# jyf588/SimGAN

Measured on AMD Instinct MI355X. Metric: env-steps/sec of GAIL-dyn PPO update, higher is better.
Workload: dtype f32; 1 GPU; northstar: GAIL-dyn update, T=128 N=512/GPU obs=47 act=12 D-in=86 policy=mlp h64 D h100 ppo_epoch=10 num_mini_batch=1...; optimizer_steps_per_update=2720, parallelism=single GPU

## Files before the change

simgan_amd/_lib.py:

```python
import ctypes as C
import os

import numpy as np

_HERE = os.path.dirname(os.path.abspath(__file__))
LIB_PATH = os.path.join(_HERE, "libsimgan_hip.so")

c_float_p = C.POINTER(C.c_float)
c_i64_p = C.POINTER(C.c_int64)
c_double_p = C.POINTER(C.c_double)
c_u8_p = C.POINTER(C.c_uint8)
c_int_p = C.POINTER(C.c_int)
H = C.c_void_p

F_OBS, F_OBS_FEAT, F_ACTIONS, F_REWARDS, F_VALUE_PREDS, F_RETURNS, F_LOGP, F_MASKS, F_BAD_MASKS, \
    F_ADVANTAGES = range(10)
POLICY_MLP, POLICY_SPLIT, POLICY_GRU = 0, 1, 2
PROF_DISC_CHAIN, PROF_DISC_WGRAD, PROF_PPO_FWD, PROF_PPO_BWD, PROF_PPO_REDUCE, PROF_RELABEL, PROF_PPO_ADAM = range(7)


class PPOConfig(C.Structure):
    _fields_ = [("clip_param", C.c_float), ("ppo_epoch", C.c_int), ("num_mini_batch", C.c_int),
                ("value_loss_coef", C.c_float), ("entropy_coef", C.c_float), ("lr", C.c_float),
                ("eps", C.c_float), ("max_grad_norm", C.c_float),
# ... 40 lines not shown
                                         c_float_p, c_float_p]),
    "sg_policy_act_ensemble": (C.c_int, [C.POINTER(H), C.c_int, C.POINTER(C.c_int32), c_float_p, C.c_int, c_float_p, C.c_uint64,
                                         C.c_int, c_float_p, c_float_p, c_float_p]),
    "sg_rollout_create": (C.c_int, [H, C.c_int, C.c_int, C.c_int, C.c_int, C.c_int, C.POINTER(H)]),
    "sg_rollout_destroy": (C.c_int, [H]),
    "sg_rollout_upload": (C.c_int, [H, C.c_int, c_float_p, C.c_int64]),
    "sg_rollout_download": (C.c_int, [H, C.c_int, c_float_p, C.c_int64]),
    "sg_rollout_upload_step": (C.c_int, [H, C.c_int, C.c_int, c_float_p, C.c_int64]),
    "sg_rollout_download_step": (C.c_int, [H, C.c_int, C.c_int, c_float_p, C.c_int64]),
    "sg_rollout_after_update": (C.c_int, [H]),
    "sg_rollout_compute_returns": (C.c_int, [H, c_float_p, C.c_int, C.c_float, C.c_float, C.c_int]),
    "sg_rollout_compute_returns_policy": (C.c_int, [H, H, C.c_int, C.c_float, C.c_float, C.c_int]),
    "sg_rollout_fill_synthetic": (C.c_int, [H, H, C.c_uint64, C.c_float]),
    "sg_rollout_count_dones": (C.c_int, [H, c_double_p]),
    "sg_ppo_create": (C.c_int, [H, H, C.POINTER(PPOConfig), C.POINTER(H)]),
    "sg_ppo_destroy": (C.c_int, [H]),
    "sg_ppo_set_lr": (C.c_int, [H, C.c_float]),
    "sg_ppo_update": (C.c_int, [H, H, c_i64_p, C.c_int64, C.c_uint64, c_float_p]),
    "sg_ppo_last_perms": (C.c_int, [H, c_i64_p, C.c_int64]),
    "sg_ppo_set_hidden_states": (C.c_int, [H, c_float_p, C.c_int64]),
    "sg_ppo_get_adam": (C.c_int, [H, c_float_p, c_float_p, C.c_int64, c_i64_p]),
    "sg_ppo_set_adam": (C.c_int, [H, c_float_p, c_float_p, C.c_int64, C.c_int64]),
    "sg_ppo_set_symmetry": (C.c_int, [H, C.c_float, c_float_p, c_float_p]),
    "sg_ppo_set_mirrored_obs": (C.c_int, [H, c_float_p, C.c_int64]),
    "sg_ppo_last_symmetry_loss": (C.c_int, [H, c_float_p]),
    "sg_a2c_create": (C.c_int, [H, H, C.POINTER(A2CConfig), C.POINTER(H)]),
    "sg_a2c_get_rmsprop": (C.c_int, [H, c_float_p, C.c_int64, c_i64_p]),
    "sg_a2c_set_rmsprop": (C.c_int, [H, c_float_p, C.c_int64, C.c_int64]),
    "sg_acktr_create": (C.c_int, [H, H, C.POINTER(ACKTRConfig), C.POINTER(H)]),
    "sg_acktr_set_value_noise": (C.c_int, [H, c_float_p, C.c_int64]),
    "sg_acktr_get_state": (C.c_int, [H, c_float_p, C.c_int64, c_float_p, C.c_int64, c_float_p, C.c_int64, c_i64_p]),
    "sg_disc_create": (C.c_int, [H, C.c_int, C.c_int, C.POINTER(H)]),
    "sg_disc_destroy": (C.c_int, [H]),
    "sg_disc_num_params": (C.c_int, [H, c_i64_p]),
    "sg_disc_set_params": (C.c_int, [H, c_float_p, C.c_int64]),
    "sg_disc_get_params": (C.c_int, [H, c_float_p, C.c_int64]),
    "sg_disc_get_adam": (C.c_int, [H, c_float_p, c_float_p, C.c_int64, c_i64_p]),
    "sg_disc_set_adam": (C.c_int, [H, c_float_p, c_float_p, C.c_int64, C.c_int64]),
    "sg_disc_set_expert": (C.c_int, [H, c_float_p, C.c_int64]),
    "sg_disc_update_gail_dyn": (C.c_int, [H, H, C.c_int, c_i64_p, C.c_int64, c_i64_p, C.c_int64, c_float_p, C.c_int64, C.c_uint64,
                                          c_float_p, c_int_p]),
    "sg_disc_update_rows": (C.c_int, [H, c_float_p, C.c_int64, C.c_int, C.c_int, c_i64_p, C.c_int64, c_i64_p, C.c_int64, c_float_p,
                                      C.c_int64, C.c_uint64, c_float_p, c_int_p]),
    "sg_disc_predict_reward": (C.c_int, [H, c_float_p, C.c_int, C.c_float, c_float_p, C.c_float, c_float_p, c_float_p]),
    "sg_disc_predict_prob": (C.c_int, [H, c_float_p, C.c_int, c_float_p]),
    "sg_disc_predict_reward_steps": (C.c_int, [H, H, C.c_float, C.c_float, c_float_p, c_float_p]),
    "sg_disc_grad_pen": (C.c_int, [H, c_float_p, c_float_p, c_float_p, C.c_int, C.c_uint64, c_float_p]),
    "sg_disc_last_draws": (C.c_int, [H, c_i64_p, c_i64_p, c_float_p, c_i64_p]),
    "sg_disc_reset_returns": (C.c_int, [H]),
    "sg_disc_get_returns": (C.c_int, [H, c_float_p, C.c_int, c_int_p]),
    "sg_disc_set_returns": (C.c_int, [H, c_float_p, C.c_int]),
    "sg_disc_relabel_rewards": (C.c_int, [H, H, C.c_float, C.c_float, c_double_p]),
    "sg_disc_relabel_rewards_auto": (C.c_int, [H, H, C.c_float, C.c_double, C.c_int]),
    "sg_disc_set_rms": (C.c_int, [H, c_double_p]),
    "sg_disc_get_scalars": (C.c_int, [H, c_double_p]),
    "sg_results_publish": (C.c_int, [H, H, H, C.c_int]),
    "sg_results_fetch": (C.c_int, [H, C.c_int, c_double_p]),
    "sg_ctx_profile": (C.c_int, [H, C.c_int]),
    "sg_ctx_profile_read": (C.c_int, [H, C.c_int, c_double_p, c_i64_p]),
    "sg_ctx_profile_reset": (C.c_int, [H]),
    "sg_host_alloc": (C.c_int, [C.c_int64, C.POINTER(C.c_void_p)]),
    "sg_host_free": (C.c_int, [C.c_void_p]),
    "sg_ctx_mark": (C.c_int, [H, c_int_p]),
    "sg_ctx_mark_elapsed": (C.c_int, [H, C.c_int, C.c_int, c_double_p]),
}

TEST_LIB_PATH = os.path.join(_HERE, "libsimgan_hip_test.so")
c_ll_p = C.POINTER(C.c_longlong)
TEST_PROTOTYPES = {
    "sg_test_last_error": (C.c_char_p, []),
    "sg_test_gemm": (C.c_int, [H, C.c_int, C.c_int, C.c_int, C.c_int, c_float_p, c_float_p, c_float_p]),
    "sg_test_gemm_bench": (C.c_int, [H, C.c_int, C.c_int, C.c_int, C.c_int, C.c_int, C.c_int, C.c_int, c_ll_p]),
    "sg_test_mfma_probe": (C.c_int, [H, C.c_int, c_float_p, c_float_p, c_float_p]),
    "sg_test_flag_probe": (C.c_int, [H, C.c_int, C.c_int, C.c_int, C.c_int, c_ll_p, c_float_p]),
    "sg_test_fetch_probe": (C.c_int, [H, C.c_int, C.c_int, C.c_int, c_ll_p]),
    "sg_test_pmc_calibrate": (C.c_int, [H, C.c_int64]),
    "sg_test_pstep_probe": (C.c_int, [H, C.c_int, C.c_int, C.c_int, C.c_int, C.c_int, c_ll_p, c_int_p]),
    "sg_test_graph_state": (C.c_int, [H, H, c_int_p]),
    "sg_test_disc_phase_times": (C.c_int, [H, C.c_int, c_ll_p, C.c_int]),
    "sg_test_disc_step4_times": (C.c_int, [H, C.c_int, c_ll_p, C.c_int]),
    "sg_test_disc_gathers": (C.c_int, [H, c_ll_p]),
    "sg_test_ppo_phase_times": (C.c_int, [H, C.c_int, c_ll_p, C.c_int]),
    "sg_test_rng": (C.c_int, [H, C.c_int, C.c_int64, C.c_uint64, C.c_void_p]),
    "sg_test_kfac_eig": (C.c_int, [H, C.c_int, c_float_p, c_float_p, c_float_p, C.POINTER(C.c_int)]),
    "sg_test_acktr_noise": (C.c_int, [H, C.c_int64, C.c_uint64, C.c_int64, c_float_p]),
    "sg_test_raise_kfac_error": (C.c_int, [H]),
    "sg_test_tear_probe": (C.c_int, [H, C.c_int, C.c_int, C.c_int, c_ll_p]),
    "sg_test_raise_handoff_error": (C.c_int, [H, H]),
}
_TEST_LIB = None

_LIB = None


class SimganHipError(RuntimeError):
    pass


def load():
    global _LIB
    if _LIB is not None:
        return _LIB
    if not os.path.exists(LIB_PATH):
        raise SimganHipError(
            f"{LIB_PATH} not found: the HIP extension is not built. There is no CPU fallback; "
            "run `make -C simgan_amd/csrc` (hipcc, gfx950).")
    lib = C.CDLL(LIB_PATH)
    for name, (res, args) in PROTOTYPES.items():
        fn = getattr(lib, name)
        fn.restype = res
        fn.argtypes = args
    _LIB = lib
    return lib


def check(rc):
    if rc != 0:
        raise SimganHipError(load().sg_last_error().decode(errors="replace"))


def load_test():
    global _TEST_LIB
    if _TEST_LIB is not None:
        return _TEST_LIB
    load()
    if not os.path.exists(TEST_LIB_PATH):
        raise SimganHipError(f"{TEST_LIB_PATH} not found: run `make -C simgan_amd/csrc`")
    lib = C.CDLL(TEST_LIB_PATH)
    for name, (res, args) in TEST_PROTOTYPES.items():
        fn = getattr(lib, name)
        fn.restype = res
        fn.argtypes = args
    _TEST_LIB = lib
    return lib


def check_test(rc):
    if rc != 0:
        raise SimganHipError(load_test().sg_test_last_error().decode(errors="replace"))


def fptr(a):
    assert isinstance(a, np.ndarray) and a.dtype == np.float32 and a.flags["C_CONTIGUOUS"], (type(a), getattr(a, "dtype", None))
    return a.ctypes.data_as(c_float_p)


def i64ptr(a):
    assert isinstance(a, np.ndarray) and a.dtype == np.int64 and a.flags["C_CONTIGUOUS"]
    return a.ctypes.data_as(c_i64_p)


def as_f32(x):
    if hasattr(x, "detach"):
        x = x.detach().cpu().numpy()
    return np.ascontiguousarray(x, dtype=np.float32)


def as_i64(x):
    if hasattr(x, "detach"):
        x = x.detach().cpu().numpy()
    return np.ascontiguousarray(x, dtype=np.int64)


class _PinnedBlock(object):

    def __init__(self, nbytes):
# ... 143 lines not shown
```

simgan_amd/csrc/sg_common.h:

```cpp
#pragma once
#include <hip/hip_runtime.h>
#include <stdint.h>

#include <string>
#include <atomic>
#include <vector>
#include <mutex>
inline std::recursive_mutex& sg_capture_mutex() { static std::recursive_mutex m; return m; }
struct SgDeviceWideGuard {
    std::lock_guard<std::recursive_mutex> l{sg_capture_mutex()};
    ~SgDeviceWideGuard() { (void)hipGetLastError(); }
};
#define SG_DEVICE_WIDE() SgDeviceWideGuard _sg_device_wide_guard
static inline hipError_t sg_dev_malloc(void** p, size_t n) { std::lock_guard<std::recursive_mutex> l(sg_capture_mutex()); return hipMalloc(p, n); }
static inline hipError_t sg_dev_free(void* p) { std::lock_guard<std::recursive_mutex> l(sg_capture_mutex()); return hipFree(p); }
static inline hipError_t sg_host_malloc(void** p, size_t n) { std::lock_guard<std::recursive_mutex> l(sg_capture_mutex()); return hipHostMalloc(p, n, hipHostMallocDefault); }
static inline hipError_t sg_host_release(void* p) { std::lock_guard<std::recursive_mutex> l(sg_capture_mutex()); return hipHostFree(p); }

#include "../../include/simgan_hip.h"
#include "sg_gemm.hpp"

void sg_set_error(const char* fmt, ...);

#define SG_CHECK(expr)                                                                      \
// ... 79 lines not shown
    hipStream_t stream = nullptr;
    int num_cu = 0;
    int lds_bytes = 0;
    bool profile = false;
    SgProfSlot prof[SG_PROF_COUNT];
    std::vector<hipEvent_t> event_pool;
    std::vector<hipEvent_t> marks;
    SgComm* comm = nullptr;
    int rank = 0, world = 1;
    bool disc_sharded = false;
    bool use_comm = false;
    std::atomic<int> n_learners{0};
    float* d_scratch = nullptr;
    size_t scratch_bytes = 0;
    void* h_pinned = nullptr;
    size_t pinned_bytes = 0;
    double* mailbox = nullptr;
    double* results = nullptr;
    hipEvent_t res_ev[8] = {nullptr};
    struct sg_disc* res_d[8] = {nullptr};
    struct sg_ppo* res_a[8] = {nullptr};
};
#define SG_RESULT_SLOTS 8

bool sg_ctx_exclusive(const sg_ctx* ctx);
void sg_ctx_learner_born(sg_ctx* ctx);
void sg_ctx_learner_gone(sg_ctx* ctx);
int sg_ctx_scratch(sg_ctx* ctx, size_t bytes, float** out);
int sg_ctx_pinned(sg_ctx* ctx, size_t bytes, void** out);
int sg_ctx_fetch_f64(sg_ctx* ctx, const double* dev, double* host, int n);
int sg_ctx_put_f64(sg_ctx* ctx, double* dev, const double* host, int n);
struct SgEv { hipEvent_t a = nullptr, b = nullptr; };
SgEv sg_prof_events(sg_ctx* ctx, int which);
#ifdef __HIPCC__
#include <hip/hip_ext.h>
#define SG_LAUNCH(ctx, which, kernel, grid, block, lds, ...)                                                  \
    do {                                                                                                      \
        if ((ctx)->profile) {                                                                                 \
            SgEv _ev = sg_prof_events(ctx, which);                                                            \
            hipExtLaunchKernelGGL(kernel, grid, block, lds, (ctx)->stream, _ev.a, _ev.b, 0, __VA_ARGS__);     \
        } else {                                                                                              \
            hipLaunchKernelGGL(kernel, grid, block, lds, (ctx)->stream, __VA_ARGS__);                         \
        }                                                                                                     \
    } while (0)
#endif

struct SgGruDesc {
    int O, H, Op, ldO, Hp, ldH;
    int off;
    int wih, whh, bih, bhh;
    int total;
};
SgGruDesc sg_make_gru_desc(int O, int H, int off);
int64_t sg_gru_flat_count(const SgGruDesc& g);
void sg_gru_pad(const SgGruDesc& g, const float* flat, float* padded);
void sg_gru_unpad(const SgGruDesc& g, const float* padded, float* flat);

struct sg_policy {
    sg_ctx* ctx;
    SgPolicyDesc desc;
    bool recurrent = false;
    SgGruDesc gru;
    float* d_params = nullptr;
    float* d_io = nullptr;
    size_t io_bytes = 0;
};

size_t sg_policy_padded_count(const sg_policy* p);
bool sg_gru_fits(const sg_ctx* ctx, const SgGruDesc& g);

#define SG_STEP4_FLAG_WORD0 64
#define SG_STEP4_MAX_FLAGS 1024
#ifndef SG_STEP4_FLAG_STRIDE
#define SG_STEP4_FLAG_STRIDE 32
#endif
#define SG_STEP4_ERR_WORD (SG_STEP4_FLAG_WORD0 + SG_STEP4_MAX_FLAGS * SG_STEP4_FLAG_STRIDE)
#define SG_STEP4_STATE_BYTES (4 * (SG_STEP4_ERR_WORD + 16))
#define SG_PAIR_ERR_WORD 0
unsigned* sg_comm_peer_err_word(struct sg_ctx* ctx);
bool sg_comm_peer_on(const struct sg_ctx* ctx);
uint32_t sg_comm_peer_generation(const struct sg_ctx* ctx);
unsigned* sg_disc_err_word(struct sg_disc* d);
uint64_t sg_next_feat_version();
struct sg_rollout {
    sg_ctx* ctx;
    int T, N, O, A, F;
    float* d_field[SG_F_COUNT] = {nullptr};
    int64_t field_count[SG_F_COUNT] = {0};
    int field_slots[SG_F_COUNT] = {0};
    int field_width[SG_F_COUNT] = {0};
    int64_t* d_perm = nullptr;
    uint64_t feat_version = sg_next_feat_version();
};

#define SG_H0_SLOTS 8
struct sg_ppo {
    int64_t opt_t = 0;
    uint64_t scratch_key = 0;
    hipGraphExec_t steps_graph = nullptr;
    bool graph_refused = false;
    uint64_t steps_graph_key[18] = {0};
    sg_ctx* ctx;
    sg_policy* policy;
    sg_ppo_config cfg;
    float *d_m = nullptr, *d_v = nullptr, *d_grad = nullptr;
    float* d_slabs = nullptr;
    size_t slabs_cap = 0;
    float* d_stacks = nullptr;
    size_t stacks_cap = 0;
    float* d_state = nullptr;
    int64_t* d_perms = nullptr;
    int64_t perms_cap = 0;
    int64_t last_perm_count = 0;
    double* d_loss_acc = nullptr;
    float* d_part = nullptr;
    long long* d_dbg = nullptr;
    unsigned* d_pair = nullptr;
    bool self_wait_failed = false;
    bool pair_primed = false;
    float sym_coef = 0.f;
    float* d_mobs_mat = nullptr;
    float* d_mact = nullptr;
    float* d_mrows = nullptr;
    int64_t mrows_cap = 0;
    int64_t mrows_host = 0;
    float* d_h0 = nullptr;
    int64_t h0_cap = 0, h0_count = 0;
    float* h_h0 = nullptr;
    hipEvent_t h0_ev[8] = {nullptr};
    uint64_t h0_calls = 0;
    float* d_gru = nullptr;
    size_t gru_cap = 0;
    int64_t gru_layout[8] = {0};
    bool a2c = false;
    float alpha = 0.f;
    struct SgKfac* kfac = nullptr;
};

struct sg_disc {
    sg_ctx* ctx;
    SgDiscDesc desc;
    bool self_wait_failed = false;
    float *d_params = nullptr, *d_m = nullptr, *d_v = nullptr;
    float* d_slabs = nullptr;
    int n_slabs = 0;
    float* d_state = nullptr;
    float* d_expert = nullptr;
    int64_t n_expert = 0;
    int64_t *d_eperm = nullptr, *d_pperm = nullptr;
    int64_t eperm_cap = 0, pperm_cap = 0;
    float* d_alpha = nullptr;
    int64_t alpha_cap = 0;
    int64_t last_draws[3] = {0, 0, 0};
    float* d_feat_all = nullptr;
    int64_t feat_all_cap = 0;
    const float* gather_src = nullptr;
    int64_t gather_rows = 0;
    uint64_t gather_version = 0;
    int64_t n_gathers = 0;
    int64_t opt_t = 0;
    hipGraphExec_t epoch_graph = nullptr;
    bool graph_refused = false;
    uint64_t epoch_graph_key[12] = {0};
    float* d_wT = nullptr;
    float *d_erows = nullptr, *d_prows = nullptr;
    int64_t erows_cap = 0, prows_cap = 0;
    float* d_rows = nullptr;
    int64_t rows_cap = 0;
    double* d_loss_acc = nullptr;
    double* d_scal = nullptr;
    int last_n_d = 0;
    float* d_returns = nullptr;
    int returns_n = 0;
    bool returns_none = true;
    uint64_t rng_calls = 0;
    long long* d_dbg_step4 = nullptr;
    long long* d_dbg = nullptr;
};

struct SgOptState {
    float lr;
    float reserved[3];
    float step_size2[2];
    float bc2_sqrt2[2];
    int t0;
    int pad[3];
};

#ifdef __HIPCC__
__attribute__((unused)) static __global__ void k_zero_f64(double* p, int n) {
    if ((int)threadIdx.x < n) p[threadIdx.x] = 0.0;
}
__attribute__((unused)) static __global__ void k_opt_commit(SgOptState* st, int n_steps) { st->t0 += n_steps; }
__device__ __forceinline__ void sg_opt_prepare(SgOptState* st, int t) {
    const double bc1 = 1.0 - pow(0.9, (double)t), bc2 = 1.0 - pow(0.999, (double)t);
    st->step_size2[t & 1] = (float)((double)st->lr / bc1);
    st->bc2_sqrt2[t & 1] = (float)sqrt(bc2);
}
#endif

#include <stdio.h>

template <typename F>
static inline int sg_try_capture(sg_ctx* ctx, hipGraphExec_t* exec, F&& enqueue) {
    std::lock_guard<std::recursive_mutex> lock(sg_capture_mutex());
    hipGraph_t graph = nullptr;
    auto refuse = [&](const char* what, hipError_t e, int rc) {
        static bool told = false;
        if (!told) {
            fprintf(stderr, "[simgan_hip] graph capture not used (%s: %s%s); falling back to direct launches\n", what,
                    e != hipSuccess ? hipGetErrorString(e) : "no HIP error", rc != 0 ? ", enqueue reported an error" : "");
            told = true;
        }
        (void)hipGetLastError();
        return 1;
    };
    hipError_t e = hipStreamBeginCapture(ctx->stream, hipStreamCaptureModeRelaxed);
    if (e != hipSuccess) return refuse("hipStreamBeginCapture", e, 0);
    const int rc = enqueue();
    e = hipStreamEndCapture(ctx->stream, &graph);
    if (rc != 0 || e != hipSuccess || !graph) {
        if (graph) (void)hipGraphDestroy(graph);
        return refuse("hipStreamEndCapture", e, rc);
    }
    e = hipGraphInstantiate(exec, graph, nullptr, nullptr, 0);
    (void)hipGraphDestroy(graph);
    if (e != hipSuccess) { *exec = nullptr; return refuse("hipGraphInstantiate", e, 0); }
    return 0;
}

int sg_comm_graph_ok(const sg_ctx* ctx);
void sg_comm_destroy(sg_ctx* ctx);
int sg_rollout_count_dones_dev(sg_rollout* r, double* d_out);
int sg_comm_allreduce_f32(sg_ctx* ctx, float* dev, int64_t n);
int sg_comm_allreduce_f64(sg_ctx* ctx, double* dev, int64_t n);
int sg_comm_allgather_f32(sg_ctx* ctx, const float* dev_in, float* dev_out, int64_t n_per_rank);
```

simgan_amd/csrc/sg_disc.hip:

```cpp
#include <math.h>
#include <stdio.h>
#include <stdlib.h>
#include <string.h>

#include <chrono>
#include <vector>

#include "sg_common.h"
#include "sg_rng.hpp"

int sg_fill_perm(sg_ctx* ctx, int64_t* d_perm, int64_t n, uint64_t seed, uint64_t stream_id);

#include "sg_disc_kernels.hpp"
#include "sg_disc_step4.hpp"

static bool disc_needs_gw(const sg_ctx* ctx, const SgDiscDesc& dd) {
    const char* e = getenv("SG_DISC_GW");
    if (e && e[0] == '1') return true;
    return disc_chain_lds_bytes(dd) > (size_t)ctx->lds_bytes;
}
static void launch_disc_chain(sg_ctx* ctx, const SgDiscDesc& dd, dim3 grid, size_t lds, const DiscArgs& a, bool gw) {
    const int kf = dd.Fp / 16, kh = dd.Hp / 16;
    const dim3 block(SG_DISC_THREADS);
    if (gw) { SG_LAUNCH(ctx, SG_PROF_DISC_CHAIN, (k_disc_chain<0, 0, true>), grid, block, lds, a); return; }
    if (kf == 6 && kh == 7) SG_LAUNCH(ctx, SG_PROF_DISC_CHAIN, (k_disc_chain<6, 7>), grid, block, lds, a);
    else if (kf == 2 && kh == 7) SG_LAUNCH(ctx, SG_PROF_DISC_CHAIN, (k_disc_chain<2, 7>), grid, block, lds, a);
    else if (kf == 1 && kh == 1) SG_LAUNCH(ctx, SG_PROF_DISC_CHAIN, (k_disc_chain<1, 1>), grid, block, lds, a);
    else SG_LAUNCH(ctx, SG_PROF_DISC_CHAIN, (k_disc_chain<0, 0>), grid, block, lds, a);
}

static bool disc_chain_thin(const sg_ctx* ctx, const SgDiscDesc& dd) {
    const char* e = getenv("SG_DISC_CHAIN");
    if (e && !strcmp(e, "wide")) return false;
    if (disc_needs_gw(ctx, dd)) return false;
    const int kf = dd.Fp / 16, kh = dd.Hp / 16;
    return (kf == 6 && kh == 7) || (kf == 2 && kh == 7) || (kf == 1 && kh == 1);
}
static void launch_disc_chain4(sg_ctx* ctx, const SgDiscDesc& dd, dim3 grid, const DiscArgs& a, const PregatherArgs& next) {
    const int kf = dd.Fp / 16, kh = dd.Hp / 16;
    const dim3 block(64 * (kf > kh ? kf : kh));
#define SG_CHAIN4(KF_, KH_)                                                                                         \
    SG_LAUNCH(ctx, SG_PROF_DISC_CHAIN, (k_disc_chain4<KF_, KH_>), grid, block, 0, a.params, a.wT, a.ops, a.part, a.dbg, \
              a.B, a.G, a.inv_B, a.lambda_, next)
    if (kf == 6 && kh == 7) SG_CHAIN4(6, 7);
    else if (kf == 2 && kh == 7) SG_CHAIN4(2, 7);
    else SG_CHAIN4(1, 1);
#undef SG_CHAIN4
}
static void launch_disc_step4(sg_ctx* ctx, const SgDiscDesc& dd, sg_disc* d, float* ops, int B, int G, int k1, const Step4Args& sa) {
    const int kf = dd.Fp / 16, kh = dd.Hp / 16;
    const dim3 grid(((12 * G + 7) & ~7) + 8 * (kh + kf) + 2 * G), block(512);
    SgOptState* st = reinterpret_cast<SgOptState*>(d->d_state);
#define SG_STEP4(KF_, KH_)                                                                                                   \
    SG_LAUNCH(ctx, SG_PROF_DISC_STEP, (k_disc_step4<KF_, KH_>), grid, block, 0, d->d_params, d->d_m, d->d_v, d->d_wT, ops, st, \
              sg_wgrad_pack(G, 0, k1), B, sa)
    if (kf == 6 && kh == 7) SG_STEP4(6, 7);
    else if (kf == 2 && kh == 7) SG_STEP4(2, 7);
    else SG_STEP4(1, 1);
#undef SG_STEP4
}
unsigned* sg_disc_err_word(sg_disc* d) { return reinterpret_cast<unsigned*>(d->d_state) + SG_STEP4_ERR_WORD; }
static void disc_refresh_images(sg_disc* d) {
    hipLaunchKernelGGL(k_disc_images, dim3(32), dim3(256), 0, d->ctx->stream, d->desc, d->d_params, d->d_wT);
}

__global__ void k_fill_alpha(float* alpha, int64_t n, uint64_t seed, uint64_t stream) {
    const int64_t i = (int64_t)blockIdx.x * blockDim.x + threadIdx.x;
    if (i < n) alpha[i] = sg_uniform(seed, stream, (uint64_t)i);
}

__global__ void __launch_bounds__(128) k_disc_grad_pen(SgDiscDesc d, const float* __restrict__ W, const float* __restrict__ e,
                                                       const float* __restrict__ p, const float* __restrict__ alpha, int n,
                                                       float* __restrict__ pen) {
    extern __shared__ float sm[];
    float* xm = sm;
    float* h1 = xm + d.Fp;
    float* h2 = h1 + d.Hp;
    float* d2 = h2 + d.Hp;
    float* d1 = d2 + d.Hp;
    float* red = d1 + d.Hp;
    const int r = blockIdx.x, t = threadIdx.x, F = d.F, Hd = d.Hd;
    if (r >= n) return;
    const float al = alpha[r];
    for (int j = t; j < F; j += blockDim.x) xm[j] = al * e[(size_t)r * F + j] + (1.0f - al) * p[(size_t)r * F + j];
    __syncthreads();
    for (int i = t; i < Hd; i += blockDim.x) {
        float a = W[d.b1 + i];
        const float* w = W + d.w1 + (size_t)i * d.ldF;
        for (int j = 0; j < F; ++j) a += w[j] * xm[j];
        h1[i] = sg_tanh(a);
    }
    __syncthreads();
    for (int i = t; i < Hd; i += blockDim.x) {
        float a = W[d.b2 + i];
        const float* w = W + d.w2 + (size_t)i * d.ldH;
        for (int k = 0; k < Hd; ++k) a += w[k] * h1[k];
        const float h = sg_tanh(a);
        h2[i] = h;
        d2[i] = W[d.w3 + i] * (1.0f - h * h);
    }
    __syncthreads();
    for (int k = t; k < Hd; k += blockDim.x) {
        float a = 0.f;
        for (int i = 0; i < Hd; ++i) a += W[d.w2 + (size_t)i * d.ldH + k] * d2[i];
        d1[k] = a * (1.0f - h1[k] * h1[k]);
    }
    __syncthreads();
    float part = 0.f;
    for (int j = t; j < F; j += blockDim.x) {
        float a = 0.f;
        for (int i = 0; i < Hd; ++i) a += W[d.w1 + (size_t)i * d.ldF + j] * d1[i];
        part += a * a;
    }
    for (int o = 32; o > 0; o >>= 1) part += __shfl_down(part, o, 64);
    if ((t & 63) == 0) red[t >> 6] = part;
    __syncthreads();
    if (t == 0) {
        const float nn = sqrtf(red[0] + red[1]);
        pen[r] = (nn - 1.0f) * (nn - 1.0f);
    }
}


struct DiscFwdArgs {
    SgDiscDesc d;
    const float* params;
    const float* x;
    int n;
    float offset;
    const double* neg_offset_dev;
    float* reward;
    int prob;
};

static size_t disc_fwd_lds_bytes(const SgDiscDesc& d, bool gw = false) {
    return sizeof(float) * ((gw ? 0 : (size_t)d.total) + 32 * d.ldF + 2 * 32 * d.ldH);
}

template <bool GW>
__global__ __launch_bounds__(256) void k_disc_forward(DiscFwdArgs a) {
    extern __shared__ __attribute__((aligned(16))) float smem[];
    constexpr int R = 32;
    const SgDiscDesc& d = a.d;
    const int tid = threadIdx.x, ldF = d.ldF, ldH = d.ldH, Fp = d.Fp, Hp = d.Hp;
    const float* W = GW ? a.params : smem;
    float* X = smem + (GW ? 0 : d.total);
    float* H1 = X + R * ldF;
    float* H2 = H1 + R * ldH;
    const float* b1 = W + d.b1;
    const float* b2 = W + d.b2;
    const float* w3 = W + d.w3;
    if (!GW) sg_stage(smem, a.params, d.total / 4);
    const float offset = a.neg_offset_dev ? -(float)(*a.neg_offset_dev) : a.offset;
    for (int base = blockIdx.x * R; base < a.n; base += gridDim.x * R) {
        __syncthreads();
        {
            const __amdgpu_buffer_rsrc_t rx = __builtin_amdgcn_make_buffer_rsrc(
                const_cast<float*>(a.x) + (size_t)base * d.F, 0, (a.n - base < R ? a.n - base : R) * d.F * 4, 0x00020000);
            for (int i0 = tid; i0 < R * Fp; i0 += 12 * blockDim.x) {
                float v[12];
#pragma unroll
                for (int u = 0; u < 12; ++u) {
                    const int i = i0 + u * blockDim.x, r = i / Fp, c = i - r * Fp;
                    const int off = (i < R * Fp && c < d.F) ? (r * d.F + c) * 4 : 0x7ffffff0;
                    v[u] = __uint_as_float(__builtin_amdgcn_raw_buffer_load_b32(rx, off, 0, 0));
                }
#pragma unroll
                for (int u = 0; u < 12; ++u) {
                    const int i = i0 + u * blockDim.x, r = i / Fp, c = i - r * Fp;
                    if (i < R * Fp) X[r * ldF + c] = v[u];
                }
            }
        }
        __syncthreads();
        sg_layer_nt<2, GW>(X, ldF, W + d.w1, ldF, Fp, Hp, [&](int r, int c, float v) { H1[r * ldH + c] = sg_tanh(v + b1[c]); });
        __syncthreads();
        sg_layer_nt<2, GW>(H1, ldH, W + d.w2, ldH, Hp, Hp, [&](int r, int c, float v) { H2[r * ldH + c] = sg_tanh(v + b2[c]); });
        __syncthreads();
        const int r = tid >> 3, sub = tid & 7;
        float s = 0.f;
        for (int c = sub; c < Hp; c += 8) s += H2[r * ldH + c] * w3[c];
        s += __shfl_xor(s, 1); s += __shfl_xor(s, 2); s += __shfl_xor(s, 4);
        if (sub == 0 && base + r < a.n) {
            const float sg = sg_sigmoid(s + W[d.b3]);
            a.reward[base + r] = a.prob ? sg : logf(sg + 1e-7f) - logf(1.f - sg + 1e-7f) + offset;
        }
    }
}

__global__ void k_returns_step(float* returns, const float* reward, const float* masks, float gamma, int first, int n) {
    const int i = blockIdx.x * blockDim.x + threadIdx.x;
    if (i < n) returns[i] = first ? reward[i] : returns[i] * gamma * masks[i] + reward[i];
}

__global__ void k_returns_scan(float* d_returns, const float* raw , const float* masks ,
                               float gamma, int first, int T, int N, float* rets ) {
    constexpr int C = 8;
    const int n = blockIdx.x * blockDim.x + threadIdx.x;
    if (n >= N) return;
    float ret = first ? 0.f : d_returns[n];
    for (int t0 = 0; t0 < T; t0 += C) {
        float rw[C], mk[C];
#pragma unroll
        for (int u = 0; u < C; ++u) {
            const int t = t0 + u < T ? t0 + u : T - 1;
            rw[u] = raw[(size_t)t * N + n];
            mk[u] = masks[(size_t)t * N + n];
        }
#pragma unroll
        for (int u = 0; u < C; ++u) {
            const int t = t0 + u;
            if (t >= T) break;
            ret = (first && t == 0) ? rw[u] : ret * gamma * mk[u] + rw[u];
            rets[(size_t)t * N + n] = ret;
        }
    }
    d_returns[n] = ret;
}

__global__ __launch_bounds__(256) void k_batch_stats(const float* rets, int N, double n_global, double* stats , int pass) {
    __shared__ double ws[4];
    const int t = blockIdx.x;
    const float* x = rets + (size_t)t * N;
    double s = 0.0;
    if (pass == 0) {
        for (int i = threadIdx.x; i < N; i += blockDim.x) s += (double)x[i];
    } else {
        const float mean = (float)(stats[t] / n_global);
        for (int i = threadIdx.x; i < N; i += blockDim.x) { const float dd = x[i] - mean; s += (double)(dd * dd); }
    }
    s = sg_wave_sum(s);
    if ((threadIdx.x & 63) == 0) ws[threadIdx.x >> 6] = s;
    __syncthreads();
    if (threadIdx.x == 0) stats[(size_t)pass * gridDim.x + t] = ws[0] + ws[1] + ws[2] + ws[3];
}

constexpr size_t SG_RMS_SCAN_LDS_BYTES = 64 * 1024;
__global__ __launch_bounds__(256) void k_rms_scan(const double* stats, int T, double n_global, double* rms ,
                                                  float* scale , int staged) {
    extern __shared__ __attribute__((aligned(16))) double sst[];
    if (staged) {
        for (int i = threadIdx.x; i < 2 * T; i += blockDim.x) sst[i] = stats[i];
        __syncthreads();
    }
    if (threadIdx.x == 0) {
        const double* st = staged ? sst : stats;
        double mean = rms[0], var = rms[1], count = rms[2];
        for (int t = 0; t < T; ++t) {
            const double bmean = (double)(float)(st[t] / n_global);
            const double bvar = (double)(float)(st[T + t] / n_global);
            const double delta = bmean - mean, tot = count + n_global;
            const double new_mean = mean + delta * n_global / tot;
            const double M2 = var * count + bvar * n_global + delta * delta * count * n_global / tot;
            mean = new_mean; var = M2 / tot; count = tot;
            if (staged) sst[2 * T + t] = sqrt(var + 1e-7);
            else scale[t] = (float)sqrt(var + 1e-7);
        }
        rms[0] = mean; rms[1] = var; rms[2] = count;
    }
    if (!staged) return;
    __syncthreads();
    for (int t = threadIdx.x; t < T; t += blockDim.x) scale[t] = (float)sst[2 * T + t];
}

__global__ void k_normalize_rewards(float* rewards, const float* scale, int T, int N) {
    const int64_t i = (int64_t)blockIdx.x * blockDim.x + threadIdx.x;
    if (i >= (int64_t)T * N) return;
    const float v = rewards[i] / scale[i / N];
    rewards[i] = fminf(fmaxf(v, -10.f), 10.f);
}


extern "C" int sg_disc_create(sg_ctx* ctx, int input_dim, int hidden_dim, sg_disc** out) {
    SG_DEVICE_WIDE();
    SG_REQUIRE(ctx && out, "sg_disc_create: NULL argument");
    SG_REQUIRE(input_dim > 0 && hidden_dim > 0, "sg_disc_create: bad dims");
    SG_CHECK(hipSetDevice(ctx->device));
    sg_disc* d = new sg_disc();
    d->ctx = ctx;
    d->desc = sg_make_disc_desc(input_dim, hidden_dim);
    SG_REQUIRE(disc_chain_lds_bytes(d->desc, true) <= (size_t)ctx->lds_bytes,
               "sg_disc_create: the activation tiles of a (%d x %d) discriminator need %zu bytes of LDS, the CU has %d", input_dim,
               hidden_dim, disc_chain_lds_bytes(d->desc, true), ctx->lds_bytes);
    const size_t tot = d->desc.total;
    SG_CHECK(sg_dev_malloc((void**)&d->d_params, sizeof(float) * tot));
    SG_CHECK(sg_dev_malloc((void**)&d->d_m, sizeof(float) * tot));
    SG_CHECK(sg_dev_malloc((void**)&d->d_v, sizeof(float) * tot));
    static_assert(sizeof(SgOptState) <= 4 * SG_STEP4_FLAG_WORD0, "the hand-off flags of k_disc_step4 sit behind the optimizer state");
    SG_CHECK(sg_dev_malloc((void**)&d->d_state, SG_STEP4_STATE_BYTES));
    SG_CHECK(hipMemsetAsync(d->d_state, 0, SG_STEP4_STATE_BYTES, ctx->stream));
    SG_CHECK(sg_dev_malloc((void**)&d->d_loss_acc, sizeof(double) * 8));
    SG_CHECK(sg_dev_malloc((void**)&d->d_scal, sizeof(double) * 8));
    {
        const double scal0[8] = {0.0, 1.0, 1e-4, 0.0, 0.0, 0.0, 0.0, 0.0};
        SG_CHECK(hipMemcpyAsync(d->d_scal, scal0, sizeof scal0, hipMemcpyHostToDevice, ctx->stream));
        SG_CHECK(hipStreamSynchronize(ctx->stream));
    }
    const size_t wT_f = (size_t)2 * d->desc.Hp * (d->desc.Fp + d->desc.Hp);
    SG_CHECK(sg_dev_malloc((void**)&d->d_wT, sizeof(float) * wT_f));
    SG_CHECK(hipMemsetAsync(d->d_wT, 0, sizeof(float) * wT_f, ctx->stream));
    SG_CHECK(hipMemsetAsync(d->d_params, 0, sizeof(float) * tot, ctx->stream));
    SG_CHECK(hipMemsetAsync(d->d_m, 0, sizeof(float) * tot, ctx->stream));
    SG_CHECK(hipMemsetAsync(d->d_v, 0, sizeof(float) * tot, ctx->stream));
    SgOptState st;
    memset(&st, 0, sizeof st);
    st.lr = 1e-3f;
    SG_CHECK(hipMemcpyAsync(d->d_state, &st, sizeof st, hipMemcpyHostToDevice, ctx->stream));
    SG_CHECK(hipStreamSynchronize(ctx->stream));
    sg_ctx_learner_born(ctx);
#if SG_STEP4_VERIFY
    SG_CHECK(sg_dev_malloc((void**)&d->d_dbg_step4, sizeof(long long) * 8 * 512 + sizeof(float) * 128 * 8 * 32 * 64 + 4 * 96 * 8 * 8 * 64 + 8 * 4 * 512));
    SG_CHECK(hipMemset(d->d_dbg_step4, 0, sizeof(long long) * 8 * 512 + sizeof(float) * 128 * 8 * 32 * 64 + 4 * 96 * 8 * 8 * 64 + 8 * 4 * 512));
#endif
    *out = d;
    return 0;
}

// ... 145 lines not shown
    const bool replicated = ctx->use_comm && !ctx->disc_sharded;
    const bool sharded = ctx->use_comm && ctx->disc_sharded;
    const bool owned = sharded && world > 1 && policy_perm != nullptr;
    SG_REQUIRE(!owned || (expert_perm && alpha), "sg_disc_update_gail_dyn: sharded data-parallel mode takes injected draws all "
               "together (expert_perm, policy_perm and alpha), or none of them");
    SG_REQUIRE(!(sharded && world > 1 && !policy_perm && (expert_perm || alpha)), "sg_disc_update_gail_dyn: sharded data-parallel "
               "mode takes injected draws all together (expert_perm, policy_perm and alpha), or none of them");
    const int split = (sharded && !owned) ? world : 1;
    SG_REQUIRE(batch_size % split == 0, "sg_disc_update_gail_dyn: batch_size %d must divide by world size %d", batch_size, world);
    SG_REQUIRE(d->n_expert >= batch_size, "The size of tensor a (%lld) must match the size of tensor b (%d) at "
               "non-singleton dimension 0 (expert rows < gail batch size)", (long long)d->n_expert, batch_size);
    SG_CHECK(hipSetDevice(ctx->device));
    const int64_t TN_glob = TN_loc * (ctx->use_comm ? world : 1);
    const int64_t TN = (replicated || owned) ? TN_glob : TN_loc;
    const int64_t n_e = d->n_expert / batch_size;
    const int64_t n_p = (sharded && !owned) ? TN_loc / (batch_size / split) : TN / batch_size;
    const int n_d = (int)(n_e < n_p ? n_e : n_p);
    SG_REQUIRE(n_d > 0, "sg_disc_update_gail_dyn: rollout (%lld rows) smaller than one batch (%d)", (long long)TN, batch_size / split);
    if (n_steps) *n_steps = n_d;
    if (expert_perm) SG_TRY(check_index_array(who, "expert_perm", expert_perm, n_expert_perm, d->n_expert, d->n_expert));
    if (policy_perm) SG_TRY(check_index_array(who, "policy_perm", policy_perm, n_policy_perm, TN, TN));
    if (alpha) SG_REQUIRE(n_alpha >= (int64_t)n_d * batch_size, "sg_disc_update_gail_dyn: alpha holds %lld draws, the epoch consumes %lld",
                          (long long)n_alpha, (long long)n_d * batch_size);
    const float* next_feat = rows_local;
    if (replicated) {
        const char* cenv = getenv("SG_DISC_GATHER_CACHE");
        const bool reuse = src_version && d->gather_version == src_version && d->gather_src == rows_local && d->gather_rows == TN_loc &&
                           d->feat_all_cap >= TN * rowF && !(cenv && !strcmp(cenv, "0"));
        if (!reuse) {
            d->gather_rows = 0;
            SG_TRY(ensure_cap(&d->d_feat_all, &d->feat_all_cap, TN * rowF, ctx->stream));
            SG_TRY(sg_comm_allgather_f32(ctx, next_feat, d->d_feat_all, TN_loc * rowF));
            d->gather_src = rows_local; d->gather_rows = TN_loc; d->gather_version = src_version;
        }
        d->n_gathers += reuse ? 0 : 1;
        next_feat = d->d_feat_all;
    }

    std::vector<int> step_cnt(n_d), step_off(n_d + 1);
    std::vector<int64_t> ep_own, pp_own;
    std::vector<float> al_own;
    int B_loc = batch_size / split;
    if (owned) {
        const int64_t Ng = n_cols ? (int64_t)n_cols * world : 0;
        B_loc = 1;
        for (int k = 0; k < n_d; ++k) {
            step_off[k] = (int)pp_own.size();
            for (int i = 0; i < batch_size; ++i) {
                const int64_t g = policy_perm[(size_t)k * batch_size + i];
                int64_t owner, local;
                if (Ng) { const int64_t t = g / Ng, c = g - t * Ng; owner = c / n_cols; local = t * n_cols + (c - owner * n_cols); }
                else { owner = g / TN_loc; local = g - owner * TN_loc; }
                if (owner != ctx->rank) continue;
                pp_own.push_back(local);
                ep_own.push_back(expert_perm[(size_t)k * batch_size + i]);
                al_own.push_back(alpha[(size_t)k * batch_size + i]);
            }
            step_cnt[k] = (int)pp_own.size() - step_off[k];
            if (step_cnt[k] > B_loc) B_loc = step_cnt[k];
        }
        step_off[n_d] = (int)pp_own.size();
    } else {
        for (int k = 0; k <= n_d; ++k) { step_off[k] = k * B_loc; if (k < n_d) step_cnt[k] = B_loc; }
    }
    const int64_t rows_total = step_off[n_d];

    SG_TRY(ensure_cap(&d->d_eperm, &d->eperm_cap, d->n_expert, ctx->stream));
    SG_TRY(ensure_cap(&d->d_pperm, &d->pperm_cap, TN, ctx->stream));
    SG_TRY(ensure_cap(&d->d_alpha, &d->alpha_cap, (int64_t)n_d * batch_size, ctx->stream));
    SG_TRY(ensure_cap(&d->d_erows, &d->erows_cap, (rows_total + B_loc) * rowF, ctx->stream));
    SG_TRY(ensure_cap(&d->d_prows, &d->prows_cap, (rows_total + B_loc) * rowF, ctx->stream));
    d->rng_calls += 1;
    d->last_draws[0] = d->n_expert; d->last_draws[1] = TN; d->last_draws[2] = (int64_t)n_d * batch_size;
    if (owned) {
        d->last_draws[0] = d->last_draws[1] = d->last_draws[2] = 0;
        if (rows_total) {
            SG_CHECK(hipMemcpyAsync(d->d_eperm, ep_own.data(), sizeof(int64_t) * rows_total, hipMemcpyHostToDevice, ctx->stream));
            SG_CHECK(hipMemcpyAsync(d->d_pperm, pp_own.data(), sizeof(int64_t) * rows_total, hipMemcpyHostToDevice, ctx->stream));
            SG_CHECK(hipMemcpyAsync(d->d_alpha, al_own.data(), sizeof(float) * rows_total, hipMemcpyHostToDevice, ctx->stream));
            SG_CHECK(hipStreamSynchronize(ctx->stream));
        }
    } else {
        if (expert_perm) SG_CHECK(hipMemcpyAsync(d->d_eperm, expert_perm, sizeof(int64_t) * d->n_expert, hipMemcpyHostToDevice, ctx->stream));
        else SG_TRY(sg_fill_perm(ctx, d->d_eperm, d->n_expert, seed, 0xE0000000ull + d->rng_calls));
        if (policy_perm) SG_CHECK(hipMemcpyAsync(d->d_pperm, policy_perm, sizeof(int64_t) * TN, hipMemcpyHostToDevice, ctx->stream));
        else SG_TRY(sg_fill_perm(ctx, d->d_pperm, TN, seed, 0xF0000000ull + d->rng_calls * 1024 + (uint64_t)(sharded ? ctx->rank : 0)));
        if (alpha) SG_CHECK(hipMemcpyAsync(d->d_alpha, alpha, sizeof(float) * (size_t)n_d * batch_size, hipMemcpyHostToDevice, ctx->stream));
        else {
            const int64_t na = (int64_t)n_d * batch_size;
            hipLaunchKernelGGL(k_fill_alpha, dim3((unsigned)((na + 255) / 256)), dim3(256), 0, ctx->stream, d->d_alpha, na,
                               seed, 0xA1000000ull + d->rng_calls);
        }
        if (!out3 && (expert_perm || policy_perm || alpha)) SG_CHECK(hipStreamSynchronize(ctx->stream));
    }

    const int G = (B_loc + 15) / 16;
    SG_REQUIRE(G < 1024 && n_d < (1 << SG_WGRAD_PACK_K1_BITS) && dd.Hp < 65536 && dd.Fp < 32768,
               "sg_disc_update_gail_dyn: %d steps per epoch / batch %d exceed the weight-gradient kernel's packed arguments "
               "(< %d steps, batch < 16384 per rank)", n_d, B_loc, 1 << SG_WGRAD_PACK_K1_BITS);
    const bool thin = disc_chain_thin(ctx, dd);
    const bool gw = disc_needs_gw(ctx, dd);
    const int n_chain_wg = thin ? 12 * G : 2 * G;
    const size_t ops_f = disc_ops_floats(dd, G), part_f = (size_t)12 * G * 4 * dd.Hp, grad_f = (size_t)dd.total + 8;
    if (d->n_slabs < G) {
        SG_CHECK(hipStreamSynchronize(ctx->stream));
        if (d->d_slabs) SG_CHECK(sg_dev_free(d->d_slabs));
        SG_CHECK(sg_dev_malloc((void**)&d->d_slabs, sizeof(float) * (2 * ops_f + part_f + grad_f)));
        d->n_slabs = G;
        SG_CHECK(hipMemsetAsync(d->d_slabs, 0, sizeof(float) * (2 * ops_f + part_f + grad_f), ctx->stream));
    }

    DiscArgs a;
    a.d = dd; a.params = d->d_params; a.expert = d->d_expert;
    a.next_feat = next_feat;
    a.B = B_loc; a.G = G; a.inv_B = 1.0f / (float)batch_size; a.lambda_ = 10.0f;
    float* stacks[2] = {d->d_slabs, d->d_slabs + ops_f};
    a.part = d->d_slabs + 2 * ops_f; a.st = reinterpret_cast<SgOptState*>(d->d_state);
    a.dbg = d->d_dbg;
    a.wT = d->d_wT;
    float* grad = d->d_slabs + 2 * ops_f + part_f;
    WgradArgs wa;
    wa.d = dd; wa.part = a.part; wa.G = G; wa.params = d->d_params; wa.m = d->d_m; wa.v = d->d_v;
    wa.grad_out = sharded ? grad : nullptr; wa.st = a.st; wa.eps = 1e-8f; wa.inv_B = a.inv_B; wa.lambda_ = a.lambda_;
    wa.loss_acc = d->d_loss_acc;
    wa.nparts = n_chain_wg; wa.wT = d->d_wT; wa.dbg = d->d_dbg;
    const size_t lds = disc_chain_lds_bytes(dd, gw);
    const int n_tiles = (dd.Hp / 16) * (dd.Hp / 16) + (dd.Hp / 16) * (dd.Fp / 16);
    const int nblk = (dd.total + 255) / 256;
    const int n_vec = (3 * dd.Hp + 4 + 63) / 64;
    const int th_ = dd.Hp / 16, tf_ = dd.Fp / 16;
    const char* xenv = getenv("SG_WGRAD_XCD");
    wa.xcd_map = (th_ <= 7 && n_vec <= (8 - th_) * (th_ + tf_) && !(xenv && !strcmp(xenv, "0"))) ? 1 : 0;
    const int n_gather_wgrad = !thin ? 2 * G : (wa.xcd_map && (8 - th_) * (th_ + tf_) > n_vec) ? 0 : 1;
    const int n_wgrad_blocks = (wa.xcd_map ? 8 * (th_ + tf_) : n_tiles + n_vec) + n_gather_wgrad;
    const char* fenv = getenv("SG_DISC_FUSED");
    const bool fused = thin && !sharded && !owned && !d->d_dbg && wa.xcd_map && 12 * G <= SG_STEP4_MAX_FLAGS && !d->self_wait_failed &&
                       (fenv ? strcmp(fenv, "0") != 0 : sg_ctx_exclusive(ctx));
    const bool dbg_timing = getenv("SG_DEBUG_TIMING") != nullptr;
    const auto t_enq0 = std::chrono::steady_clock::now();
    auto enqueue_epoch = [&]() -> int {
        hipLaunchKernelGGL(k_zero_f64, dim3(1), dim3(64), 0, ctx->stream, d->d_loss_acc, 3);
        {
            EpochRowsArgs er;
            er.expert = d->d_expert; er.feat = a.next_feat; er.eperm = d->d_eperm; er.pperm = d->d_pperm;
            er.erows = d->d_erows; er.prows = d->d_prows; er.F = dd.F;
            if (owned) {
                er.n_d = 1; er.B_loc = (int)rows_total; er.batch_size = (int)rows_total; er.roff = 0;
            } else {
                er.n_d = n_d; er.B_loc = B_loc; er.batch_size = batch_size; er.roff = sharded ? ctx->rank * B_loc : 0;
            }
            er.remap_N = (replicated && world > 1) ? n_cols : 0; er.remap_W = world; er.TN_loc = TN_loc;
            if (rows_total) hipLaunchKernelGGL(k_disc_epoch_rows, dim3(2048), dim3(256), 0, ctx->stream, er);
        }
        for (int k = 0; k < n_d; ++k) {
            const size_t al_off = owned ? (size_t)step_off[k] : (size_t)k * batch_size + (sharded ? (size_t)ctx->rank * B_loc : 0);
            const size_t al_next = owned ? (size_t)step_off[k + 1] : al_off + batch_size;
            a.eperm = d->d_eperm + al_off;
            a.alpha = d->d_alpha + al_off;
            a.pperm = d->d_pperm + (size_t)step_off[k];
            a.B = step_cnt[k];
            a.ops = stacks[k & 1];
            wa.ops = a.ops;
            PregatherArgs pg;
            pg.B = step_cnt[k]; pg.G = G; pg.F = dd.F; pg.Fp = dd.Fp; pg.ldF = dd.ldF; pg.Hp = dd.Hp; pg.st = a.st;
            wa.k1 = k + 1;
            if (k == 0) {
                pg.erows = d->d_erows; pg.prows = d->d_prows; pg.alpha = a.alpha; pg.ops = a.ops;
                hipLaunchKernelGGL(k_disc_pregather, dim3(2 * G), dim3(512), 0, ctx->stream, pg);
            }
            pg.B = k + 1 < n_d ? step_cnt[k + 1] : 0;
            pg.erows = d->d_erows + (size_t)step_off[k + 1] * dd.F; pg.prows = d->d_prows + (size_t)step_off[k + 1] * dd.F;
            pg.alpha = d->d_alpha + al_next;
            pg.ops = (k + 1 < n_d) ? stacks[(k + 1) & 1] : nullptr;
            wa.next = pg;
            if (fused) {
                Step4Args sa;
                sa.next = pg; sa.loss_acc = d->d_loss_acc;
                sa.dbg = (SG_STEP4_VERIFY || k == n_d - 2 || n_d < 2) ? d->d_dbg_step4 : nullptr;
                launch_disc_step4(ctx, dd, d, a.ops, a.B, G, wa.k1, sa);
                continue;
            }
            if (thin) launch_disc_chain4(ctx, dd, dim3(n_chain_wg + 2 * G), a, pg);
            else launch_disc_chain(ctx, dd, dim3(n_chain_wg), lds, a, gw);
            SG_LAUNCH(ctx, SG_PROF_DISC_WGRAD, k_disc_wgrad, dim3(n_wgrad_blocks), dim3(SG_WGRAD_THREADS), 0, wa.ops, wa.params, wa.m,
                      wa.v, wa.st, wa.wT, dd.Hp | (dd.Fp << 16),
                      sg_wgrad_pack(wa.G, (wa.xcd_map ? 1 : 0) | (wa.grad_out ? 2 : 0) | (wa.dbg ? 4 : 0) | (thin ? 8 : 0), wa.k1), wa);
            if (sharded) {
                SG_TRY(sg_comm_allreduce_f32(ctx, grad, (int64_t)grad_f));
                hipLaunchKernelGGL(k_disc_adam_flat, dim3(nblk), dim3(256), 0, ctx->stream, d->d_params, d->d_m, d->d_v, grad,
                                   dd.total, a.st, 1e-8f, a.inv_B, a.lambda_, d->d_loss_acc, dd, d->d_wT, wa.k1);
            }
        }
        hipLaunchKernelGGL(k_opt_commit, dim3(1), dim3(1), 0, ctx->stream, a.st, n_d);
        return 0;
    };
    const char* genv = getenv("SG_DISC_GRAPH");
    const char* gcenv = getenv("SG_DISC_GRAPH_COMM");
    const bool comm_ok = !d->graph_refused && (!sharded || (sg_comm_graph_ok(ctx) && !(gcenv && !strcmp(gcenv, "0"))));
    bool use_graph = comm_ok && !owned && !ctx->profile && !d->d_dbg && !(genv && !strcmp(genv, "0"));
    if (use_graph) {
        const uint64_t key[12] = {(uint64_t)(uintptr_t)d->d_slabs, (uint64_t)(uintptr_t)d->d_eperm, (uint64_t)(uintptr_t)d->d_pperm,
                                  (uint64_t)(uintptr_t)d->d_alpha, (uint64_t)(uintptr_t)next_feat, (uint64_t)(uintptr_t)d->d_expert,
                                  (uint64_t)n_d, (uint64_t)B_loc, (uint64_t)batch_size,
                                  (uint64_t)thin | (sharded ? 2u : 0u) | (gw ? 4u : 0u) | (fused ? 8u : 0u) | (sg_comm_peer_on(ctx) ? 16u : 0u) | ((uint64_t)((replicated && world > 1) ? n_cols : 0) << 8), (uint64_t)ops_f | ((uint64_t)sg_comm_peer_generation(ctx) << 40),
                                  (uint64_t)(uintptr_t)d->d_erows ^ ((uint64_t)(uintptr_t)d->d_prows << 1)};
        if (!d->epoch_graph || memcmp(key, d->epoch_graph_key, sizeof key) != 0) {
            if (d->epoch_graph) { SG_CHECK(hipGraphExecDestroy(d->epoch_graph)); d->epoch_graph = nullptr; }
            if (sg_try_capture(ctx, &d->epoch_graph, enqueue_epoch) != 0) {
                d->graph_refused = true;
                use_graph = false;
            } else {
                memcpy(d->epoch_graph_key, key, sizeof key);
            }
        }
        if (use_graph) SG_CHECK(hipGraphLaunch(d->epoch_graph, ctx->stream));
    }
    if (!use_graph) SG_TRY(enqueue_epoch());
    SG_CHECK(hipGetLastError());
    const auto t_enq1 = std::chrono::steady_clock::now();
    d->opt_t += n_d;
    d->last_n_d = n_d;
    if (!out3) return 0;
    double acc[3];
    SG_TRY(sg_ctx_fetch_f64(ctx, d->d_loss_acc, acc, 3));
    if (dbg_timing) {
        const auto t_done = std::chrono::steady_clock::now();
        fprintf(stderr, "[sg] disc epoch: %d steps, enqueue %.3f ms, enqueue->done %.3f ms\n", n_d,
                std::chrono::duration<double, std::milli>(t_enq1 - t_enq0).count(),
                std::chrono::duration<double, std::milli>(t_done - t_enq1).count());
    }
    if (fused && acc[0] != acc[0]) {
        unsigned err = 0;
        SG_COPY_SYNC(ctx, &err, reinterpret_cast<unsigned*>(d->d_state) + SG_STEP4_ERR_WORD, sizeof err, hipMemcpyDeviceToHost);
        if (err) {
            SG_CHECK(hipMemsetAsync(reinterpret_cast<unsigned*>(d->d_state) + SG_STEP4_ERR_WORD, 0, sizeof err, ctx->stream));
            d->self_wait_failed = true;
            SG_REQUIRE(false, "sg_disc_update_gail_dyn: the weight-gradient workgroups of k_disc_step4 waited %d s for the chain "
                       "workgroups of their own launch and gave up (the discriminator's state is undefined; SG_DISC_FUSED=0 runs "
                       "the step as two launches)", (int)(SG_STEP4_TIMEOUT_TICKS / 100000000ll));
        }
    }
    for (int i = 0; i < 3; ++i) out3[i] = (float)(acc[i] / n_d);
    return 0;
}

extern "C" int sg_disc_update_gail_dyn(sg_disc* d, sg_rollout* r, int batch_size, const int64_t* expert_perm, int64_t n_expert_perm,
                                       const int64_t* policy_perm, int64_t n_policy_perm, const float* alpha, int64_t n_alpha,
                                       uint64_t seed, float out3[3], int* n_steps) {
    SG_REQUIRE(d && r, "sg_disc_update_gail_dyn: NULL argument");
    SG_REQUIRE(r->F == d->desc.F, "sg_disc_update_gail_dyn: rollout feat_len %d != discriminator input_dim %d", r->F, d->desc.F);
    return disc_update_core(d, r->d_field[SG_F_OBS_FEAT] + (size_t)r->N * r->F, (int64_t)r->T * r->N, r->N, batch_size,
                            expert_perm, n_expert_perm, policy_perm, n_policy_perm, alpha, n_alpha, seed, out3, n_steps, r->feat_version);
}

extern "C" int sg_disc_update_rows(sg_disc* d, const float* policy_rows, int64_t n_rows, int n_cols, int batch_size,
                                   const int64_t* expert_perm, int64_t n_expert_perm, const int64_t* policy_perm, int64_t n_policy_perm,
                                   const float* alpha, int64_t n_alpha, uint64_t seed, float out3[3], int* n_steps) {
    SG_REQUIRE(d && policy_rows && n_rows > 0, "sg_disc_update_rows: bad argument");
    sg_ctx* ctx = d->ctx;
    SG_CHECK(hipSetDevice(ctx->device));
    SG_TRY(ensure_cap(&d->d_rows, &d->rows_cap, n_rows * d->desc.F, ctx->stream));
    SG_CHECK(hipMemcpyAsync(d->d_rows, policy_rows, sizeof(float) * (size_t)n_rows * d->desc.F, hipMemcpyHostToDevice, ctx->stream));
    return disc_update_core(d, d->d_rows, n_rows, n_cols, batch_size, expert_perm, n_expert_perm, policy_perm, n_policy_perm, alpha,
                            n_alpha, seed, out3, n_steps);
}

static int disc_forward_dev(sg_disc* d, const float* d_x, int n, float offset, float* d_reward, int prob = 0,
                            const double* neg_offset_dev = nullptr) {
    sg_ctx* ctx = d->ctx;
    DiscFwdArgs f;
    f.d = d->desc; f.params = d->d_params; f.x = d_x; f.n = n; f.offset = offset; f.reward = d_reward; f.prob = prob;
    f.neg_offset_dev = neg_offset_dev;
    int grid = (n + 31) / 32;
    if (grid > 2 * ctx->num_cu) grid = 2 * ctx->num_cu;
    const bool gw = disc_needs_gw(ctx, d->desc) || disc_fwd_lds_bytes(d->desc) > (size_t)ctx->lds_bytes;
    if (gw) SG_LAUNCH(ctx, SG_PROF_RELABEL, k_disc_forward<true>, dim3(grid), dim3(256), disc_fwd_lds_bytes(d->desc, true), f);
    else SG_LAUNCH(ctx, SG_PROF_RELABEL, k_disc_forward<false>, dim3(grid), dim3(256), disc_fwd_lds_bytes(d->desc), f);
    SG_CHECK(hipGetLastError());
    return 0;
}

static int ensure_returns(sg_disc* d, int n) {
    if (d->d_returns && d->returns_n == n) return 0;
    SG_REQUIRE(d->returns_none || d->returns_n == n,
               "Discriminator.returns holds %d rows but %d were passed (the reference would broadcast-fail)", d->returns_n, n);
    SG_CHECK(hipStreamSynchronize(d->ctx->stream));
    if (d->d_returns) SG_CHECK(sg_dev_free(d->d_returns));
// ... 69 lines not shown
        hipLaunchKernelGGL(k_fill_alpha, dim3((unsigned)((n + 255) / 256)), dim3(256), 0, ctx->stream, d_al, (int64_t)n, seed, 0xA2000000ull);
    }
    const size_t lds = sizeof(float) * (size_t)(dd.Fp + 4 * dd.Hp + 2);
    hipLaunchKernelGGL(k_disc_grad_pen, dim3((unsigned)n), dim3(128), lds, ctx->stream, dd, d->d_params, d_e, d_p, d_al, n, d_pen);
    SG_CHECK(hipGetLastError());
    SG_CHECK(hipMemcpyAsync(pen, d_pen, sizeof(float) * n, hipMemcpyDeviceToHost, ctx->stream));
    SG_CHECK(hipStreamSynchronize(ctx->stream));
    return 0;
}

extern "C" int sg_disc_predict_prob(sg_disc* d, const float* x, int n, float* prob) {
    SG_REQUIRE(d && x && prob && n > 0, "sg_disc_predict_prob: bad argument");
    sg_ctx* ctx = d->ctx;
    SG_CHECK(hipSetDevice(ctx->device));
    float* scratch = nullptr;
    const size_t fx = (size_t)n * d->desc.F;
    SG_TRY(sg_ctx_scratch(ctx, sizeof(float) * (fx + (size_t)n), &scratch));
    SG_CHECK(hipMemcpyAsync(scratch, x, sizeof(float) * fx, hipMemcpyHostToDevice, ctx->stream));
    SG_TRY(disc_forward_dev(d, scratch, n, 0.f, scratch + fx, 1));
    SG_CHECK(hipMemcpyAsync(prob, scratch + fx, sizeof(float) * n, hipMemcpyDeviceToHost, ctx->stream));
    SG_CHECK(hipStreamSynchronize(ctx->stream));
    return 0;
}

extern "C" int sg_disc_last_draws(sg_disc* d, int64_t* expert_perm, int64_t* policy_perm, float* alpha, int64_t counts3[3]) {
    SG_REQUIRE(d, "sg_disc_last_draws: NULL argument");
    SG_REQUIRE(d->last_draws[0] > 0, "sg_disc_last_draws: no update epoch has run on this discriminator");
    if (counts3) for (int i = 0; i < 3; ++i) counts3[i] = d->last_draws[i];
    SG_CHECK(hipSetDevice(d->ctx->device));
    SG_CHECK(hipStreamSynchronize(d->ctx->stream));
    if (expert_perm) SG_COPY_SYNC(d->ctx, expert_perm, d->d_eperm, sizeof(int64_t) * d->last_draws[0], hipMemcpyDeviceToHost);
    if (policy_perm) SG_COPY_SYNC(d->ctx, policy_perm, d->d_pperm, sizeof(int64_t) * d->last_draws[1], hipMemcpyDeviceToHost);
    if (alpha) SG_COPY_SYNC(d->ctx, alpha, d->d_alpha, sizeof(float) * d->last_draws[2], hipMemcpyDeviceToHost);
    return 0;
}

extern "C" int sg_disc_reset_returns(sg_disc* d) {
    SG_REQUIRE(d, "sg_disc_reset_returns: NULL argument");
    d->returns_none = true;
    return 0;
}

extern "C" int sg_disc_get_returns(sg_disc* d, float* returns, int n, int* is_none) {
    SG_REQUIRE(d && is_none, "sg_disc_get_returns: NULL argument");
    *is_none = d->returns_none ? 1 : 0;
    if (d->returns_none || !returns) return 0;
    SG_REQUIRE(n == d->returns_n, "sg_disc_get_returns: holds %d rows, asked for %d", d->returns_n, n);
    SG_CHECK(hipMemcpyAsync(returns, d->d_returns, sizeof(float) * n, hipMemcpyDeviceToHost, d->ctx->stream));
    SG_CHECK(hipStreamSynchronize(d->ctx->stream));
    return 0;
}

extern "C" int sg_disc_set_returns(sg_disc* d, const float* returns, int n) {
    SG_REQUIRE(d && returns && n > 0, "sg_disc_set_returns: bad argument");
    d->returns_none = true;
    SG_TRY(ensure_returns(d, n));
    SG_CHECK(hipMemcpyAsync(d->d_returns, returns, sizeof(float) * n, hipMemcpyHostToDevice, d->ctx->stream));
    SG_CHECK(hipStreamSynchronize(d->ctx->stream));
    d->returns_none = false;
    return 0;
}

static int relabel_core(sg_disc* d, sg_rollout* r, float gamma, float offset, const double* neg_offset_dev, double* rms_host) {
    sg_ctx* ctx = d->ctx;
    SG_REQUIRE(r->F == d->desc.F, "sg_disc_relabel_rewards: rollout feat_len %d != discriminator input_dim %d", r->F, d->desc.F);
    SG_CHECK(hipSetDevice(ctx->device));
    const int T = r->T, N = r->N;
    const int64_t TN = (int64_t)T * N;
    SG_TRY(ensure_returns(d, N));
    float* scratch = nullptr;
    const size_t bytes = sizeof(float) * (size_t)TN + sizeof(double) * (2 * (size_t)T + 4) + sizeof(float) * T + 64;
    SG_TRY(sg_ctx_scratch(ctx, bytes, &scratch));
    float* rets = scratch;
    double* stats = reinterpret_cast<double*>(scratch + ((TN + 3) & ~(int64_t)3));
    double* rms = rms_host ? stats + 2 * (size_t)T : d->d_scal;
    float* scale = reinterpret_cast<float*>(stats + 2 * (size_t)T + 4);
    if (rms_host) SG_TRY(sg_ctx_put_f64(ctx, rms, rms_host, 3));
    float* rewards = r->d_field[SG_F_REWARDS];
    SG_TRY(disc_forward_dev(d, r->d_field[SG_F_OBS_FEAT] + (size_t)N * r->F, (int)TN, offset, rewards, 0, neg_offset_dev));
    hipLaunchKernelGGL(k_returns_scan, dim3((N + 63) / 64), dim3(64), 0, ctx->stream, d->d_returns, rewards,
                       r->d_field[SG_F_MASKS], gamma, d->returns_none ? 1 : 0, T, N, rets);
    d->returns_none = false;
    const double n_global = (double)N * ctx->world;
    hipLaunchKernelGGL(k_batch_stats, dim3(T), dim3(256), 0, ctx->stream, rets, N, n_global, stats, 0);
    if (ctx->use_comm) SG_TRY(sg_comm_allreduce_f64(ctx, stats, T));
    hipLaunchKernelGGL(k_batch_stats, dim3(T), dim3(256), 0, ctx->stream, rets, N, n_global, stats, 1);
    if (ctx->use_comm) SG_TRY(sg_comm_allreduce_f64(ctx, stats + T, T));
    const size_t rms_lds = sizeof(double) * 3 * (size_t)T;
    const int rms_staged = rms_lds <= SG_RMS_SCAN_LDS_BYTES ? 1 : 0;
    hipLaunchKernelGGL(k_rms_scan, dim3(1), dim3(256), rms_staged ? rms_lds : 0, ctx->stream, stats, T, n_global, rms, scale, rms_staged);
    hipLaunchKernelGGL(k_normalize_rewards, dim3((unsigned)((TN + 255) / 256)), dim3(256), 0, ctx->stream, rewards, scale, T, N);
    SG_CHECK(hipGetLastError());
    if (rms_host) SG_TRY(sg_ctx_fetch_f64(ctx, rms, rms_host, 3));
    return 0;
}

extern "C" int sg_disc_relabel_rewards(sg_disc* d, sg_rollout* r, float gamma, float offset, double rms_state[3]) {
    SG_REQUIRE(d && r && rms_state, "sg_disc_relabel_rewards: NULL argument");
    return relabel_core(d, r, gamma, offset, nullptr, rms_state);
}

__global__ void k_alive_bonus(double* scal, double n_glob, double t_steps, double tar_length, int no_alive_bonus) {
    const double dones = scal[3] + n_glob / 2.0;
    const double expert_dones = (t_steps * n_glob) / tar_length;
    const double d_sa = 1.0 - dones / (dones + expert_dones);
    scal[4] = no_alive_bonus ? 0.0 : log(d_sa) - log(1.0 - d_sa);
}

extern "C" int sg_disc_relabel_rewards_auto(sg_disc* d, sg_rollout* r, float gamma, double gail_tar_length, int no_alive_bonus) {
    SG_REQUIRE(d && r && gail_tar_length > 0, "sg_disc_relabel_rewards_auto: bad argument");
    sg_ctx* ctx = d->ctx;
    SG_CHECK(hipSetDevice(ctx->device));
    SG_TRY(sg_rollout_count_dones_dev(r, d->d_scal + 3));
    hipLaunchKernelGGL(k_alive_bonus, dim3(1), dim3(1), 0, ctx->stream, d->d_scal, (double)r->N * ctx->world, (double)r->T,
                       gail_tar_length, no_alive_bonus);
    return relabel_core(d, r, gamma, 0.f, d->d_scal + 4, nullptr);
}

extern "C" int sg_disc_set_rms(sg_disc* d, const double rms_state[3]) {
    SG_REQUIRE(d && rms_state, "sg_disc_set_rms: NULL argument");
    SG_COPY_SYNC(d->ctx, d->d_scal, rms_state, sizeof(double) * 3, hipMemcpyHostToDevice);
    return 0;
}

extern "C" int sg_disc_get_scalars(sg_disc* d, double out5[5]) {
    SG_REQUIRE(d && out5, "sg_disc_get_scalars: NULL argument");
    SG_COPY_SYNC(d->ctx, out5, d->d_scal, sizeof(double) * 5, hipMemcpyDeviceToHost);
    return 0;
}
```

simgan_amd/csrc/sg_disc_kernels.hpp:

```cpp
#pragma once
#include "sg_common.h"
#include "sg_thin.hpp"

struct DiscArgs {
    SgDiscDesc d;
    const float* params;
    const float* expert;
    const float* next_feat;
    const int64_t* eperm;
    const int64_t* pperm;
    const float* alpha;
    int B;
    int G;
    float inv_B;
    float lambda_;
    float* ops;
    float* part;
    SgOptState* st;
    long long* dbg;
    const float* wT;
};

#define SG_PHASE_SYNC(n)                                                         \
    do {                                                                         \
        __syncthreads();                                                         \
        if (a.dbg && threadIdx.x == 0) a.dbg[blockIdx.x * 32 + (n)] = clock64(); \
    } while (0)

__device__ __forceinline__ float sg_log_sigmoid(float x) { return fminf(x, 0.f) - log1pf(expf(-fabsf(x))); }
__device__ __forceinline__ float sg_sigmoid(float x) { return 1.f / (1.f + expf(-x)); }

__device__ __forceinline__ float sg_rowlane_sum(float s, int L) {
    for (int o = 1; o < L; o <<= 1) s += __shfl_xor(s, o);
    return s;
}

#define SG_DISC_THREADS 512

#define SG_STK(Kt, row, c) ((((size_t)((c) >> 4)) * (size_t)(Kt) + (size_t)(row)) * 16 + ((c) & 15))
struct SgStacks { float *L2, *R2, *L1, *R1, *R1t; };
__host__ __device__ __forceinline__ SgStacks sg_disc_stacks(float* ops, int Kt, int Hp, int Fp, int ldF) {
    SgStacks k;
    k.L2 = ops; k.R2 = k.L2 + (size_t)Kt * Hp; k.L1 = k.R2 + (size_t)Kt * Hp; k.R1 = k.L1 + (size_t)Kt * Hp;
    k.R1t = k.R1 + (size_t)Kt * ldF;
    return k;
}

static size_t disc_chain_lds_bytes(const SgDiscDesc& d, bool gw = false) {
    const size_t bce = (size_t)32 * d.ldF + 2 * 32 * d.ldH + 64;
    const size_t mix = (size_t)2 * 16 * d.ldF + 7 * 16 * d.ldH + 64;
    return sizeof(float) * ((gw ? 0 : (size_t)d.total) + (bce > mix ? bce : mix));
}
static size_t disc_ops_floats(const SgDiscDesc& d, int G) {
    const size_t Kt = (size_t)64 * G;
    return Kt * (3 * (size_t)d.Hp + d.ldF + d.Fp);
}

struct PregatherArgs {
    const float* erows;
    const float* prows;
    const float* alpha;
    float* ops;
    int B, G, F, Fp, ldF, Hp;
    SgOptState* st;
};

struct EpochRowsArgs {
    const float *expert, *feat;
    const int64_t *eperm, *pperm;
    float *erows, *prows;
    int n_d, B_loc, batch_size, roff, F;
    int remap_N, remap_W;
    int64_t TN_loc;
};
__global__ __launch_bounds__(256) void k_disc_epoch_rows(EpochRowsArgs a) {
    const int64_t total = (int64_t)a.n_d * a.B_loc * a.F;
    for (int64_t i = (int64_t)blockIdx.x * blockDim.x + threadIdx.x; i < total; i += (int64_t)gridDim.x * blockDim.x) {
        const int64_t row = i / a.F;
        const int c = (int)(i - row * a.F);
        const int k = (int)(row / a.B_loc), b = (int)(row - (int64_t)k * a.B_loc);
        a.erows[i] = a.expert[(size_t)a.eperm[(size_t)k * a.batch_size + a.roff + b] * a.F + c];
        int64_t g = a.pperm[(size_t)k * a.B_loc + b];
        if (a.remap_N) {
            const int64_t Ng = (int64_t)a.remap_N * a.remap_W, t = g / Ng, cg = g - t * Ng, rk = cg / a.remap_N;
            g = rk * a.TN_loc + t * a.remap_N + (cg - rk * a.remap_N);
        }
        a.prows[i] = a.feat[(size_t)g * a.F + c];
    }
}

__device__ __forceinline__ void sg_disc_pregather(const PregatherArgs& p, int j) {
    const int nb = 16 * p.G, Kt = 4 * nb;
    const SgStacks stk = sg_disc_stacks(p.ops, Kt, p.Hp, p.Fp, p.ldF);
    float* R1s = stk.R1;
    float* R1t = stk.R1t;
    const int Fp = p.Fp, F = p.F;
    const bool bce = j < p.G;
    const int g = bce ? j : j - p.G;
    const int rows = bce ? 32 : 16;
    const int row0 = bce ? 32 * g : 3 * nb + 16 * g;
    for (int base = threadIdx.x; base < rows * Fp; base += 8 * blockDim.x) {
        float v[8];
#pragma unroll
        for (int u = 0; u < 8; ++u) {
            const int i = base + u * blockDim.x;
            const int r = i / Fp, c = i - r * Fp;
            const int b = g * 16 + (r & 15);
            v[u] = 0.f;
            if (i < rows * Fp && b < p.B && c < F) {
                if (bce) v[u] = (r < 16) ? p.erows[(size_t)b * F + c] : p.prows[(size_t)b * F + c];
                else {
                    const float al = p.alpha[b];
                    v[u] = al * p.erows[(size_t)b * F + c] + (1.f - al) * p.prows[(size_t)b * F + c];
                }
            }
        }
#pragma unroll
        for (int u = 0; u < 8; ++u) {
            const int i = base + u * blockDim.x;
            if (i < rows * Fp) {
                R1s[(size_t)(row0 + i / Fp) * p.ldF + (i % Fp)] = v[u];
                R1t[SG_STK(Kt, row0 + i / Fp, i % Fp)] = v[u];
            }
        }
    }
}

__global__ __launch_bounds__(512) void k_disc_pregather(PregatherArgs p) {
    if (blockIdx.x == 0 && threadIdx.x == 0) sg_opt_prepare(p.st, p.st->t0 + 1);
    sg_disc_pregather(p, blockIdx.x);
}

template <int KF, int KH, bool GW = false>
__global__ __launch_bounds__(SG_DISC_THREADS) void k_disc_chain(DiscArgs a) {
    extern __shared__ __attribute__((aligned(16))) float smem[];
    SgDiscDesc d = a.d;
    if (KF > 0 && KH > 0) {
        d.Fp = 16 * KF; d.ldF = d.Fp + 4; d.Hp = 16 * KH; d.ldH = d.Hp + 4;
        d.w1 = 0; d.b1 = d.Hp * d.ldF; d.w2 = d.b1 + d.Hp; d.b2 = d.w2 + d.Hp * d.ldH;
        d.w3 = d.b2 + d.Hp; d.b3 = d.w3 + d.Hp; d.total = d.b3 + 16;
    }
    const int tid = threadIdx.x;
    const int ldF = d.ldF, ldH = d.ldH, Fp = d.Fp, Hp = d.Hp;
    const float* W = GW ? a.params : smem;
    const float* W1 = W + d.w1;
    const float* b1 = W + d.b1;
    const float* W2 = W + d.w2;
    const float* b2 = W + d.b2;
    const float* w3 = W + d.w3;
    float* buf = smem + (GW ? 0 : d.total);
    const int nb = 16 * a.G, Kt = 4 * nb;
    const SgStacks stk = sg_disc_stacks(a.ops, Kt, Hp, Fp, ldF);
    float* L2s = stk.L2;
    float* R2s = stk.R2;
    float* L1s = stk.L1;
    float* R1s = stk.R1;
    float* R1t = stk.R1t;
    float* part = a.part + (size_t)blockIdx.x * (4 * Hp);
    if (a.dbg && tid == 0) a.dbg[blockIdx.x * 32] = clock64();

    const int li = tid & 15, lq = (tid & 63) >> 4;
    if ((int)blockIdx.x < a.G) {
        constexpr int R = 32;
        const int g = blockIdx.x;
        const int row0 = 32 * g;
        float* X = buf;
        float* H1 = X + R * ldF;
        float* H2 = H1 + R * ldH;
        float* DD = H2 + R * ldH;
        float* LOSS = DD + R;
        float4 wv[12];
        if (!GW) sg_stage_issue<12>(wv, a.params, d.total / 4);
        for (int i = tid; i < R * (Fp / 4); i += blockDim.x) {
            const int r = i / (Fp / 4), c = 4 * (i % (Fp / 4));
            *reinterpret_cast<float4*>(X + r * ldF + c) = *reinterpret_cast<const float4*>(R1s + (size_t)(row0 + r) * ldF + c);
        }
        if (!GW) sg_stage_commit<12>(smem, wv, a.params, d.total / 4);
        SG_PHASE_SYNC(1);
        sg_layer_nt<2, GW>(X, ldF, W1, ldF, Fp, Hp, [&](int r, int c, float v) {
            const float h = sg_tanh(v + b1[c]);
            H1[r * ldH + c] = h;
            R2s[SG_STK(Kt, row0 + r, c)] = h;
        });
        SG_PHASE_SYNC(2);
        sg_layer_nt<2, GW>(H1, ldH, W2, ldH, Hp, Hp, [&](int r, int c, float v) { H2[r * ldH + c] = sg_tanh(v + b2[c]); });
        SG_PHASE_SYNC(3);
        {
            const int L = blockDim.x / R, r = tid / L, sub = tid % L;
            float s = 0.f;
            for (int c = sub; c < Hp; c += L) s += H2[r * ldH + c] * w3[c];
            s = sg_rowlane_sum(s, L);
            if (sub == 0) {
                const float dd = s + W[d.b3];
                const bool valid = g * 16 + (r & 15) < a.B;
                float loss = 0.f, grad = 0.f;
                if (valid) {
                    if (r < 16) { loss = -sg_log_sigmoid(dd); grad = a.inv_B * (sg_sigmoid(dd) - 1.f); }
                    else { loss = dd - sg_log_sigmoid(dd); grad = a.inv_B * sg_sigmoid(dd); }
                }
                DD[r] = grad;
                LOSS[r] = loss;
            }
        }
        SG_PHASE_SYNC(4);
        for (int c = tid; c < Hp; c += blockDim.x) {
            const float w = w3[c];
            float gw = 0.f, gb = 0.f;
            for (int r = 0; r < R; ++r) {
                const float h = H2[r * ldH + c], dd = DD[r];
                gw += dd * h;
                const float dz = dd * w * (1.f - h * h);
                gb += dz;
// ... 671 lines not shown
```

simgan_amd/csrc/sg_ppo.hip:

```cpp
#include <math.h>
#include <stdlib.h>
#include <string.h>

#include <algorithm>
#include <vector>

#include "sg_common.h"
#include "sg_rng.hpp"
#include "sg_ppo_kernels.hpp"
#include "sg_kfac.hpp"
#include "sg_gru_kernels.hpp"

__global__ void k_fill_perm(int64_t* perm, int64_t n, int half_bits, uint64_t key) {
    const int64_t i = (int64_t)blockIdx.x * blockDim.x + threadIdx.x;
    if (i < n) perm[i] = sg_perm_at(i, n, half_bits, key);
}

int sg_fill_perm(sg_ctx* ctx, int64_t* d_perm, int64_t n, uint64_t seed, uint64_t stream_id) {
    const uint64_t key = sg_key(seed, 0x5045524Dull, stream_id);
    hipLaunchKernelGGL(k_fill_perm, dim3((unsigned)((n + 255) / 256)), dim3(256), 0, ctx->stream, d_perm, n,
                       sg_perm_half_bits((uint64_t)n), key);
    SG_CHECK(hipGetLastError());
    return 0;
}

static int max_trunk_floats(const SgPolicyDesc& d) {
    int m = 0;
    for (int t = 0; t < d.n_trunks; ++t) m = d.trunk[t].size > m ? d.trunk[t].size : m;
    return m;
}
static int max_bwd_floats(const SgPolicyDesc& d) {
    int m = 0;
    for (int t = 0; t < d.n_trunks; ++t) { const int s = d.trunk[t].size - d.trunk[t].w2; m = s > m ? s : m; }
    return m;
}
static int stack_ldP(const SgPolicyDesc& d) {
    int m = 0;
    for (int t = 0; t < d.n_trunks; ++t) m = d.trunk[t].ldP > m ? d.trunk[t].ldP : m;
    return m;
}
static size_t ppo_fwd_lds(const SgPolicyDesc& d, int MT, bool gw) {
    const int R = 16 * MT;
    return sizeof(float) * ((gw ? 0 : (size_t)max_trunk_floats(d)) + R * d.ldO + 2 * R * d.ldH);
}
static bool ppo_fused(const SgPolicyDesc& d, int MT) {
    const char* e = getenv("SG_PPO_FUSED");
    return d.kind == SG_POLICY_MLP && MT <= 2 && !(e && !strcmp(e, "0"));
}
static size_t ppo_bwd_lds(const SgPolicyDesc& d, int MT, bool gw) {
    const int R = 16 * MT;
    return sizeof(float) * ((gw ? 0 : (size_t)(ppo_fused(d, MT) ? max_trunk_floats(d) : max_bwd_floats(d))) + R * d.ldO + 2 * R * d.ldH + 2 * R * stack_ldP(d) +
                            ((R * d.A + 3) & ~3) + 7 * R);
}
static size_t ppo_bwd_sym_lds(const SgPolicyDesc& d, int MT, bool gw) {
    const int R = 16 * MT;
    return sizeof(float) * ((gw ? 0 : (size_t)max_bwd_floats(d)) + R * d.ldO + 2 * R * d.ldH + 3 * R * stack_ldP(d) +
                            ((R * d.A + 3) & ~3) + 7 * R + ((d.A * d.A + 3) & ~3));
}

static size_t a2c_bwd_lds(const SgPolicyDesc& d, int MT, bool gw) {
    const int R = 16 * MT;
    return sizeof(float) * ((gw ? 0 : (size_t)max_bwd_floats(d)) + R * d.ldO + 2 * R * d.ldH + 2 * R * stack_ldP(d) +
                            ((R * d.A + 3) & ~3) + 7 * R);
}
#define SG_A2C_CHUNK_ROWS 4096

#define SG_PPO_SHAPES(X) X(1, 3, 4) X(2, 3, 4)  X(2, 1, 7)  \
                         X(2, 4, 7)  X(2, 7, 4)

static int ppo_block_threads(int MT) {
    const char* we = getenv("SG_PPO_WAVES");
    return (MT >= 2 && !(we && atoi(we) == 4)) ? 512 : 256;
}

static void launch_ppo_fwd(sg_ctx* ctx, int MT, const SgPolicyDesc& d, dim3 grid, size_t lds, const PpoArgs& pa, bool gw) {
    const int ko = d.Op / 16, kh = d.Hc == d.H ? d.Hp / 16 : 0;
    const dim3 block(ppo_block_threads(MT));
    if (gw) {
        if (MT == 2) SG_LAUNCH(ctx, SG_PROF_PPO_FWD, (k_ppo_fwd<2, 0, 0, true>), grid, block, lds, pa);
        else SG_LAUNCH(ctx, SG_PROF_PPO_FWD, (k_ppo_fwd<1, 0, 0, true>), grid, block, lds, pa);
        return;
    }
#define SG_CASE(mt, o, h) \
    if (MT == mt && ko == o && kh == h) { SG_LAUNCH(ctx, SG_PROF_PPO_FWD, (k_ppo_fwd<mt, o, h>), grid, block, lds, pa); return; }
    SG_PPO_SHAPES(SG_CASE)
#undef SG_CASE
    if (MT == 4) SG_LAUNCH(ctx, SG_PROF_PPO_FWD, (k_ppo_fwd<4, 0, 0>), grid, block, lds, pa);
    else if (MT == 2) SG_LAUNCH(ctx, SG_PROF_PPO_FWD, (k_ppo_fwd<2, 0, 0>), grid, block, lds, pa);
    else SG_LAUNCH(ctx, SG_PROF_PPO_FWD, (k_ppo_fwd<1, 0, 0>), grid, block, lds, pa);
}
static void launch_ppo_fwd_critic(sg_ctx* ctx, int MT, const SgPolicyDesc& d, dim3 grid, size_t lds, const PpoArgs& pa) {
    const int ko = d.Op / 16, kh = d.Hc == d.H ? d.Hp / 16 : 0;
    const dim3 block(ppo_block_threads(MT));
    if (MT == 2 && ko == 4 && kh == 7) { SG_LAUNCH(ctx, SG_PROF_PPO_FWD, (k_ppo_fwd_critic<2, 4, 7>), grid, block, lds, pa); return; }
    if (MT == 2 && ko == 1 && kh == 7) { SG_LAUNCH(ctx, SG_PROF_PPO_FWD, (k_ppo_fwd_critic<2, 1, 7>), grid, block, lds, pa); return; }
    if (MT == 2) SG_LAUNCH(ctx, SG_PROF_PPO_FWD, (k_ppo_fwd_critic<2, 0, 0>), grid, block, lds, pa);
    else SG_LAUNCH(ctx, SG_PROF_PPO_FWD, (k_ppo_fwd_critic<1, 0, 0>), grid, block, lds, pa);
}
static void launch_ppo_pair(sg_ctx* ctx, int MT, const SgPolicyDesc& d, int G, size_t lds, const PpoArgs& pa) {
    const int ko = d.Op / 16, kh = d.Hc == d.H ? d.Hp / 16 : 0;
    const dim3 block(ppo_block_threads(MT)), grid(3 * G);
    if (MT == 2 && ko == 1 && kh == 7) { SG_LAUNCH(ctx, SG_PROF_PPO_BWD, (k_ppo_pair<2, 1, 7>), grid, block, lds, pa); return; }
    if (MT == 2 && ko == 4 && kh == 7) { SG_LAUNCH(ctx, SG_PROF_PPO_BWD, (k_ppo_pair<2, 4, 7>), grid, block, lds, pa); return; }
    if (MT == 2) SG_LAUNCH(ctx, SG_PROF_PPO_BWD, (k_ppo_pair<2, 0, 0>), grid, block, lds, pa);
// ... 124 lines not shown
    SG_CHECK(sg_dev_malloc((void**)&k->d_ks, sizeof(KfacDevState)));
    SG_CHECK(sg_dev_malloc((void**)&k->d_vec, sizeof(float) * (d.total + 8)));
    SG_CHECK(sg_dev_malloc((void**)&k->d_t0, sizeof(float) * to));
    SG_CHECK(sg_dev_malloc((void**)&k->d_t1, sizeof(float) * to));
    SG_CHECK(sg_dev_malloc((void**)&k->d_one, sizeof(float) * 4));
    SG_CHECK(sg_dev_malloc((void**)&k->d_vpart, sizeof(float) * SG_KFAC_MODULES * k->max_tiles));
    SG_CHECK(hipMemsetAsync(k->d_m, 0, sizeof(float) * fo, ctx->stream));
    SG_CHECK(hipMemsetAsync(k->d_Q, 0, sizeof(float) * fo, ctx->stream));
    SG_CHECK(hipMemsetAsync(k->d_d, 0, sizeof(float) * vo, ctx->stream));
    SG_CHECK(hipMemsetAsync(k->d_ks, 0, sizeof(KfacDevState), ctx->stream));
    SG_CHECK(hipMemsetAsync(k->d_vec, 0, sizeof(float) * (d.total + 8), ctx->stream));
    const float one[4] = {1.f, 1.f, 1.f, 1.f};
    SG_COPY_SYNC(ctx, k->d_one, one, sizeof one, hipMemcpyHostToDevice);
    std::vector<KfacJob> jobs(4 * SG_KFAC_MODULES);
    for (int m = 0; m < SG_KFAC_MODULES; ++m) {
        const KfacModule& md = k->mod[m];
        const float* Qa = md.a_f >= 0 ? k->d_Q + k->off[md.a_f] : k->d_one;
        const float* da = md.a_f >= 0 ? k->d_d + k->voff[md.a_f] : k->d_one;
        const float* Qg = k->d_Q + k->off[md.g_f];
        const float* dg = k->d_d + k->voff[md.g_f];
        float* t0 = k->d_t0 + md.toff;
        float* t1 = k->d_t1 + md.toff;
        const int M = md.out, N = md.in;
        KfacJob j;
        memset(&j, 0, sizeof j);
        j.M = M; j.N = N;
        KfacJob s1 = j, s2 = j, s3 = j, s4 = j;
        s1.K = M; s1.A = Qg; s1.lda = M; s1.ta = 1; s1.B = d_grad + md.goff; s1.ldb = md.gld; s1.C = t0; s1.ldc = N;
        s2.K = N; s2.A = t0; s2.lda = N; s2.B = Qa; s2.ldb = N; s2.C = t1; s2.ldc = N; s2.epi = 1; s2.dg = dg; s2.da = da;
        s3.K = M; s3.A = Qg; s3.lda = M; s3.B = t1; s3.ldb = N; s3.C = t0; s3.ldc = N;
        s4.K = N; s4.A = t0; s4.lda = N; s4.B = Qa; s4.ldb = N; s4.tb = 1; s4.C = k->d_vec + md.goff; s4.ldc = md.gld; s4.epi = 2;
        s4.G = d_grad + md.goff; s4.ldg = md.gld;
        jobs[0 * SG_KFAC_MODULES + m] = s1;
        jobs[1 * SG_KFAC_MODULES + m] = s2;
        jobs[2 * SG_KFAC_MODULES + m] = s3;
        jobs[3 * SG_KFAC_MODULES + m] = s4;
    }
    SG_CHECK(sg_dev_malloc((void**)&k->d_jobs, sizeof(KfacJob) * jobs.size()));
    SG_COPY_SYNC(ctx, k->d_jobs, jobs.data(), sizeof(KfacJob) * jobs.size(), hipMemcpyHostToDevice);
    std::vector<int4> tiles;
    for (int f = 0; f < SG_KFAC_NF; ++f) {
        const int T = (k->n[f] + 15) / 16;
        for (int ti = 0; ti < T; ++ti)
            for (int tj = ti; tj < T; ++tj) tiles.push_back(make_int4(f, ti, tj, 0));
    }
    k->n_tiles = (int)tiles.size();
    SG_CHECK(sg_dev_malloc((void**)&k->d_tiles, sizeof(int4) * tiles.size()));
    SG_COPY_SYNC(ctx, k->d_tiles, tiles.data(), sizeof(int4) * tiles.size(), hipMemcpyHostToDevice);
    return 0;
}

static KfacEigArgs kfac_eig_args(const SgKfac* k) {
    KfacEigArgs e;
    memset(&e, 0, sizeof e);
    e.m = k->d_m; e.Q = k->d_Q; e.dv = k->d_d; e.work = k->d_work;
    for (int f = 0; f < SG_KFAC_NF; ++f) { e.n[f] = k->n[f]; e.off[f] = k->off[f]; e.voff[f] = k->voff[f]; e.woff[f] = k->woff[f]; }
    e.lds_n = k->lds_n; e.tf = k->cfg.Tf; e.ks = k->d_ks;
    return e;
}

static size_t kfac_eig_lds(const SgKfac* k) {
    int nl = 0;
    for (int f = 0; f < SG_KFAC_NF; ++f) if (k->n[f] <= k->lds_n) nl = std::max(nl, k->n[f]);
    return sizeof(double) * 2 * (size_t)nl * nl;
}

extern "C" int sg_ppo_create(sg_ctx* ctx, sg_policy* p, const sg_ppo_config* cfg, sg_ppo** out) {
    SG_DEVICE_WIDE();
    SG_REQUIRE(ctx && p && cfg && out, "sg_ppo_create: NULL argument");
    SG_REQUIRE(!(p->recurrent && ctx->use_comm && ctx->world > 1), "sg_ppo_create: PPO with a recurrent policy runs on one rank: this "
               "context has a communicator of world %d (data-parallel PPO through time is not implemented)", ctx->world);
    SG_REQUIRE(cfg->ppo_epoch > 0 && cfg->num_mini_batch > 0, "sg_ppo_create: ppo_epoch and num_mini_batch must be positive");
    SG_REQUIRE(ppo_fwd_lds(p->desc, 1, true) <= (size_t)ctx->lds_bytes && ppo_bwd_lds(p->desc, 1, true) <= (size_t)ctx->lds_bytes,
               "sg_ppo_create: the 16-row activation tiles of this policy do not fit LDS (%zu / %zu > %d bytes)",
               ppo_fwd_lds(p->desc, 1, true), ppo_bwd_lds(p->desc, 1, true), ctx->lds_bytes);
    SG_CHECK(hipSetDevice(ctx->device));
    sg_ppo* a = new sg_ppo();
    a->ctx = ctx; a->policy = p; a->cfg = *cfg;
    const size_t tot = sg_policy_padded_count(p) + 8;
    SG_CHECK(sg_dev_malloc((void**)&a->d_m, sizeof(float) * tot));
    SG_CHECK(sg_dev_malloc((void**)&a->d_v, sizeof(float) * tot));
    SG_CHECK(sg_dev_malloc((void**)&a->d_grad, sizeof(float) * tot));
    SG_CHECK(sg_dev_malloc((void**)&a->d_state, sizeof(SgOptState)));
    SG_CHECK(sg_dev_malloc((void**)&a->d_loss_acc, sizeof(double) * 8));
    SG_CHECK(sg_dev_malloc((void**)&a->d_part, sizeof(float) * ((tot + 8 + SG_PPO_REDUCE_PARAMS - 1) / SG_PPO_REDUCE_PARAMS + 8 +
                                                                 (p->recurrent ? (p->gru.total + 255) / 256 : 0))));
    SG_CHECK(hipMemsetAsync(a->d_m, 0, sizeof(float) * tot, ctx->stream));
    SG_CHECK(hipMemsetAsync(a->d_v, 0, sizeof(float) * tot, ctx->stream));
    SG_CHECK(hipMemsetAsync(a->d_loss_acc, 0, sizeof(double) * 8, ctx->stream));
    SG_CHECK(sg_dev_malloc((void**)&a->d_pair, SG_PAIR_BYTES));
    SG_CHECK(hipMemsetAsync(a->d_pair, 0, SG_PAIR_BYTES, ctx->stream));
    SgOptState st;
    memset(&st, 0, sizeof st);
    st.lr = cfg->lr;
    SG_CHECK(hipMemcpyAsync(a->d_state, &st, sizeof st, hipMemcpyHostToDevice, ctx->stream));
    SG_CHECK(hipStreamSynchronize(ctx->stream));
    sg_ctx_learner_born(ctx);
    *out = a;
    return 0;
}

extern "C" int sg_a2c_create(sg_ctx* ctx, sg_policy* p, const sg_a2c_config* cfg, sg_ppo** out) {
    SG_REQUIRE(ctx && p && cfg && out, "sg_a2c_create: NULL argument");
    SG_REQUIRE(!p->recurrent, "sg_a2c_create: A2C is implemented for feed-forward policies only, not for a recurrent Policy");
    SG_REQUIRE(p->desc.kind == SG_POLICY_MLP, "sg_a2c_create: A2C is implemented for Policy (MLP) only, not for SplitPolicy");
    SG_REQUIRE(!(ctx->use_comm && ctx->world > 1), "sg_a2c_create: A2C runs on one rank: this context has a communicator of "
               "world %d (data-parallel A2C is not implemented)", ctx->world);
    SG_REQUIRE(cfg->alpha >= 0.f && cfg->alpha <= 1.f && cfg->eps >= 0.f && cfg->max_grad_norm > 0.f,
               "sg_a2c_create: alpha must lie in [0, 1], eps >= 0 and max_grad_norm > 0 (got %g, %g, %g)", (double)cfg->alpha,
               (double)cfg->eps, (double)cfg->max_grad_norm);
    sg_ppo_config pc;
    memset(&pc, 0, sizeof pc);
    pc.ppo_epoch = 1; pc.num_mini_batch = 1;
    pc.value_loss_coef = cfg->value_loss_coef; pc.entropy_coef = cfg->entropy_coef;
    pc.lr = cfg->lr; pc.eps = cfg->eps; pc.max_grad_norm = cfg->max_grad_norm;
    sg_ppo* a = nullptr;
    SG_TRY(sg_ppo_create(ctx, p, &pc, &a));
    a->a2c = true;
    a->alpha = cfg->alpha;
    *out = a;
    return 0;
}

extern "C" int sg_acktr_create(sg_ctx* ctx, sg_policy* p, const sg_acktr_config* cfg, sg_ppo** out) {
    SG_DEVICE_WIDE();
    SG_REQUIRE(ctx && p && cfg && out, "sg_acktr_create: NULL argument");
    SG_REQUIRE(!p->recurrent, "sg_acktr_create: ACKTR is not defined for a recurrent Policy (the reference refuses it too: "
               "a2c/arguments.py:253-255)");
    SG_REQUIRE(p->desc.kind == SG_POLICY_MLP, "sg_acktr_create: ACKTR is implemented for Policy (MLP) only, not for SplitPolicy");
    SG_REQUIRE(!(ctx->use_comm && ctx->world > 1), "sg_acktr_create: ACKTR runs on one rank: this context has a communicator of "
               "world %d (data-parallel ACKTR is not implemented)", ctx->world);
    SG_REQUIRE(cfg->lr > 0.f && cfg->momentum >= 0.f && cfg->momentum < 1.f && cfg->stat_decay > 0.f && cfg->stat_decay < 1.f &&
               cfg->kl_clip > 0.f && cfg->damping >= 0.f && cfg->Tf >= 1,
               "sg_acktr_create: need lr > 0, momentum in [0, 1), stat_decay in (0, 1), kl_clip > 0, damping >= 0 and Tf >= 1");
    sg_a2c_config ac;
    memset(&ac, 0, sizeof ac);
    ac.value_loss_coef = cfg->value_loss_coef; ac.entropy_coef = cfg->entropy_coef;
    ac.lr = cfg->lr; ac.eps = 1.f; ac.alpha = 0.f; ac.max_grad_norm = 1.f;
    sg_ppo* a = nullptr;
    SG_TRY(sg_a2c_create(ctx, p, &ac, &a));
    a->kfac = new SgKfac();
    a->kfac->cfg = *cfg;
    const int rc = kfac_setup(ctx, a->kfac, p->desc, a->d_grad);
    if (rc != 0) {
        const std::string err = sg_last_error();
        sg_ppo_destroy(a);
        sg_set_error("%s", err.c_str());
        return rc;
    }
    *out = a;
    return 0;
}

extern "C" int sg_acktr_set_value_noise(sg_ppo* a, const float* eps, int64_t n) {
    SG_REQUIRE(a, "sg_acktr_set_value_noise: NULL argument");
    SG_REQUIRE(a->kfac, "sg_acktr_set_value_noise: not an ACKTR handle");
    SgKfac* k = a->kfac;
    if (!eps) {
        k->eps_pending = false;
        k->eps_host.clear();
        return 0;
    }
    SG_REQUIRE(n > 0 && n < (1ll << 30), "sg_acktr_set_value_noise: %lld values", (long long)n);
    k->eps_host.assign(eps, eps + n);
    k->eps_pending = true;
    return 0;
}

extern "C" int sg_acktr_get_state(sg_ppo* a, float* m_aa, int64_t n_aa, float* m_gg, int64_t n_gg, float* momentum_buf,
                                  int64_t n, int64_t* steps) {
    SG_REQUIRE(a && m_aa && m_gg && momentum_buf && steps, "sg_acktr_get_state: NULL argument");
    SG_REQUIRE(a->kfac, "sg_acktr_get_state: not an ACKTR handle");
// ... 417 lines not shown
                memcpy(a->steps_graph_key, key, sizeof key);
            }
        }
        if (use_graph) SG_CHECK(hipGraphLaunch(a->steps_graph, ctx->stream));
    }
    if (!use_graph) SG_TRY(enqueue_step());
    SG_CHECK(hipGetLastError());
    a->opt_t += 1;
    if (!out3) return 0;
    double acc[4];
    SG_TRY(sg_ctx_fetch_f64(ctx, a->d_loss_acc, acc, kf ? 4 : 3));
    for (int i = 0; i < 3; ++i) out3[i] = (float)acc[i];
    SG_REQUIRE(!kf || acc[3] == 0.0, "sg_ppo_update: k_kfac_eig hit its sweep cap (%d): the K-FAC eigenbases are not valid",
               SG_KFAC_SWEEPS);
    return 0;
}

extern "C" int sg_ppo_set_hidden_states(sg_ppo* a, const float* hxs0, int64_t count) {
    SG_REQUIRE(a && hxs0, "sg_ppo_set_hidden_states: NULL argument");
    SG_REQUIRE(a->policy->recurrent, "sg_ppo_set_hidden_states: the policy is feed-forward: it has no hidden state");
    const int H = a->policy->gru.H;
    SG_REQUIRE(count > 0 && count % H == 0, "sg_ppo_set_hidden_states: %lld floats is not a whole number of %d-float states",
               (long long)count, H);
    sg_ctx* ctx = a->ctx;
    SG_CHECK(hipSetDevice(ctx->device));
    if (a->h0_cap < count) {
        SG_DEVICE_WIDE();
        SG_CHECK(hipStreamSynchronize(ctx->stream));
        if (a->d_h0) SG_CHECK(sg_dev_free(a->d_h0));
        if (a->h_h0) SG_CHECK(sg_host_release(a->h_h0));
        a->d_h0 = nullptr; a->h_h0 = nullptr; a->h0_cap = 0;
        SG_CHECK(sg_dev_malloc((void**)&a->d_h0, sizeof(float) * count));
        SG_CHECK(sg_host_malloc((void**)&a->h_h0, sizeof(float) * count * SG_H0_SLOTS));
        a->h0_cap = count;
    }
    const int slot = (int)(a->h0_calls++ % SG_H0_SLOTS);
    if (!a->h0_ev[slot]) SG_CHECK(hipEventCreateWithFlags(&a->h0_ev[slot], hipEventDisableTiming));
    else SG_CHECK(hipEventSynchronize(a->h0_ev[slot]));
    float* stage = a->h_h0 + (size_t)slot * a->h0_cap;
    memcpy(stage, hxs0, sizeof(float) * count);
    SG_CHECK(hipMemcpyAsync(a->d_h0, stage, sizeof(float) * count, hipMemcpyHostToDevice, ctx->stream));
    SG_CHECK(hipEventRecord(a->h0_ev[slot], ctx->stream));
    a->h0_count = count;
    return 0;
}

static int gru_ppo_update(sg_ppo* a, sg_rollout* r, const int64_t* perms, int64_t n_perms, uint64_t seed, float out3[3]) {
    sg_ctx* ctx = a->ctx;
    sg_policy* pol = a->policy;
    const SgPolicyDesc& d = pol->desc;
    const SgGruDesc& g = pol->gru;
    SG_REQUIRE(r->O == g.O && r->A == d.A, "sg_ppo_update: rollout dims (obs %d, act %d) do not match the policy (%d, %d)", r->O, r->A,
               g.O, d.A);
    SG_REQUIRE(!(ctx->use_comm && ctx->world > 1), "sg_ppo_update: PPO with a recurrent policy runs on one rank (world %d)", ctx->world);
    const int T = r->T, N = r->N, M = a->cfg.num_mini_batch, E = a->cfg.ppo_epoch;
    SG_REQUIRE(N >= M, "PPO requires the number of processes (%d) to be greater than or equal to the number of PPO mini batches (%d).", N, M);
    const int per = N / M;
    SG_REQUIRE(N % per == 0, "sg_ppo_update: %d processes do not split into minibatches of %d = %d // %d environments (the reference "
               "indexes past its permutation here)", N, per, N, M);
    const int S = N / per;
    SG_REQUIRE((int64_t)a->h0_count == (int64_t)N * g.H, "sg_ppo_update: a recurrent policy takes the hidden states of rollout slot 0 "
               "from the host: sg_ppo_set_hidden_states must hand over %lld floats before every update (pending: %lld)",
               (long long)N * g.H, (long long)a->h0_count);
    a->h0_count = 0;
    const int64_t TN = (int64_t)T * N;
    SG_REQUIRE(TN < (1ll << 30), "sg_ppo_update: rollout too large");
    if (perms) {
        SG_REQUIRE(n_perms == (int64_t)E * N, "sg_ppo_update: perms holds %lld indices, %d epochs x %d environments need %lld",
                   (long long)n_perms, E, N, (long long)E * N);
        std::vector<uint8_t> seen((size_t)N);
        for (int e = 0; e < E; ++e) {
            std::fill(seen.begin(), seen.end(), (uint8_t)0);
            for (int i = 0; i < N; ++i) {
                const int64_t v = perms[(size_t)e * N + i];
                SG_REQUIRE(v >= 0 && v < N && !seen[(size_t)v], "sg_ppo_update: perms of epoch %d are not a permutation of the %d environments", e, N);
                seen[(size_t)v] = 1;
            }
        }
    }
    SG_CHECK(hipSetDevice(ctx->device));

    float* adv = r->d_field[SG_F_ADVANTAGES];
    double* stats = a->d_loss_acc + 4;
    hipLaunchKernelGGL(k_adv_stats, dim3(1), dim3(1024), 0, ctx->stream, r->d_field[SG_F_RETURNS], r->d_field[SG_F_VALUE_PREDS], TN, adv, stats, 0);
    hipLaunchKernelGGL(k_adv_stats, dim3(1), dim3(1024), 0, ctx->stream, r->d_field[SG_F_RETURNS], r->d_field[SG_F_VALUE_PREDS], TN, adv, stats, 1);
    hipLaunchKernelGGL(k_adv_stats, dim3(64), dim3(1024), 0, ctx->stream, r->d_field[SG_F_RETURNS], r->d_field[SG_F_VALUE_PREDS], TN, adv, stats, 2);
    SG_CHECK(hipGetLastError());

    if (a->perms_cap < (int64_t)E * N) {
        SG_CHECK(hipStreamSynchronize(ctx->stream));
        if (a->d_perms) SG_CHECK(sg_dev_free(a->d_perms));
        a->d_perms = nullptr; a->perms_cap = 0;
        SG_CHECK(sg_dev_malloc((void**)&a->d_perms, sizeof(int64_t) * (size_t)E * N));
        a->perms_cap = (int64_t)E * N;
    }
    a->last_perm_count = (int64_t)E * N;
    if (perms) {
        SG_CHECK(hipMemcpyAsync(a->d_perms, perms, sizeof(int64_t) * (size_t)E * N, hipMemcpyHostToDevice, ctx->stream));
        if (!out3) SG_CHECK(hipStreamSynchronize(ctx->stream));
    } else {
        for (int e = 0; e < E; ++e) SG_TRY(sg_fill_perm(ctx, a->d_perms + (size_t)e * N, N, seed, (uint64_t)e * 2654435761ull));
    }

    const int mb = T * per;
    const bool gw = sg_policy_needs_gw(ctx, d) || ppo_fwd_lds(d, 1, false) > (size_t)ctx->lds_bytes;
    const int ldP = stack_ldP(d);
    auto bwd_lds = [&](int mt) {
        const int R = 16 * mt;
        return sizeof(float) * ((gw ? 0 : (size_t)max_trunk_floats(d)) + R * d.ldO + 2 * R * d.ldH + 2 * R * ldP + ((R * d.A + 3) & ~3) + 7 * R);
    };
    int MT = ((mb + 31) / 32) * d.n_trunks >= ctx->num_cu ? 2 : 1;
    if (MT == 2 && bwd_lds(2) > (size_t)ctx->lds_bytes) MT = 1;
    SG_REQUIRE(bwd_lds(MT) <= (size_t)ctx->lds_bytes, "sg_ppo_update: the heads' 16-row tiles do not fit LDS (%zu bytes)", bwd_lds(MT));
    const int R = 16 * MT, G = (mb + R - 1) / R, mbp = G * R;
    const int slab_stride = (d.total + 8 + 63) & ~63;
    const int TNp = (int)TN + 64;
    const int rows_p = (mb + 15) & ~15;
    const int Hp = g.Hp, G3 = 3 * Hp;
    const int chunks = rows_p / 16;
    const int KS = std::max(1, std::min(16, chunks / 8));
    const int gblocks = (g.total + 255) / 256;
    const int nblk_r = (d.total + 8 + SG_PPO_REDUCE_PARAMS - 1) / SG_PPO_REDUCE_PARAMS;
    const int tot_all = d.total + g.total;
    const int nblk = (tot_all + 8 + 255) / 256;

    const size_t slab_f = (size_t)G * slab_stride;
    const size_t hx_f = (size_t)(mbp + 64) * d.ldO;
    const size_t stack_f = hx_f + (size_t)TNp * d.A + 4 * (size_t)TNp;
    auto r4 = [](size_t x) { return (x + 3) & ~(size_t)3; };
    const size_t o_x = 0, o_mk = o_x + r4((size_t)TNp * g.ldO), o_h0 = o_mk + r4((size_t)TNp), o_gi = o_h0 + r4((size_t)N * g.H);
    const size_t o_sr = o_gi + (size_t)rows_p * G3, o_sz = o_sr + (size_t)rows_p * Hp, o_sn = o_sz + (size_t)rows_p * Hp;
    const size_t o_shn = o_sn + (size_t)rows_p * Hp, o_hm = o_shn + (size_t)rows_p * Hp, o_dgi = o_hm + (size_t)rows_p * g.ldH;
    const size_t o_dgh = o_dgi + (size_t)rows_p * G3, o_dxa = o_dgh + (size_t)rows_p * G3, o_dxc = o_dxa + (size_t)mbp * d.ldO;
    const size_t o_part = o_dxc + (size_t)mbp * d.ldO, gru_f = o_part + (size_t)KS * g.total;
    if (a->slabs_cap < slab_f || a->stacks_cap < stack_f || a->gru_cap < gru_f) {
        SG_CHECK(hipStreamSynchronize(ctx->stream));
        if (a->d_slabs) SG_CHECK(sg_dev_free(a->d_slabs));
        if (a->d_stacks) SG_CHECK(sg_dev_free(a->d_stacks));
        if (a->d_gru) SG_CHECK(sg_dev_free(a->d_gru));
        a->d_slabs = a->d_stacks = a->d_gru = nullptr;
        a->slabs_cap = a->stacks_cap = a->gru_cap = 0;
        SG_CHECK(sg_dev_malloc((void**)&a->d_slabs, sizeof(float) * slab_f));
        SG_CHECK(sg_dev_malloc((void**)&a->d_stacks, sizeof(float) * stack_f));
        SG_CHECK(sg_dev_malloc((void**)&a->d_gru, sizeof(float) * gru_f));
        a->slabs_cap = slab_f; a->stacks_cap = stack_f; a->gru_cap = gru_f;
        a->scratch_key = 0;
    }
    const int64_t layout[8] = {G, slab_stride, mbp, TNp, MT, KS, per, ((int64_t)g.total << 32) | (int64_t)rows_p};
    if (a->scratch_key != 0x475255ull || memcmp(layout, a->gru_layout, sizeof layout) != 0) {
        SG_CHECK(hipMemsetAsync(a->d_slabs, 0, sizeof(float) * slab_f, ctx->stream));
        SG_CHECK(hipMemsetAsync(a->d_stacks, 0, sizeof(float) * stack_f, ctx->stream));
        SG_CHECK(hipMemsetAsync(a->d_gru, 0, sizeof(float) * gru_f, ctx->stream));
        memcpy(a->gru_layout, layout, sizeof layout);
        a->scratch_key = 0x475255ull;
    }
    hipLaunchKernelGGL(k_zero_f64, dim3(1), dim3(64), 0, ctx->stream, a->d_loss_acc, 4);

    float* hX = a->d_stacks;
    float* epACT = hX + hx_f;
    float* epSC = epACT + (size_t)TNp * d.A;
    float* gb = a->d_gru;

    GruGatherArgs ga;
    ga.obs = r->d_field[SG_F_OBS]; ga.actions = r->d_field[SG_F_ACTIONS]; ga.old_logp = r->d_field[SG_F_LOGP]; ga.adv = adv;
    ga.vpred = r->d_field[SG_F_VALUE_PREDS]; ga.ret = r->d_field[SG_F_RETURNS]; ga.masks = r->d_field[SG_F_MASKS]; ga.h0 = a->d_h0;
    ga.T = T; ga.N = N; ga.per = per; ga.O = g.O; ga.ldO = g.ldO; ga.A = d.A; ga.H = g.H; ga.sc_stride = TNp;
    ga.X = gb + o_x; ga.ACT = epACT; ga.SC = epSC; ga.MK = gb + o_mk; ga.H0 = gb + o_h0;

    PpoArgs pa;
    pa.d = d; pa.params = pol->d_params;
    pa.sc_stride = TNp; pa.mb = mb; pa.mbp = mbp; pa.inv_B = 1.0f / (float)mb;
    pa.clip = a->cfg.clip_param; pa.vcoef = a->cfg.value_loss_coef; pa.ecoef = a->cfg.entropy_coef;
    pa.use_clipped = a->cfg.use_clipped_value_loss;
    pa.slabs = a->d_slabs; pa.slab_stride = slab_stride; pa.ldP = ldP; pa.dbg = nullptr;
    pa.st = reinterpret_cast<SgOptState*>(a->d_state); pa.G = G; pa.k1 = 0;
    pa.pair = a->d_pair; pa.Xm = nullptr; pa.MA = nullptr; pa.sym_c = 0.f;
    for (int t = 0; t < 3; ++t) { pa.H1[t] = hX; pa.H2[t] = hX; pa.OUT[t] = hX; }
    pa.X = hX;
    pa.DX[0] = gb + o_dxa; pa.DX[1] = gb + o_dxc;
    pa.wbuf_floats = gw ? 0 : max_trunk_floats(d);

    GruScanArgs tr;
    tr.sr = gb + o_sr; tr.sz = gb + o_sz; tr.sn = gb + o_sn; tr.shn = gb + o_shn; tr.hm = gb + o_hm;
    GruBwdArgs ba;
// ... 93 lines not shown
    }
    if (a->policy->recurrent) return gru_ppo_update(a, r, perms, n_perms, seed, out3);
    sg_ctx* ctx = a->ctx;
    const SgPolicyDesc& d = a->policy->desc;
    SG_REQUIRE(r->O == d.O && r->A == d.A, "sg_ppo_update: rollout dims (obs %d, act %d) do not match the policy (%d, %d)",
               r->O, r->A, d.O, d.A);
    const int64_t TN = (int64_t)r->T * r->N;
    const int M = a->cfg.num_mini_batch, E = a->cfg.ppo_epoch;
    SG_REQUIRE(TN >= M, "PPO requires the number of processes (%d) * number of steps (%d) = %lld to be greater than "
               "or equal to the number of PPO mini batches (%d).", r->N, r->T, (long long)TN, M);
    SG_CHECK(hipSetDevice(ctx->device));
    const int world = ctx->world;
    const bool owned = perms != nullptr && ctx->use_comm && world > 1;
    const int64_t TN_perm = owned ? TN * world : TN;
    if (perms) {
        SG_REQUIRE(n_perms == (int64_t)E * TN_perm, "sg_ppo_update: perms holds %lld indices, %d epochs x %lld rows need %lld",
                   (long long)n_perms, E, (long long)TN_perm, (long long)E * TN_perm);
        for (int64_t i = 0; i < n_perms; ++i)
            SG_REQUIRE(perms[i] >= 0 && perms[i] < TN_perm, "sg_ppo_update: perms[%lld] = %lld is outside [0, %lld)", (long long)i,
                       (long long)perms[i], (long long)TN_perm);
    }
    std::vector<int> step_cnt((size_t)E * M), step_off((size_t)E * M);
    std::vector<int64_t> own_perm;
    std::vector<int64_t> epoch_rows(E, TN);
    int mb = (int)(TN / M);
    int64_t mb_global = (int64_t)mb * (ctx->use_comm ? world : 1);
    if (owned) {
        const int64_t Ng = (int64_t)r->N * world;
        mb_global = TN_perm / M;
        own_perm.assign((size_t)E * TN, 0);
        mb = 1;
        std::vector<uint8_t> seen((size_t)TN_perm);
        for (int e = 0; e < E; ++e) {
            std::fill(seen.begin(), seen.end(), (uint8_t)0);
            for (int64_t i = 0; i < TN_perm; ++i) {
                const int64_t g = perms[(size_t)e * TN_perm + i];
                SG_REQUIRE(!seen[(size_t)g], "sg_ppo_update: perms of epoch %d repeat row id %lld: not a permutation", e, (long long)g);
                seen[(size_t)g] = 1;
            }
            int64_t n_own = 0;
            for (int k = 0; k < M; ++k) {
                step_off[(size_t)e * M + k] = (int)n_own;
                for (int64_t i = 0; i < mb_global; ++i) {
                    const int64_t g = perms[(size_t)e * TN_perm + (size_t)k * mb_global + i];
                    const int64_t t = g / Ng, c = g - t * Ng, owner = c / r->N;
                    if (owner == ctx->rank) {
                        SG_REQUIRE(n_own < TN, "sg_ppo_update: epoch %d hands this rank more than its %lld rows", e, (long long)TN);
                        own_perm[(size_t)e * TN + n_own++] = t * r->N + (c - owner * r->N);
                    }
                }
                const int cnt = (int)n_own - step_off[(size_t)e * M + k];
                step_cnt[(size_t)e * M + k] = cnt;
                if (cnt > mb) mb = cnt;
            }
            epoch_rows[e] = n_own;
        }
    } else {
        for (int e = 0; e < E; ++e)
            for (int k = 0; k < M; ++k) { step_cnt[(size_t)e * M + k] = mb; step_off[(size_t)e * M + k] = k * mb; }
    }

    const bool sym = a->sym_coef > 0.f;
    if (sym) {
        if (a->d_mobs_mat) {
            if (a->mrows_cap < TN * d.O) {
                SG_CHECK(hipStreamSynchronize(ctx->stream));
                if (a->d_mrows) SG_CHECK(sg_dev_free(a->d_mrows));
                SG_CHECK(sg_dev_malloc((void**)&a->d_mrows, sizeof(float) * TN * d.O));
                a->mrows_cap = TN * d.O;
            }
            hipLaunchKernelGGL(k_mirror_rows, dim3((unsigned)((TN * d.O + 255) / 256)), dim3(256), 0, ctx->stream,
                               r->d_field[SG_F_OBS], a->d_mobs_mat, a->d_mrows, TN, d.O);
            SG_CHECK(hipGetLastError());
        } else {
            SG_REQUIRE(a->mrows_host == TN * d.O, "sg_ppo_update: the symmetry loss takes its mirrored observations from the host: "
                       "sg_ppo_set_mirrored_obs must hand over %lld floats (T*N rows of %d) before every update (pending: %lld)",
                       (long long)(TN * d.O), d.O, (long long)a->mrows_host);
            a->mrows_host = 0;
        }
    }

    float* adv = r->d_field[SG_F_ADVANTAGES];
    double* stats = a->d_loss_acc + 4;
    hipLaunchKernelGGL(k_adv_stats, dim3(1), dim3(1024), 0, ctx->stream, r->d_field[SG_F_RETURNS],
                       r->d_field[SG_F_VALUE_PREDS], TN, adv, stats, 0);
    if (ctx->use_comm) SG_TRY(sg_comm_allreduce_f64(ctx, stats, 3));
    hipLaunchKernelGGL(k_adv_stats, dim3(1), dim3(1024), 0, ctx->stream, r->d_field[SG_F_RETURNS],
                       r->d_field[SG_F_VALUE_PREDS], TN, adv, stats, 1);
    if (ctx->use_comm) SG_TRY(sg_comm_allreduce_f64(ctx, stats + 1, 1));
    hipLaunchKernelGGL(k_adv_stats, dim3(64), dim3(1024), 0, ctx->stream, r->d_field[SG_F_RETURNS],
                       r->d_field[SG_F_VALUE_PREDS], TN, adv, stats, 2);
    SG_CHECK(hipGetLastError());

    if (a->perms_cap < (int64_t)E * TN) {
        SG_CHECK(hipStreamSynchronize(ctx->stream));
        if (a->d_perms) SG_CHECK(sg_dev_free(a->d_perms));
        SG_CHECK(sg_dev_malloc((void**)&a->d_perms, sizeof(int64_t) * (size_t)E * TN));
        a->perms_cap = (int64_t)E * TN;
    }
    a->last_perm_count = owned ? 0 : (int64_t)E * TN;
    if (owned) {
        SG_CHECK(hipMemcpyAsync(a->d_perms, own_perm.data(), sizeof(int64_t) * (size_t)E * TN, hipMemcpyHostToDevice, ctx->stream));
        SG_CHECK(hipStreamSynchronize(ctx->stream));
    } else if (perms) {
        SG_CHECK(hipMemcpyAsync(a->d_perms, perms, sizeof(int64_t) * (size_t)E * TN, hipMemcpyHostToDevice, ctx->stream));
        if (!out3) SG_CHECK(hipStreamSynchronize(ctx->stream));
    } else {
        for (int e = 0; e < E; ++e)
            SG_TRY(sg_fill_perm(ctx, a->d_perms + (size_t)e * TN, TN, seed, (uint64_t)e * 2654435761ull + (uint64_t)ctx->rank));
    }

    const int ncols = d.n_trunks + (sym ? 1 : 0);
    int MT = ((size_t)((mb + 15) / 16) * (size_t)(d.total + 8) * sizeof(float) > ((size_t)24 << 20) ||
              ((mb + 31) / 32) * ncols >= ctx->num_cu) ? 2 : 1;
    if (const char* e = getenv("SG_PPO_ROWS")) {
        const int v = atoi(e);
        if (v == 16 || v == 32 || v == 64) MT = v / 16;
    }
    const bool gw = sg_policy_needs_gw(ctx, d) || ppo_fwd_lds(d, 1, false) > (size_t)ctx->lds_bytes ||
                    ppo_bwd_lds(d, 1, false) > (size_t)ctx->lds_bytes || (sym && ppo_bwd_sym_lds(d, 1, false) > (size_t)ctx->lds_bytes);
    if ((gw || sym) && MT > 2) MT = 2;
    while (MT > 1 && (ppo_fwd_lds(d, MT, gw) > (size_t)ctx->lds_bytes || ppo_bwd_lds(d, MT, gw) > (size_t)ctx->lds_bytes ||
                      (sym && ppo_bwd_sym_lds(d, MT, gw) > (size_t)ctx->lds_bytes))) MT /= 2;
    const int R = 16 * MT;
    const int G = (mb + R - 1) / R;
    const int mbp = G * R;
    const int ldP = stack_ldP(d);
    const int slab_stride = (d.total + 8 + 63) & ~63;
    const int TNp = (int)TN + 64 + (owned ? mbp : 0);

    const size_t slab_f = (size_t)(sym ? 2 : 1) * G * slab_stride;
    const size_t xm_off = ((size_t)TNp * (d.ldO + d.A + 4) + 3) & ~(size_t)3;
    const size_t epoch_f = sym ? xm_off + (size_t)TNp * d.ldO : (size_t)TNp * (d.ldO + d.A + 4);
    const size_t stack_f = (size_t)ncols * mbp * (2 * (size_t)d.ldH + ldP);
    if (a->slabs_cap < slab_f || a->stacks_cap < epoch_f + stack_f) {
        SG_CHECK(hipStreamSynchronize(ctx->stream));
        if (a->d_slabs) SG_CHECK(sg_dev_free(a->d_slabs));
        if (a->d_stacks) SG_CHECK(sg_dev_free(a->d_stacks));
        SG_CHECK(sg_dev_malloc((void**)&a->d_slabs, sizeof(float) * slab_f));
        SG_CHECK(sg_dev_malloc((void**)&a->d_stacks, sizeof(float) * (epoch_f + stack_f)));
        a->slabs_cap = slab_f;
        a->stacks_cap = epoch_f + stack_f;
        a->scratch_key = 0;
    }
    const uint64_t key = ((uint64_t)G << 40) ^ ((uint64_t)slab_stride << 20) ^ ((uint64_t)mbp << 8) ^ (uint64_t)TNp ^ ((uint64_t)MT << 60) ^
                         ((uint64_t)sym << 63);
    if (a->scratch_key != key) {
        SG_CHECK(hipMemsetAsync(a->d_slabs, 0, sizeof(float) * slab_f, ctx->stream));
        SG_CHECK(hipMemsetAsync(a->d_stacks, 0, sizeof(float) * (epoch_f + stack_f), ctx->stream));
        a->scratch_key = key;
    }
    hipLaunchKernelGGL(k_zero_f64, dim3(1), dim3(64), 0, ctx->stream, a->d_loss_acc, 4);

    float* epX = a->d_stacks;
    float* epACT = epX + (size_t)TNp * d.ldO;
    float* epSC = epACT + (size_t)TNp * d.A;
    float* epXm = sym ? a->d_stacks + xm_off : nullptr;
    float* stk = a->d_stacks + epoch_f;

    EpochGatherArgs ga;
    ga.obs = r->d_field[SG_F_OBS]; ga.actions = r->d_field[SG_F_ACTIONS]; ga.old_logp = r->d_field[SG_F_LOGP];
    ga.adv = adv; ga.vpred = r->d_field[SG_F_VALUE_PREDS]; ga.ret = r->d_field[SG_F_RETURNS];
    ga.TN = TN; ga.O = d.O; ga.Op = d.Op; ga.ldO = d.ldO; ga.A = d.A; ga.sc_stride = TNp;
    ga.X = epX; ga.ACT = epACT; ga.SC = epSC;
    ga.mobs = sym ? a->d_mrows : nullptr; ga.Xm = epXm;

    PpoArgs pa;
    pa.d = d; pa.params = a->policy->d_params;
    pa.sc_stride = TNp; pa.mb = mb; pa.mbp = mbp; pa.inv_B = 1.0f / (float)mb_global;
    pa.clip = a->cfg.clip_param; pa.vcoef = a->cfg.value_loss_coef; pa.ecoef = a->cfg.entropy_coef;
    pa.use_clipped = a->cfg.use_clipped_value_loss;
    pa.slabs = a->d_slabs; pa.slab_stride = slab_stride; pa.ldP = ldP; pa.dbg = a->d_dbg;
    pa.st = reinterpret_cast<SgOptState*>(a->d_state); pa.G = G; pa.k1 = 0;
    pa.pair = a->d_pair;
    pa.Xm = nullptr; pa.MA = a->d_mact;
    pa.sym_c = sym ? (float)(2.0 * a->sym_coef / ((double)mb_global * d.A)) : 0.f;
    for (int t = 0; t < 3; ++t) {
        const bool on = t < ncols;
        pa.H1[t] = on ? stk : nullptr; if (on) stk += (size_t)mbp * d.ldH;
        pa.H2[t] = on ? stk : nullptr; if (on) stk += (size_t)mbp * d.ldH;
        pa.OUT[t] = on ? stk : nullptr; if (on) stk += (size_t)mbp * ldP;
    }
    const int wb_f = gw ? 0 : max_trunk_floats(d), wb_b = gw ? 0 : max_bwd_floats(d);
    const bool fused = !sym && ppo_fused(d, MT);
    const size_t lds_fc = sizeof(float) * ((size_t)wb_f + R * d.ldO + 2 * R * d.ldH + 2 * R * ldP + ((R * d.A + 3) & ~3) + 7 * R);
    const char* cfenv = getenv("SG_PPO_CRITIC_FIRST");
    const bool crit_first = !gw && !fused && d.kind == SG_POLICY_SPLIT && MT <= 2 && lds_fc <= (size_t)ctx->lds_bytes &&
                            (cfenv ? cfenv[0] == '1' : G * d.n_trunks > ctx->num_cu);
    const char* penv = getenv("SG_PPO_PAIR");
    const bool pair = !gw && !fused && !crit_first && d.kind == SG_POLICY_SPLIT && d.n_trunks == 3 && MT <= 2 &&
                      lds_fc <= (size_t)ctx->lds_bytes && 3 * G <= ctx->num_cu && 2 * ldP + 2 <= std::min(d.trunk[0].ldH, d.trunk[1].ldH) && !a->d_dbg &&
                      !a->self_wait_failed && (penv ? strcmp(penv, "0") != 0 : sg_ctx_exclusive(ctx));
    if (pair && !a->pair_primed) SG_CHECK(hipMemsetAsync(a->d_stacks, 0, sizeof(float) * (epoch_f + stack_f), ctx->stream));
    a->pair_primed = pair;
    const size_t lds_f = ppo_fwd_lds(d, MT, gw), lds_b = sym ? ppo_bwd_sym_lds(d, MT, gw) : ppo_bwd_lds(d, MT, gw);
    const int nblk = (d.total + 8 + 255) / 256;
    const int nblk_r = (d.total + 8 + SG_PPO_REDUCE_PARAMS - 1) / SG_PPO_REDUCE_PARAMS;
    SgOptState* st = reinterpret_cast<SgOptState*>(a->d_state);

    auto enqueue_steps = [&]() -> int {
        hipLaunchKernelGGL(k_opt_prepare_first, dim3(1), dim3(1), 0, ctx->stream, st);
        for (int e = 0; e < E; ++e) {
            ga.perm = a->d_perms + (size_t)e * TN;
            ga.TN = epoch_rows[e];
            if (ga.TN) hipLaunchKernelGGL(sym ? k_ppo_epoch_gather_sym : k_ppo_epoch_gather, dim3((unsigned)((ga.TN + 63) / 64)), dim3(256), 0,
                                          ctx->stream, ga);
            for (int k = 0; k < M; ++k) {
                const size_t rb = (size_t)step_off[(size_t)e * M + k];
                pa.mb = step_cnt[(size_t)e * M + k];
                pa.X = epX + rb * d.ldO; pa.ACT = epACT + rb * d.A; pa.SC = epSC + rb;
                if (sym) pa.Xm = epXm + rb * d.ldO;
                pa.k1 = e * M + k + 1;
                if (sym) {
                    pa.wbuf_floats = wb_f;
                    launch_ppo_fwd_sym(ctx, MT, d, dim3(G, 3), lds_f, pa, gw);
                    pa.wbuf_floats = wb_b;
                    launch_ppo_bwd_sym(ctx, MT, d, dim3(G, 3), lds_b, pa, gw);
                } else if (pair) {
                    pa.wbuf_floats = wb_f;
                    launch_ppo_pair(ctx, MT, d, G, lds_fc, pa);
                } else if (crit_first) {
                    pa.wbuf_floats = wb_f;
                    launch_ppo_fwd_critic(ctx, MT, d, dim3(G, d.n_trunks), lds_fc > lds_f ? lds_fc : lds_f, pa);
                    pa.wbuf_floats = wb_b;
                    launch_ppo_bwd(ctx, MT, d, dim3(G, d.n_trunks - 1), lds_b, pa, false, false);
                } else {
                    if (!fused) {
                        pa.wbuf_floats = wb_f;
                        launch_ppo_fwd(ctx, MT, d, dim3(G, d.n_trunks), lds_f, pa, gw);
                    }
                    pa.wbuf_floats = fused ? wb_f : wb_b;
                    launch_ppo_bwd(ctx, MT, d, dim3(G, d.n_trunks), lds_b, pa, fused, gw);
                }
                if (sym) SG_LAUNCH(ctx, SG_PROF_PPO_REDUCE, k_ppo_reduce_sym, dim3(nblk_r), dim3(256), 0, a->d_slabs, G, slab_stride,
                                   d.total, a->d_grad, a->d_part, d.trunk[0].off, d.trunk[0].off + d.trunk[0].ex);
                else SG_LAUNCH(ctx, SG_PROF_PPO_REDUCE, k_ppo_reduce, dim3(nblk_r), dim3(256), 0, a->d_slabs, G, slab_stride,
                               d.total, a->d_grad, a->d_part);
                if (ctx->use_comm) {
                    SG_TRY(sg_comm_allreduce_f32(ctx, a->d_grad, d.total + 8));
                    hipLaunchKernelGGL(k_sumsq, dim3(nblk), dim3(256), 0, ctx->stream, a->d_grad, d.total, a->d_part);
                }
                SG_LAUNCH(ctx, SG_PROF_PPO_ADAM, sym ? k_ppo_adam_sym : k_ppo_adam, dim3(nblk), dim3(256), 0, a->policy->d_params, a->d_m,
                          a->d_v, a->d_grad, a->d_part, ctx->use_comm ? nblk : nblk_r, d.total, st, e * M + k + 1, a->cfg.eps,
                          a->cfg.max_grad_norm, pa.inv_B, a->d_loss_acc);
            }
        }
        hipLaunchKernelGGL(k_opt_commit, dim3(1), dim3(1), 0, ctx->stream, st, E * M);
        return 0;
    };
    const char* genv = getenv("SG_PPO_GRAPH");
    const char* gcenv = getenv("SG_PPO_GRAPH_COMM");
    const bool comm_ok = !a->graph_refused && (!ctx->use_comm || (sg_comm_graph_ok(ctx) && !(gcenv && !strcmp(gcenv, "0"))));
    bool use_graph = comm_ok && !owned && !ctx->profile && !a->d_dbg && !(genv && !strcmp(genv, "0"));
    if (use_graph) {
        uint32_t fbits[6];
        const float fv[6] = {a->cfg.clip_param, a->cfg.value_loss_coef, a->cfg.entropy_coef, a->cfg.eps, a->cfg.max_grad_norm, pa.inv_B};
        memcpy(fbits, fv, sizeof fbits);
        uint32_t cbits;
        memcpy(&cbits, &a->sym_coef, sizeof cbits);
        const uint64_t key[18] = {(uint64_t)(uintptr_t)a->d_slabs, (uint64_t)(uintptr_t)a->d_stacks, (uint64_t)(uintptr_t)a->d_perms,
                                  (uint64_t)(uintptr_t)r->d_field[SG_F_OBS], (uint64_t)(uintptr_t)r->d_field[SG_F_ACTIONS],
                                  (uint64_t)(uintptr_t)r->d_field[SG_F_RETURNS], (uint64_t)(uintptr_t)a->policy->d_params,
                                  (uint64_t)TN, ((uint64_t)E << 32) | (uint64_t)M, ((uint64_t)MT << 32) | (uint64_t)G,
                                  ((uint64_t)fbits[0] << 32) | fbits[1], ((uint64_t)fbits[2] << 32) | fbits[3],
                                  ((uint64_t)fbits[4] << 32) | fbits[5], (uint64_t)a->cfg.use_clipped_value_loss,
                                  (uint64_t)(uintptr_t)r->d_field[SG_F_LOGP], 0x50504full + (fused ? 1 : 0) + (ctx->use_comm ? 2 : 0) + (crit_first ? 4 : 0) + (gw ? 8 : 0) + (pair ? 16 : 0) + (sg_comm_peer_on(ctx) ? 32 : 0) + (sym ? 64 : 0) + ((uint64_t)sg_comm_peer_generation(ctx) << 32),
                                  sym ? (uint64_t)(uintptr_t)a->d_mrows : 0, sym ? (uint64_t)cbits : 0};
        if (!a->steps_graph || memcmp(key, a->steps_graph_key, sizeof key) != 0) {
            if (a->steps_graph) { SG_CHECK(hipGraphExecDestroy(a->steps_graph)); a->steps_graph = nullptr; }
            if (sg_try_capture(ctx, &a->steps_graph, enqueue_steps) != 0) {
                a->graph_refused = true;
                use_graph = false;
            } else {
                memcpy(a->steps_graph_key, key, sizeof key);
            }
        }
        if (use_graph) SG_CHECK(hipGraphLaunch(a->steps_graph, ctx->stream));
    }
    if (!use_graph) SG_TRY(enqueue_steps());
    SG_CHECK(hipGetLastError());
    a->opt_t += (int64_t)E * M;
    if (!out3) return 0;
    double acc[3];
    SG_TRY(sg_ctx_fetch_f64(ctx, a->d_loss_acc, acc, 3));
    if (pair && (acc[0] != acc[0] || acc[1] != acc[1] || acc[2] != acc[2])) {
        unsigned err = 0;
        SG_COPY_SYNC(ctx, &err, a->d_pair + SG_PAIR_ERR_WORD, sizeof err, hipMemcpyDeviceToHost);
        if (err) {
            SG_CHECK(hipMemsetAsync(a->d_pair + SG_PAIR_ERR_WORD, 0, sizeof err, ctx->stream));
            a->self_wait_failed = true;
            SG_REQUIRE(false, "sg_ppo_update: a workgroup of k_ppo_pair waited %d s for its partner's words and gave "
                       "up (the policy's state is undefined; SG_PPO_PAIR=0 runs the multi-launch step)", (int)(SG_PAIR_TIMEOUT_TICKS / 100000000ll));
        }
    }
    const double nu = (double)E * M;
    for (int i = 0; i < 3; ++i) out3[i] = (float)(acc[i] / nu);
    return 0;
}

__global__ void k_publish(double* dst, const double* d_acc, const double* d_scal, const double* p_acc, double n_d, double n_p,
                          const unsigned* d_err, const unsigned* a_err, const unsigned* peer_err) {
    const int t = threadIdx.x;
    if (t < 3) dst[t] = d_acc ? d_acc[t] : 0.0;
    else if (t < 8) dst[t] = d_scal ? d_scal[t - 3] : 0.0;
    else if (t < 11) dst[t] = p_acc ? p_acc[t - 8] : 0.0;
    else if (t == 11) dst[t] = n_d;
    else if (t == 12) dst[t] = n_p;
    else if (t == 13) dst[t] = d_err ? (double)*d_err : 0.0;
    else if (t == 14) dst[t] = a_err ? (double)*a_err : 0.0;
    else if (t == 15) dst[t] = peer_err ? (double)__hip_atomic_load(peer_err, __ATOMIC_RELAXED, __HIP_MEMORY_SCOPE_AGENT) : 0.0;
}

extern "C" int sg_results_publish(sg_ctx* ctx, sg_disc* d, sg_ppo* a, int slot) {
    SG_REQUIRE(ctx && slot >= 0 && slot < SG_RESULT_SLOTS, "sg_results_publish: bad argument");
    SG_REQUIRE((!d || d->ctx == ctx) && (!a || a->ctx == ctx), "sg_results_publish: objects of another context");
    SG_CHECK(hipSetDevice(ctx->device));
    hipLaunchKernelGGL(k_publish, dim3(1), dim3(64), 0, ctx->stream, ctx->results + 16 * slot, d ? d->d_loss_acc : nullptr,
                       d ? d->d_scal : nullptr, a ? a->d_loss_acc : nullptr, d ? (double)d->last_n_d : 1.0,
                       a ? (double)a->cfg.ppo_epoch * a->cfg.num_mini_batch : 1.0,
                       d ? sg_disc_err_word(d) : nullptr,
                       (a && a->kfac) ? reinterpret_cast<const unsigned*>(&a->kfac->d_ks->err)
                                      : (a && a->d_pair) ? a->d_pair + SG_PAIR_ERR_WORD : nullptr,
                       sg_comm_peer_err_word(ctx));
    SG_CHECK(hipGetLastError());
    SG_CHECK(hipEventRecord(ctx->res_ev[slot], ctx->stream));
    ctx->res_d[slot] = d;
    ctx->res_a[slot] = a;
    return 0;
}

extern "C" int sg_results_fetch(sg_ctx* ctx, int slot, double out13[13]) {
    SG_REQUIRE(ctx && out13 && slot >= 0 && slot < SG_RESULT_SLOTS, "sg_results_fetch: bad argument");
    SG_CHECK(hipEventSynchronize(ctx->res_ev[slot]));
    const double* src = ctx->results + 16 * slot;
    memcpy(out13, src, sizeof(double) * 13);
    const bool d_err = src[13] != 0.0;
    const bool k_err = src[14] != 0.0 && ctx->res_a[slot] && ctx->res_a[slot]->kfac;
    const bool a_err = src[14] != 0.0 && !k_err;
    if (src[15] != 0.0) {
        SG_CHECK(hipSetDevice(ctx->device));
        if (unsigned* w = sg_comm_peer_err_word(ctx)) SG_CHECK(hipMemsetAsync(w, 0, sizeof(unsigned), ctx->stream));
        SG_REQUIRE(false, "sg_results_fetch: rank %d: a peer-mesh all-reduce (SG_COMM_PEER) waited 20 s for a peer's flags and gave up "
                   "during or before the update this slot reports; that step's gradient was NaN on this rank", ctx->rank);
    }
    if (d_err || a_err) {
        SG_CHECK(hipSetDevice(ctx->device));
        sg_disc* d = ctx->res_d[slot];
        sg_ppo* a = ctx->res_a[slot];
        if (d_err && d) {
// ... 17 lines not shown
```

simgan_amd/csrc/sg_ppo_kernels.hpp:

```cpp
#pragma once
#include "sg_common.h"
#include "sg_thin.hpp"

#define HALF_LOG_2PI 0.91893853320467274178f

struct PpoArgs {
    SgPolicyDesc d;
    const float* params;
    const float* X;
    const float* ACT;
    const float* SC;
    int sc_stride;
    int mb, mbp;
    float inv_B;
    float clip, vcoef, ecoef;
    int use_clipped;
    float* H1[3];
    float* H2[3];
    float* OUT[3];
    float* slabs;
    int slab_stride;
    int ldP;
    int wbuf_floats;
    long long* dbg;
    SgOptState* st;
    int k1, G;
    unsigned* pair;
    const float* Xm;
    const float* MA;
    float sym_c;
    float* DX[2] = {nullptr, nullptr};
};

#define SG_PAIR_BYTES 64
#define SG_PAIR_TIMEOUT_TICKS 300000000ll



#define SG_LDS_SYNC() asm volatile("s_waitcnt lgkmcnt(0)\n\ts_barrier" ::: "memory")

#define SG_PPO_STAMP(n) do { if (a.dbg && threadIdx.x == 0 && blockIdx.y == 0) a.dbg[blockIdx.x * 16 + (n)] = clock64(); } while (0)
#define SG_PPO_WALL(n) do { if (a.dbg && threadIdx.x == 0 && blockIdx.y < 2) a.dbg[(blockIdx.x + 512 * blockIdx.y) * 16 + (n)] = wall_clock64(); } while (0)

struct EpochGatherArgs {
    const float *obs, *actions, *old_logp, *adv, *vpred, *ret;
    const int64_t* perm;
    int64_t TN;
    int O, Op, ldO, A, sc_stride;
    float *X, *ACT, *SC;
    const float* mobs;
    float* Xm;
};

template <bool SYM = false, bool ROLLOUT_ORDER = false>
__device__ __forceinline__ void sg_ppo_epoch_gather_body(const EpochGatherArgs& a) {
    __shared__ int IDX[64];
    const int tid = threadIdx.x;
    const int64_t row0 = (int64_t)blockIdx.x * 64;
    if (tid < 64) {
        const int64_t rr = row0 + tid;
        const int idx = rr < a.TN ? (ROLLOUT_ORDER ? (int)rr : (int)a.perm[rr]) : -1;
        IDX[tid] = idx;
        if (ROLLOUT_ORDER) {
            if (idx >= 0) a.SC[3 * (size_t)a.sc_stride + rr] = a.ret[idx];
        } else if (idx >= 0) {
            a.SC[0 * (size_t)a.sc_stride + rr] = a.old_logp[idx];
            a.SC[1 * (size_t)a.sc_stride + rr] = a.adv[idx];
            a.SC[2 * (size_t)a.sc_stride + rr] = a.vpred[idx];
            a.SC[3 * (size_t)a.sc_stride + rr] = a.ret[idx];
        }
    }
    __syncthreads();
    for (int base = tid; base < 64 * a.Op; base += 8 * blockDim.x) {
        float v[8];
#pragma unroll
        for (int u = 0; u < 8; ++u) {
            const int i = base + u * blockDim.x;
            const int r = i / a.Op, c = i - r * a.Op;
            v[u] = (i < 64 * a.Op && IDX[r] >= 0 && c < a.O) ? a.obs[(size_t)IDX[r] * a.O + c] : 0.f;
        }
#pragma unroll
        for (int u = 0; u < 8; ++u) {
            const int i = base + u * blockDim.x;
            if (i < 64 * a.Op && IDX[i / a.Op] >= 0) a.X[(size_t)(row0 + i / a.Op) * a.ldO + (i % a.Op)] = v[u];
        }
        if (SYM) {
#pragma unroll
            for (int u = 0; u < 8; ++u) {
                const int i = base + u * blockDim.x;
                const int r = i / a.Op, c = i - r * a.Op;
                v[u] = (i < 64 * a.Op && IDX[r] >= 0 && c < a.O) ? a.mobs[(size_t)IDX[r] * a.O + c] : 0.f;
            }
#pragma unroll
            for (int u = 0; u < 8; ++u) {
                const int i = base + u * blockDim.x;
                if (i < 64 * a.Op && IDX[i / a.Op] >= 0) a.Xm[(size_t)(row0 + i / a.Op) * a.ldO + (i % a.Op)] = v[u];
            }
        }
    }
    for (int i = tid; i < 64 * a.A; i += blockDim.x) {
        const int r = i / a.A, c = i - r * a.A;
        if (IDX[r] >= 0) a.ACT[(size_t)(row0 + r) * a.A + c] = a.actions[(size_t)IDX[r] * a.A + c];
    }
}

__global__ __launch_bounds__(256) void k_ppo_epoch_gather(EpochGatherArgs a) { sg_ppo_epoch_gather_body<false>(a); }
__global__ __launch_bounds__(256) void k_ppo_epoch_gather_sym(EpochGatherArgs a) { sg_ppo_epoch_gather_body<true>(a); }
__global__ __launch_bounds__(256) void k_a2c_gather(EpochGatherArgs a) { sg_ppo_epoch_gather_body<false, true>(a); }

__global__ __launch_bounds__(256) void k_mirror_rows(const float* obs, const float* m, float* out, int64_t rows, int O) {
    const int64_t idx = (int64_t)blockIdx.x * blockDim.x + threadIdx.x;
    if (idx >= rows * O) return;
    const int64_t r = idx / O;
    const int i = (int)(idx - r * O);
    const float* x = obs + r * O;
    const float* mi = m + (size_t)i * O;
    double s = 0.0;
    for (int j = 0; j < O; ++j) {
        const float w = mi[j];
        if (w != 0.f) s += (double)w * (double)x[j];
    }
    out[idx] = (float)s;
}

template <int MT, int KO, int KH, bool GW = false, bool SYM = false>
__device__ __forceinline__ void sg_ppo_fwd_body(const PpoArgs& a, const int t, const int bx) {
    extern __shared__ __attribute__((aligned(16))) float smem[];
    constexpr int R = 16 * MT;
    const SgPolicyDesc& d = a.d;
    const int tid = threadIdx.x;
    const bool mirror = SYM && t == 2;
    const SgTrunk tr = d.trunk[mirror ? 0 : t];
    const int Op = (KO > 0 && KH > 0) ? 16 * KO : d.Op, Hp = (KO > 0 && KH > 0) ? 16 * KH : tr.Hp;
    const int ldO = Op + 4, ldH = Hp + 4, ldP = a.ldP;
    const float* W = GW ? a.params + tr.off : smem;
    float* X = smem + a.wbuf_floats;
    float* H1 = X + R * ldO;
    float* H2 = H1 + R * ldH;
    const int row0 = bx * R;

    SG_PPO_STAMP(0);
// ... 488 lines not shown
    if (threadIdx.x == 0) part[blockIdx.x] = ws[0] + ws[1] + ws[2] + ws[3];
}

template <int NL>
__device__ __forceinline__ void sg_ppo_adam_body(float* params, float* m, float* v, const float* grad,
                                                 const float* part, int n_part, int total,
                                                 const SgOptState* st, int k1, float eps, float max_norm,
                                                 float inv_mb, double* loss_acc) {
    __shared__ float s_coef;
    const int t = st->t0 + k1;
    const float s_step_size = st->step_size2[t & 1], s_bc2_sqrt = st->bc2_sqrt2[t & 1];
    __shared__ float s_ws[4];
    {
        float s = 0.f;
        for (int j = threadIdx.x; j < n_part; j += 256) s += part[j];
        s = sg_wave_sum(s);
        if ((threadIdx.x & 63) == 0) s_ws[threadIdx.x >> 6] = s;
    }
    __syncthreads();
    if (threadIdx.x == 0) {
        const float norm = sqrtf((s_ws[0] + s_ws[1]) + (s_ws[2] + s_ws[3]));
        float coef = max_norm / (norm + 1e-6f);
        s_coef = coef > 1.f ? 1.f : coef;
    }
    __syncthreads();
    const int i = blockIdx.x * blockDim.x + threadIdx.x;
    if (i < total) {
        const float g = grad[i] * s_coef;
        float mi = m[i], vi = v[i];
        mi = mi + (g - mi) * (float)(1.0 - 0.9);
        vi = vi * (float)0.999 + (float)(1.0 - 0.999) * g * g;
        const float denom = sqrtf(vi) / s_bc2_sqrt + eps;
        params[i] = params[i] - s_step_size * (mi / denom);
        m[i] = mi;
        v[i] = vi;
    }
    if (blockIdx.x == 0 && threadIdx.x < NL)
        loss_acc[threadIdx.x] += (double)(grad[total + threadIdx.x] * inv_mb);
    if (blockIdx.x == 0 && threadIdx.x == 64) sg_opt_prepare(const_cast<SgOptState*>(st), t + 1);
}
__global__ __launch_bounds__(256) void k_ppo_adam(float* params, float* m, float* v, const float* grad,
                                                  const float* part, int n_part, int total,
                                                  const SgOptState* st, int k1, float eps, float max_norm,
                                                  float inv_mb, double* loss_acc) {
    sg_ppo_adam_body<3>(params, m, v, grad, part, n_part, total, st, k1, eps, max_norm, inv_mb, loss_acc);
}
__global__ __launch_bounds__(256) void k_ppo_adam_sym(float* params, float* m, float* v, const float* grad,
                                                      const float* part, int n_part, int total,
                                                      const SgOptState* st, int k1, float eps, float max_norm,
                                                      float inv_mb, double* loss_acc) {
    sg_ppo_adam_body<4>(params, m, v, grad, part, n_part, total, st, k1, eps, max_norm, inv_mb, loss_acc);
}

__global__ __launch_bounds__(256) void k_a2c_rmsprop(float* params, float* sq, const float* grad, const float* part, int n_part,
                                                     int total, const SgOptState* st, float alpha, float one_m_alpha, float eps,
                                                     float max_norm, float inv_b, double* loss_acc) {
    __shared__ float s_coef;
    __shared__ float s_ws[4];
    {
        float s = 0.f;
        for (int j = threadIdx.x; j < n_part; j += 256) s += part[j];
        s = sg_wave_sum(s);
        if ((threadIdx.x & 63) == 0) s_ws[threadIdx.x >> 6] = s;
    }
    __syncthreads();
    if (threadIdx.x == 0) {
        const float norm = sqrtf((s_ws[0] + s_ws[1]) + (s_ws[2] + s_ws[3]));
        const float coef = max_norm / (norm + 1e-6f);
        s_coef = coef > 1.f ? 1.f : coef;
    }
    __syncthreads();
    const int i = blockIdx.x * blockDim.x + threadIdx.x;
    if (i < total) {
        const float g = grad[i] * s_coef;
        const float s = sq[i] * alpha + one_m_alpha * g * g;
        params[i] = params[i] + (-st->lr) * (g / (sqrtf(s) + eps));
        sq[i] = s;
    }
    if (blockIdx.x == 0 && threadIdx.x < 3) loss_acc[threadIdx.x] += (double)(grad[total + threadIdx.x] * inv_b);
}

__global__ __launch_bounds__(1024) void k_adv_stats(const float* ret, const float* vpred, int64_t n, float* adv,
                                                    double* stats ,
                                                    int pass) {
    __shared__ double ws[16];
    __shared__ double s_mean;
    const int tid = threadIdx.x;
    if (pass == 0) {
        double s = 0.0;
        for (int64_t i = tid; i < n; i += blockDim.x) {
            const float a = ret[i] - vpred[i];
            adv[i] = a;
            s += (double)a;
        }
        s = sg_wave_sum(s);
        if ((tid & 63) == 0) ws[tid >> 6] = s;
        __syncthreads();
        if (tid == 0) {
            double t = 0.0;
            for (int w = 0; w < (int)(blockDim.x >> 6); ++w) t += ws[w];
            stats[0] = t;
            stats[2] = (double)n;
        }
    } else if (pass == 1) {
        if (tid == 0) s_mean = (double)(float)(stats[0] / stats[2]);
        __syncthreads();
        const double mean = s_mean;
        double s = 0.0;
        for (int64_t i = tid; i < n; i += blockDim.x) {
            const double dd = (double)adv[i] - mean;
            s += dd * dd;
        }
        s = sg_wave_sum(s);
        if ((tid & 63) == 0) ws[tid >> 6] = s;
        __syncthreads();
        if (tid == 0) {
            double t = 0.0;
            for (int w = 0; w < (int)(blockDim.x >> 6); ++w) t += ws[w];
            stats[1] = t;
        }
    } else {
        const float mean = (float)(stats[0] / stats[2]);
        const float sd = (float)sqrt(stats[1] / (stats[2] - 1.0));
        for (int64_t i = tid + (int64_t)blockIdx.x * blockDim.x; i < n; i += (int64_t)gridDim.x * blockDim.x)
            adv[i] = (adv[i] - mean) / (sd + 1e-5f);
    }
}
```

simgan_amd/csrc/sg_rollout.hip:

```cpp
#include <string.h>

#include <vector>

#include "sg_common.h"
#include "sg_rng.hpp"

int sg_policy_forward_device(sg_policy* p, const float* d_obs, int n, int mode, const float* d_noise,
                             uint64_t seed, const float* d_action_in, float* d_value, float* d_action,
                             float* d_logp, float* d_ent);

extern "C" int sg_rollout_create(sg_ctx* ctx, int T, int N, int obs_dim, int act_dim, int feat_dim,
                                 sg_rollout** out) {
    SG_DEVICE_WIDE();
    SG_REQUIRE(ctx && out, "sg_rollout_create: NULL argument");
    SG_REQUIRE(T > 0 && N > 0 && obs_dim > 0 && act_dim > 0 && feat_dim >= 0, "sg_rollout_create: bad dims");
    SG_CHECK(hipSetDevice(ctx->device));
    sg_rollout* r = new sg_rollout();
    r->ctx = ctx; r->T = T; r->N = N; r->O = obs_dim; r->A = act_dim; r->F = feat_dim;
    const int slots[SG_F_COUNT] = {T + 1, T + 1, T, T, T + 1, T + 1, T, T + 1, T + 1, T};
    const int width[SG_F_COUNT] = {obs_dim, feat_dim, act_dim, 1, 1, 1, 1, 1, 1, 1};
    for (int f = 0; f < SG_F_COUNT; ++f) {
        r->field_slots[f] = slots[f];
        r->field_width[f] = width[f];
        r->field_count[f] = (int64_t)slots[f] * N * width[f];
        const size_t bytes = sizeof(float) * (size_t)(r->field_count[f] > 0 ? r->field_count[f] : 1);
        SG_CHECK(sg_dev_malloc((void**)&r->d_field[f], bytes));
        SG_CHECK(hipMemsetAsync(r->d_field[f], 0, bytes, ctx->stream));
    }
    std::vector<float> ones((size_t)(T + 1) * N, 1.0f);
    SG_CHECK(hipMemcpyAsync(r->d_field[SG_F_MASKS], ones.data(), sizeof(float) * ones.size(), hipMemcpyHostToDevice, ctx->stream));
    SG_CHECK(hipMemcpyAsync(r->d_field[SG_F_BAD_MASKS], ones.data(), sizeof(float) * ones.size(), hipMemcpyHostToDevice, ctx->stream));
    SG_CHECK(hipStreamSynchronize(ctx->stream));
    *out = r;
    return 0;
}

extern "C" int sg_rollout_destroy(sg_rollout* r) {
    SG_DEVICE_WIDE();
    if (!r) return 0;
    (void)hipStreamSynchronize(r->ctx->stream);
    for (int f = 0; f < SG_F_COUNT; ++f)
        if (r->d_field[f]) (void)sg_dev_free(r->d_field[f]);
    if (r->d_perm) (void)sg_dev_free(r->d_perm);
    delete r;
    return 0;
}

static int check_field(const sg_rollout* r, int field, const char* who) {
    SG_REQUIRE(r, "%s: rollout is NULL", who);
    SG_REQUIRE(field >= 0 && field < SG_F_COUNT, "%s: unknown field %d", who, field);
    return 0;
}

extern "C" int sg_rollout_upload(sg_rollout* r, int field, const float* host, int64_t count) {
    SG_TRY(check_field(r, field, "sg_rollout_upload"));
    SG_REQUIRE(host, "sg_rollout_upload: host is NULL");
    SG_REQUIRE(count == r->field_count[field], "sg_rollout_upload: field %d holds %lld floats, got %lld", field,
               (long long)r->field_count[field], (long long)count);
    SG_REQUIRE(field != SG_F_ADVANTAGES, "sg_rollout_upload: advantages are read-only");
    if (count == 0) return 0;
    SG_CHECK(hipMemcpyAsync(r->d_field[field], host, sizeof(float) * count, hipMemcpyHostToDevice, r->ctx->stream));
    SG_CHECK(hipStreamSynchronize(r->ctx->stream));
    if (field == SG_F_OBS_FEAT) r->feat_version = sg_next_feat_version();
    return 0;
}

extern "C" int sg_rollout_download(sg_rollout* r, int field, float* host, int64_t count) {
    SG_TRY(check_field(r, field, "sg_rollout_download"));
    SG_REQUIRE(host, "sg_rollout_download: host is NULL");
    SG_REQUIRE(count == r->field_count[field], "sg_rollout_download: field %d holds %lld floats, got %lld", field,
               (long long)r->field_count[field], (long long)count);
    if (count == 0) return 0;
    SG_CHECK(hipMemcpyAsync(host, r->d_field[field], sizeof(float) * count, hipMemcpyDeviceToHost, r->ctx->stream));
    SG_CHECK(hipStreamSynchronize(r->ctx->stream));
    return 0;
}

extern "C" int sg_rollout_upload_step(sg_rollout* r, int field, int t, const float* host, int64_t count) {
    SG_TRY(check_field(r, field, "sg_rollout_upload_step"));
    SG_REQUIRE(host, "sg_rollout_upload_step: host is NULL");
    const int64_t per = (int64_t)r->N * r->field_width[field];
    SG_REQUIRE(t >= 0 && t < r->field_slots[field], "sg_rollout_upload_step: slot %d out of range [0,%d)", t, r->field_slots[field]);
    SG_REQUIRE(count == per, "sg_rollout_upload_step: a slot of field %d holds %lld floats, got %lld", field, (long long)per, (long long)count);
    if (count == 0) return 0;
    SG_CHECK(hipMemcpyAsync(r->d_field[field] + (size_t)t * per, host, sizeof(float) * per, hipMemcpyHostToDevice, r->ctx->stream));
    SG_CHECK(hipStreamSynchronize(r->ctx->stream));
    if (field == SG_F_OBS_FEAT) r->feat_version = sg_next_feat_version();
    return 0;
}

extern "C" int sg_rollout_download_step(sg_rollout* r, int field, int t, float* host, int64_t count) {
    SG_TRY(check_field(r, field, "sg_rollout_download_step"));
    SG_REQUIRE(host, "sg_rollout_download_step: host is NULL");
    const int64_t per = (int64_t)r->N * r->field_width[field];
    SG_REQUIRE(t >= 0 && t < r->field_slots[field], "sg_rollout_download_step: slot %d out of range [0,%d)", t, r->field_slots[field]);
    SG_REQUIRE(count == per, "sg_rollout_download_step: a slot of field %d holds %lld floats, got %lld", field, (long long)per, (long long)count);
    if (count == 0) return 0;
    SG_CHECK(hipMemcpyAsync(host, r->d_field[field] + (size_t)t * per, sizeof(float) * per, hipMemcpyDeviceToHost, r->ctx->stream));
    SG_CHECK(hipStreamSynchronize(r->ctx->stream));
    return 0;
}

struct AfterUpdateArgs {
    float* base[4];
    int64_t per[4];
    int T;
};
__global__ __launch_bounds__(256) void k_after_update(AfterUpdateArgs a) {
    const int f = blockIdx.y;
    float* p = a.base[f];
    const int64_t per = a.per[f];
    for (int64_t i = (int64_t)blockIdx.x * blockDim.x + threadIdx.x; i < per; i += (int64_t)gridDim.x * blockDim.x)
        p[i] = p[(int64_t)a.T * per + i];
}

extern "C" int sg_rollout_after_update(sg_rollout* r) {
    SG_REQUIRE(r, "sg_rollout_after_update: NULL argument");
    const int fields[4] = {SG_F_OBS, SG_F_OBS_FEAT, SG_F_MASKS, SG_F_BAD_MASKS};
    AfterUpdateArgs a;
    a.T = r->T;
    for (int i = 0; i < 4; ++i) {
        a.base[i] = r->d_field[fields[i]];
        a.per[i] = (int64_t)r->N * r->field_width[fields[i]];
    }
    hipLaunchKernelGGL(k_after_update, dim3(32, 4), dim3(256), 0, r->ctx->stream, a);
    r->feat_version = sg_next_feat_version();
    SG_CHECK(hipGetLastError());
    return 0;
}

__global__ void k_compute_returns(int T, int N, const float* __restrict__ rewards, float* value_preds,
                                  float* returns, const float* __restrict__ masks,
                                  const float* __restrict__ bad_masks, const float* __restrict__ next_value,
                                  int use_gae, float gamma, float lam, int proper) {
    constexpr int C = 8;
    const int n = blockIdx.x * blockDim.x + threadIdx.x;
    if (n >= N) return;
    const float nv = next_value[n];
    float gae = 0.f, v_next = nv, ret = nv;
    if (use_gae) value_preds[(size_t)T * N + n] = nv;
    else returns[(size_t)T * N + n] = nv;
    for (int t1 = T - 1; t1 >= 0; t1 -= C) {
        float rw[C], vp[C], mk[C], bm[C];
#pragma unroll
        for (int u = 0; u < C; ++u) {
            const int t = t1 - u >= 0 ? t1 - u : 0;
            const size_t i = (size_t)t * N + n, j = i + N;
            rw[u] = rewards[i]; vp[u] = value_preds[i]; mk[u] = masks[j]; bm[u] = bad_masks[j];
        }
#pragma unroll
        for (int u = 0; u < C; ++u) {
            const int t = t1 - u;
            if (t < 0) break;
            const size_t i = (size_t)t * N + n;
            if (use_gae) {
                const float delta = rw[u] + gamma * v_next * mk[u] - vp[u];
                gae = delta + gamma * lam * mk[u] * gae;
                if (proper) gae = gae * bm[u];
                returns[i] = gae + vp[u];
                v_next = vp[u];
            } else {
                if (proper) ret = (ret * gamma * mk[u] + rw[u]) * bm[u] + (1.f - bm[u]) * vp[u];
                else ret = ret * gamma * mk[u] + rw[u];
                returns[i] = ret;
            }
        }
    }
}

static int compute_returns_dev(sg_rollout* r, const float* d_next_value, int use_gae, float gamma, float lam, int proper) {
    hipLaunchKernelGGL(k_compute_returns, dim3((r->N + 63) / 64), dim3(64), 0, r->ctx->stream, r->T, r->N,
                       r->d_field[SG_F_REWARDS], r->d_field[SG_F_VALUE_PREDS], r->d_field[SG_F_RETURNS],
                       r->d_field[SG_F_MASKS], r->d_field[SG_F_BAD_MASKS], d_next_value, use_gae, gamma, lam, proper);
    SG_CHECK(hipGetLastError());
    return 0;
}

extern "C" int sg_rollout_compute_returns(sg_rollout* r, const float* next_value, int use_gae, float gamma,
                                          float gae_lambda, int use_proper_time_limits) {
    SG_REQUIRE(r && next_value, "sg_rollout_compute_returns: NULL argument");
    float* d_nv = nullptr;
    SG_TRY(sg_ctx_scratch(r->ctx, sizeof(float) * r->N, &d_nv));
    SG_CHECK(hipMemcpyAsync(d_nv, next_value, sizeof(float) * r->N, hipMemcpyHostToDevice, r->ctx->stream));
    SG_TRY(compute_returns_dev(r, d_nv, use_gae, gamma, gae_lambda, use_proper_time_limits));
    SG_CHECK(hipStreamSynchronize(r->ctx->stream));
    return 0;
}

extern "C" int sg_rollout_compute_returns_policy(sg_rollout* r, sg_policy* p, int use_gae, float gamma,
                                                 float gae_lambda, int use_proper_time_limits) {
    SG_REQUIRE(r && p, "sg_rollout_compute_returns_policy: NULL argument");
    SG_REQUIRE(!p->recurrent, "sg_rollout_compute_returns_policy: the policy is recurrent and the device rollout holds no hidden state; "
               "pass get_value's result to sg_rollout_compute_returns");
    SG_REQUIRE(p->desc.O == r->O, "sg_rollout_compute_returns_policy: obs dim mismatch");
    float* d_nv = r->d_field[SG_F_RETURNS] + (size_t)r->T * r->N;
    SG_TRY(sg_policy_forward_device(p, r->d_field[SG_F_OBS] + (size_t)r->T * r->N * r->O, r->N, 1, nullptr, 0, nullptr,
                                    d_nv, nullptr, nullptr, nullptr));
    SG_TRY(compute_returns_dev(r, d_nv, use_gae, gamma, gae_lambda, use_proper_time_limits));
    return 0;
}

__global__ void k_count_dones(const float* masks, int64_t n, double* out) {
    __shared__ double ws[16];
    double s = 0.0;
    for (int64_t i = threadIdx.x; i < n; i += blockDim.x) s += 1.0 - (double)masks[i];
    s = sg_wave_sum(s);
    if ((threadIdx.x & 63) == 0) ws[threadIdx.x >> 6] = s;
    __syncthreads();
    if (threadIdx.x == 0) {
        double t = 0.0;
        for (int w = 0; w < (int)(blockDim.x >> 6); ++w) t += ws[w];
        *out = t;
    }
}

int sg_rollout_count_dones_dev(sg_rollout* r, double* d_out) {
    hipLaunchKernelGGL(k_count_dones, dim3(1), dim3(1024), 0, r->ctx->stream, r->d_field[SG_F_MASKS],
                       (int64_t)(r->T + 1) * r->N, d_out);
    SG_CHECK(hipGetLastError());
    if (r->ctx->use_comm) SG_TRY(sg_comm_allreduce_f64(r->ctx, d_out, 1));
    return 0;
}

extern "C" int sg_rollout_count_dones(sg_rollout* r, double* dones) {
    SG_REQUIRE(r && dones, "sg_rollout_count_dones: NULL argument");
    float* scratch = nullptr;
    SG_TRY(sg_ctx_scratch(r->ctx, 64, &scratch));
    double* d_out = reinterpret_cast<double*>(scratch);
    hipLaunchKernelGGL(k_count_dones, dim3(1), dim3(1024), 0, r->ctx->stream, r->d_field[SG_F_MASKS],
                       (int64_t)(r->T + 1) * r->N, d_out);
    SG_CHECK(hipGetLastError());
    if (r->ctx->use_comm) SG_TRY(sg_comm_allreduce_f64(r->ctx, d_out, 1));
    SG_TRY(sg_ctx_fetch_f64(r->ctx, d_out, dones, 1));
    return 0;
}

__global__ void k_fill_normal(float* x, int64_t n, uint64_t seed, uint64_t stream) {
    const int64_t i = (int64_t)blockIdx.x * blockDim.x + threadIdx.x;
    if (i < n) x[i] = sg_normal(seed, stream, (uint64_t)i);
}
__global__ void k_fill_masks(float* x, int64_t n, float p_done, uint64_t seed, uint64_t stream) {
    const int64_t i = (int64_t)blockIdx.x * blockDim.x + threadIdx.x;
    if (i < n) x[i] = sg_uniform(seed, stream, (uint64_t)i) < p_done ? 0.f : 1.f;
}
__global__ void k_fill_const(float* x, int64_t n, float v) {
    const int64_t i = (int64_t)blockIdx.x * blockDim.x + threadIdx.x;
    if (i < n) x[i] = v;
}

extern "C" int sg_rollout_fill_synthetic(sg_rollout* r, sg_policy* p, uint64_t seed, float p_done) {
    SG_REQUIRE(r && p, "sg_rollout_fill_synthetic: NULL argument");
    SG_REQUIRE(!p->recurrent, "sg_rollout_fill_synthetic: feed-forward policies only (the device rollout holds no hidden state)");
    SG_REQUIRE(p->desc.O == r->O && p->desc.A == r->A, "sg_rollout_fill_synthetic: policy/rollout dims differ");
    sg_ctx* ctx = r->ctx;
    auto blocks = [](int64_t n) { return dim3((unsigned)((n + 255) / 256)); };
    const uint64_t s = seed * 1000003ull + (uint64_t)ctx->rank;
    r->feat_version = sg_next_feat_version();
    hipLaunchKernelGGL(k_fill_normal, blocks(r->field_count[SG_F_OBS]), dim3(256), 0, ctx->stream, r->d_field[SG_F_OBS], r->field_count[SG_F_OBS], s, 1ull);
    if (r->field_count[SG_F_OBS_FEAT])
        hipLaunchKernelGGL(k_fill_normal, blocks(r->field_count[SG_F_OBS_FEAT]), dim3(256), 0, ctx->stream, r->d_field[SG_F_OBS_FEAT], r->field_count[SG_F_OBS_FEAT], s, 2ull);
    hipLaunchKernelGGL(k_fill_normal, blocks(r->field_count[SG_F_REWARDS]), dim3(256), 0, ctx->stream, r->d_field[SG_F_REWARDS], r->field_count[SG_F_REWARDS], s, 3ull);
    hipLaunchKernelGGL(k_fill_masks, blocks(r->field_count[SG_F_MASKS]), dim3(256), 0, ctx->stream, r->d_field[SG_F_MASKS], r->field_count[SG_F_MASKS], p_done, s, 4ull);
    hipLaunchKernelGGL(k_fill_const, blocks(r->field_count[SG_F_BAD_MASKS]), dim3(256), 0, ctx->stream, r->d_field[SG_F_BAD_MASKS], r->field_count[SG_F_BAD_MASKS], 1.0f);
    SG_CHECK(hipGetLastError());
    const int64_t TN = (int64_t)r->T * r->N;
    SG_TRY(sg_policy_forward_device(p, r->d_field[SG_F_OBS], (int)TN, 0, nullptr, s ^ 0xACull, nullptr,
                                    r->d_field[SG_F_VALUE_PREDS], r->d_field[SG_F_ACTIONS], r->d_field[SG_F_LOGP], nullptr));
    SG_CHECK(hipStreamSynchronize(ctx->stream));
    return 0;
}
```

simgan_amd/csrc/sg_test_api.h:

```cpp
#pragma once
#include <stdint.h>

#include "../../include/simgan_hip.h"

#ifdef __cplusplus
extern "C" {
#endif
SG_API const char *sg_test_last_error(void);
SG_API int sg_test_gemm(sg_ctx *ctx, int mode, int M, int N, int K, const float *A, const float *B, float *C);
SG_API int sg_test_gemm_bench(sg_ctx *ctx, int mode, int MT, int K, int Np, int threads, int iters, int epi, long long *cycles);
SG_API int sg_test_mfma_probe(sg_ctx *ctx, int abid, const float *a, const float *b, float *d);
SG_API int sg_test_flag_probe(sg_ctx *ctx, int mode, int np, int nc, int words, long long *stamps, float *sums);
SG_API int sg_test_fetch_probe(sg_ctx *ctx, int n_blocks, int waves, int mode, long long *out);
SG_API int sg_test_pstep_probe(sg_ctx *ctx, int mode, int S, int NW, int cyc_phase, int cyc_w, long long *stamps, int *err4);
SG_API int sg_test_pmc_calibrate(sg_ctx *ctx, int64_t mbytes);
SG_API int sg_test_graph_state(sg_ppo *a, sg_disc *d, int out[2]);
SG_API int sg_test_disc_phase_times(sg_disc *d, int enable, long long *out, int n_blocks);
SG_API int sg_test_disc_step4_times(sg_disc *d, int enable, long long *out, int n_blocks);
SG_API int sg_test_ppo_phase_times(sg_ppo *a, int enable, long long *out, int n_blocks);
SG_API int sg_test_disc_gathers(sg_disc *d, long long *out);
SG_API int sg_test_tear_probe(sg_ctx *ctx, int mode, int pairs4, int iters, long long *out4);
SG_API int sg_test_rng(sg_ctx *ctx, int kind, int64_t n, uint64_t seed, void *out);
SG_API int sg_test_raise_handoff_error(sg_disc *d, sg_ppo *a);
SG_API int sg_test_kfac_eig(sg_ctx *ctx, int n, const float *A, float *Q, float *d, int *sweeps);
SG_API int sg_test_acktr_noise(sg_ctx *ctx, int64_t n, uint64_t seed, int64_t update, float *out);
SG_API int sg_test_raise_kfac_error(sg_ppo *a);
#ifdef __cplusplus
}
#endif
```

Before: 2.503 million env-steps/s.

## Fuse small setup kernels and parallelize single-block reductions across blocks

Several tiny launches are merged or removed. The disc permutation and alpha draws go into one kernel, loss-accumulator zeroing and optimizer preparation fold into existing gather kernels, the per-epoch PPO permutations are filled in one 2D launch, and the alive-bonus computation folds into the done-count kernel. The single-block done-count and advantage-stat reductions become 64-block reductions that finish with an atomic ticket and last-block accumulation, and the two batch-stats passes merge into one kernel when comm is off. The aim is to cut launch count and serial single-block reduction time, at the cost of atomic ticket state that must stay reset and a possible change in summation order.

After: 2.499 million env-steps/s. No clear change (-0.2%).

```diff
diff --git a/simgan_amd/_lib.py b/simgan_amd/_lib.py
--- a/simgan_amd/_lib.py
+++ b/simgan_amd/_lib.py
@@ -146,6 +146,8 @@
     "sg_test_disc_gathers": (C.c_int, [H, c_ll_p]),
     "sg_test_ppo_phase_times": (C.c_int, [H, C.c_int, c_ll_p, C.c_int]),
     "sg_test_rng": (C.c_int, [H, C.c_int, C.c_int64, C.c_uint64, C.c_void_p]),
+    "sg_test_draw": (C.c_int, [H, C.c_int, C.c_int64, C.c_uint64, C.c_uint64, C.c_void_p]),
+    "sg_test_adv_stats": (C.c_int, [H, c_double_p]),
     "sg_test_kfac_eig": (C.c_int, [H, C.c_int, c_float_p, c_float_p, c_float_p, C.POINTER(C.c_int)]),
     "sg_test_acktr_noise": (C.c_int, [H, C.c_int64, C.c_uint64, C.c_int64, c_float_p]),
     "sg_test_raise_kfac_error": (C.c_int, [H]),
diff --git a/simgan_amd/csrc/sg_common.h b/simgan_amd/csrc/sg_common.h
--- a/simgan_amd/csrc/sg_common.h
+++ b/simgan_amd/csrc/sg_common.h
@@ -185,6 +185,8 @@
 uint32_t sg_comm_peer_generation(const struct sg_ctx* ctx);
 unsigned* sg_disc_err_word(struct sg_disc* d);
 uint64_t sg_next_feat_version();
+#define SG_RED_BLOCKS 64
+#define SG_RED_DOUBLES (SG_RED_BLOCKS + 1)
 struct sg_rollout {
     sg_ctx* ctx;
     int T, N, O, A, F;
@@ -193,6 +195,7 @@
     int field_slots[SG_F_COUNT] = {0};
     int field_width[SG_F_COUNT] = {0};
     int64_t* d_perm = nullptr;
+    double* d_red = nullptr;
     uint64_t feat_version = sg_next_feat_version();
 };
 
@@ -300,6 +303,49 @@
     st->step_size2[t & 1] = (float)((double)st->lr / bc1);
     st->bc2_sqrt2[t & 1] = (float)sqrt(bc2);
 }
+
+struct SgAliveArgs {
+    double* scal;
+    double n_glob, t_steps, tar_length;
+    int no_alive_bonus;
+};
+__device__ __forceinline__ void sg_alive_bonus(const SgAliveArgs& a, double done_sum) {
+    const double dones = done_sum + a.n_glob / 2.0;
+    const double expert_dones = (a.t_steps * a.n_glob) / a.tar_length;
+    const double d_sa = 1.0 - dones / (dones + expert_dones);
+    a.scal[4] = a.no_alive_bonus ? 0.0 : log(d_sa) - log(1.0 - d_sa);
+}
+
+__device__ __forceinline__ void sg_red_slice(int64_t n, int64_t* lo, int64_t* hi) {
+    const int64_t slice = (n + SG_RED_BLOCKS - 1) / SG_RED_BLOCKS;
+    const int64_t a = (int64_t)blockIdx.x * slice, b = a + slice;
+    *lo = a < n ? a : n;
+    *hi = b < n ? b : n;
+}
+__device__ __forceinline__ bool sg_red_finish(double s, double* red, double* total) {
+    __shared__ double ws[16];
+    __shared__ int last;
+    const int tid = threadIdx.x;
+    s = sg_wave_sum(s);
+    if ((tid & 63) == 0) ws[tid >> 6] = s;
+    __syncthreads();
+    if (tid == 0) {
+        double t = 0.0;
+        for (int w = 0; w < (int)(blockDim.x >> 6); ++w) t += ws[w];
+        unsigned* ticket = reinterpret_cast<unsigned*>(red + SG_RED_BLOCKS);
+        __hip_atomic_store(red + blockIdx.x, t, __ATOMIC_RELAXED, __HIP_MEMORY_SCOPE_AGENT);
+        const unsigned k = __hip_atomic_fetch_add(ticket, 1u, __ATOMIC_ACQ_REL, __HIP_MEMORY_SCOPE_AGENT);
+        last = k == gridDim.x - 1 ? 1 : 0;
+        if (last) {
+            double tot = 0.0;
+            for (int b = 0; b < (int)gridDim.x; ++b) tot += __hip_atomic_load(red + b, __ATOMIC_RELAXED, __HIP_MEMORY_SCOPE_AGENT);
+            *total = tot;
+            __hip_atomic_store(ticket, 0u, __ATOMIC_RELAXED, __HIP_MEMORY_SCOPE_AGENT);
+        }
+    }
+    __syncthreads();
+    return last != 0;
+}
 #endif
 
 #include <stdio.h>
@@ -334,7 +380,8 @@
 
 int sg_comm_graph_ok(const sg_ctx* ctx);
 void sg_comm_destroy(sg_ctx* ctx);
-int sg_rollout_count_dones_dev(sg_rollout* r, double* d_out);
+struct SgAliveArgs;
+int sg_rollout_count_dones_dev(sg_rollout* r, double* d_out, const SgAliveArgs* alive, int* alive_pending);
 int sg_comm_allreduce_f32(sg_ctx* ctx, float* dev, int64_t n);
 int sg_comm_allreduce_f64(sg_ctx* ctx, double* dev, int64_t n);
 int sg_comm_allgather_f32(sg_ctx* ctx, const float* dev_in, float* dev_out, int64_t n_per_rank);
diff --git a/simgan_amd/csrc/sg_disc.hip b/simgan_amd/csrc/sg_disc.hip
--- a/simgan_amd/csrc/sg_disc.hip
+++ b/simgan_amd/csrc/sg_disc.hip
@@ -8,8 +8,6 @@
 
 #include "sg_common.h"
 #include "sg_rng.hpp"
-
-int sg_fill_perm(sg_ctx* ctx, int64_t* d_perm, int64_t n, uint64_t seed, uint64_t stream_id);
 
 #include "sg_disc_kernels.hpp"
 #include "sg_disc_step4.hpp"
@@ -67,6 +65,16 @@
 __global__ void k_fill_alpha(float* alpha, int64_t n, uint64_t seed, uint64_t stream) {
     const int64_t i = (int64_t)blockIdx.x * blockDim.x + threadIdx.x;
     if (i < n) alpha[i] = sg_uniform(seed, stream, (uint64_t)i);
+}
+
+__global__ void k_disc_draws(int64_t* eperm, int64_t ne, int e_bits, uint64_t e_key, int64_t* pperm, int64_t np, int p_bits,
+                             uint64_t p_key, float* alpha, int64_t na, uint64_t seed, uint64_t a_stream) {
+    int64_t i = (int64_t)blockIdx.x * blockDim.x + threadIdx.x;
+    if (i < ne) { eperm[i] = sg_perm_at(i, ne, e_bits, e_key); return; }
+    i -= ne;
+    if (i < np) { pperm[i] = sg_perm_at(i, np, p_bits, p_key); return; }
+    i -= np;
+    if (i < na) alpha[i] = sg_uniform(seed, a_stream, (uint64_t)i);
 }
 
 __global__ void __launch_bounds__(128) k_disc_grad_pen(SgDiscDesc d, const float* __restrict__ W, const float* __restrict__ e,
@@ -233,6 +241,27 @@
     if ((threadIdx.x & 63) == 0) ws[threadIdx.x >> 6] = s;
     __syncthreads();
     if (threadIdx.x == 0) stats[(size_t)pass * gridDim.x + t] = ws[0] + ws[1] + ws[2] + ws[3];
+}
+
+__global__ __launch_bounds__(256) void k_batch_stats2(const float* rets, int N, double n_global, double* stats ) {
+    __shared__ double ws[4];
+    __shared__ double s_sum;
+    const int t = blockIdx.x;
+    const float* x = rets + (size_t)t * N;
+    double s = 0.0;
+    for (int i = threadIdx.x; i < N; i += blockDim.x) s += (double)x[i];
+    s = sg_wave_sum(s);
+    if ((threadIdx.x & 63) == 0) ws[threadIdx.x >> 6] = s;
+    __syncthreads();
+    if (threadIdx.x == 0) { s_sum = ws[0] + ws[1] + ws[2] + ws[3]; stats[t] = s_sum; }
+    __syncthreads();
+    const float mean = (float)(s_sum / n_global);
+    s = 0.0;
+    for (int i = threadIdx.x; i < N; i += blockDim.x) { const float dd = x[i] - mean; s += (double)(dd * dd); }
+    s = sg_wave_sum(s);
+    if ((threadIdx.x & 63) == 0) ws[threadIdx.x >> 6] = s;
+    __syncthreads();
+    if (threadIdx.x == 0) stats[(size_t)gridDim.x + t] = ws[0] + ws[1] + ws[2] + ws[3];
 }
 
 constexpr size_t SG_RMS_SCAN_LDS_BYTES = 64 * 1024;
@@ -544,14 +573,16 @@
         }
     } else {
         if (expert_perm) SG_CHECK(hipMemcpyAsync(d->d_eperm, expert_perm, sizeof(int64_t) * d->n_expert, hipMemcpyHostToDevice, ctx->stream));
-        else SG_TRY(sg_fill_perm(ctx, d->d_eperm, d->n_expert, seed, 0xE0000000ull + d->rng_calls));
         if (policy_perm) SG_CHECK(hipMemcpyAsync(d->d_pperm, policy_perm, sizeof(int64_t) * TN, hipMemcpyHostToDevice, ctx->stream));
-        else SG_TRY(sg_fill_perm(ctx, d->d_pperm, TN, seed, 0xF0000000ull + d->rng_calls * 1024 + (uint64_t)(sharded ? ctx->rank : 0)));
         if (alpha) SG_CHECK(hipMemcpyAsync(d->d_alpha, alpha, sizeof(float) * (size_t)n_d * batch_size, hipMemcpyHostToDevice, ctx->stream));
-        else {
-            const int64_t na = (int64_t)n_d * batch_size;
-            hipLaunchKernelGGL(k_fill_alpha, dim3((unsigned)((na + 255) / 256)), dim3(256), 0, ctx->stream, d->d_alpha, na,
-                               seed, 0xA1000000ull + d->rng_calls);
+        const int64_t ne = expert_perm ? 0 : d->n_expert, np = policy_perm ? 0 : TN, na = alpha ? 0 : (int64_t)n_d * batch_size;
+        if (ne + np + na > 0) {
+            const uint64_t e_key = sg_key(seed, 0x5045524Dull, 0xE0000000ull + d->rng_calls);
+            const uint64_t p_key = sg_key(seed, 0x5045524Dull, 0xF0000000ull + d->rng_calls * 1024 + (uint64_t)(sharded ? ctx->rank : 0));
+            hipLaunchKernelGGL(k_disc_draws, dim3((unsigned)((ne + np + na + 255) / 256)), dim3(256), 0, ctx->stream, d->d_eperm, ne,
+                               sg_perm_half_bits((uint64_t)d->n_expert), e_key, d->d_pperm, np, sg_perm_half_bits((uint64_t)TN), p_key,
+                               d->d_alpha, na, seed, 0xA1000000ull + d->rng_calls);
+            SG_CHECK(hipGetLastError());
         }
         if (!out3 && (expert_perm || policy_perm || alpha)) SG_CHECK(hipStreamSynchronize(ctx->stream));
     }
@@ -601,9 +632,9 @@
     const bool dbg_timing = getenv("SG_DEBUG_TIMING") != nullptr;
     const auto t_enq0 = std::chrono::steady_clock::now();
     auto enqueue_epoch = [&]() -> int {
-        hipLaunchKernelGGL(k_zero_f64, dim3(1), dim3(64), 0, ctx->stream, d->d_loss_acc, 3);
         {
             EpochRowsArgs er;
+            er.zero_acc = d->d_loss_acc;
             er.expert = d->d_expert; er.feat = a.next_feat; er.eperm = d->d_eperm; er.pperm = d->d_pperm;
             er.erows = d->d_erows; er.prows = d->d_prows; er.F = dd.F;
             if (owned) {
@@ -628,7 +659,7 @@
             wa.k1 = k + 1;
             if (k == 0) {
                 pg.erows = d->d_erows; pg.prows = d->d_prows; pg.alpha = a.alpha; pg.ops = a.ops;
-                hipLaunchKernelGGL(k_disc_pregather, dim3(2 * G), dim3(512), 0, ctx->stream, pg);
+                hipLaunchKernelGGL(k_disc_pregather, dim3(2 * G), dim3(512), 0, ctx->stream, pg, rows_total ? nullptr : d->d_loss_acc);
             }
             pg.B = k + 1 < n_d ? step_cnt[k + 1] : 0;
             pg.erows = d->d_erows + (size_t)step_off[k + 1] * dd.F; pg.prows = d->d_prows + (size_t)step_off[k + 1] * dd.F;
@@ -664,7 +695,7 @@
         const uint64_t key[12] = {(uint64_t)(uintptr_t)d->d_slabs, (uint64_t)(uintptr_t)d->d_eperm, (uint64_t)(uintptr_t)d->d_pperm,
                                   (uint64_t)(uintptr_t)d->d_alpha, (uint64_t)(uintptr_t)next_feat, (uint64_t)(uintptr_t)d->d_expert,
                                   (uint64_t)n_d, (uint64_t)B_loc, (uint64_t)batch_size,
-                                  (uint64_t)thin | (sharded ? 2u : 0u) | (gw ? 4u : 0u) | (fused ? 8u : 0u) | (sg_comm_peer_on(ctx) ? 16u : 0u) | ((uint64_t)((replicated && world > 1) ? n_cols : 0) << 8), (uint64_t)ops_f | ((uint64_t)sg_comm_peer_generation(ctx) << 40),
+                                  (uint64_t)thin | (sharded ? 2u : 0u) | (gw ? 4u : 0u) | (fused ? 8u : 0u) | (sg_comm_peer_on(ctx) ? 16u : 0u) | ((uint64_t)((replicated && world > 1) ? n_cols : 0) << 8), (uint64_t)ops_f | ((uint64_t)sg_comm_peer_generation(ctx) << 40) | (1ull << 63) ,
                                   (uint64_t)(uintptr_t)d->d_erows ^ ((uint64_t)(uintptr_t)d->d_prows << 1)};
         if (!d->epoch_graph || memcmp(key, d->epoch_graph_key, sizeof key) != 0) {
             if (d->epoch_graph) { SG_CHECK(hipGraphExecDestroy(d->epoch_graph)); d->epoch_graph = nullptr; }
@@ -900,10 +931,14 @@
                        r->d_field[SG_F_MASKS], gamma, d->returns_none ? 1 : 0, T, N, rets);
     d->returns_none = false;
     const double n_global = (double)N * ctx->world;
-    hipLaunchKernelGGL(k_batch_stats, dim3(T), dim3(256), 0, ctx->stream, rets, N, n_global, stats, 0);
-    if (ctx->use_comm) SG_TRY(sg_comm_allreduce_f64(ctx, stats, T));
-    hipLaunchKernelGGL(k_batch_stats, dim3(T), dim3(256), 0, ctx->stream, rets, N, n_global, stats, 1);
-    if (ctx->use_comm) SG_TRY(sg_comm_allreduce_f64(ctx, stats + T, T));
+    if (!ctx->use_comm) {
+        hipLaunchKernelGGL(k_batch_stats2, dim3(T), dim3(256), 0, ctx->stream, rets, N, n_global, stats);
+    } else {
+        hipLaunchKernelGGL(k_batch_stats, dim3(T), dim3(256), 0, ctx->stream, rets, N, n_global, stats, 0);
+        SG_TRY(sg_comm_allreduce_f64(ctx, stats, T));
+        hipLaunchKernelGGL(k_batch_stats, dim3(T), dim3(256), 0, ctx->stream, rets, N, n_global, stats, 1);
+        SG_TRY(sg_comm_allreduce_f64(ctx, stats + T, T));
+    }
     const size_t rms_lds = sizeof(double) * 3 * (size_t)T;
     const int rms_staged = rms_lds <= SG_RMS_SCAN_LDS_BYTES ? 1 : 0;
     hipLaunchKernelGGL(k_rms_scan, dim3(1), dim3(256), rms_staged ? rms_lds : 0, ctx->stream, stats, T, n_global, rms, scale, rms_staged);
@@ -918,20 +953,18 @@
     return relabel_core(d, r, gamma, offset, nullptr, rms_state);
 }
 
-__global__ void k_alive_bonus(double* scal, double n_glob, double t_steps, double tar_length, int no_alive_bonus) {
-    const double dones = scal[3] + n_glob / 2.0;
-    const double expert_dones = (t_steps * n_glob) / tar_length;
-    const double d_sa = 1.0 - dones / (dones + expert_dones);
-    scal[4] = no_alive_bonus ? 0.0 : log(d_sa) - log(1.0 - d_sa);
-}
+__global__ void k_alive_bonus(SgAliveArgs a) { sg_alive_bonus(a, a.scal[3]); }
 
 extern "C" int sg_disc_relabel_rewards_auto(sg_disc* d, sg_rollout* r, float gamma, double gail_tar_length, int no_alive_bonus) {
     SG_REQUIRE(d && r && gail_tar_length > 0, "sg_disc_relabel_rewards_auto: bad argument");
     sg_ctx* ctx = d->ctx;
     SG_CHECK(hipSetDevice(ctx->device));
-    SG_TRY(sg_rollout_count_dones_dev(r, d->d_scal + 3));
-    hipLaunchKernelGGL(k_alive_bonus, dim3(1), dim3(1), 0, ctx->stream, d->d_scal, (double)r->N * ctx->world, (double)r->T,
-                       gail_tar_length, no_alive_bonus);
+    SgAliveArgs al;
+    al.scal = d->d_scal; al.n_glob = (double)r->N * ctx->world; al.t_steps = (double)r->T; al.tar_length = gail_tar_length;
+    al.no_alive_bonus = no_alive_bonus;
+    int pending = 0;
+    SG_TRY(sg_rollout_count_dones_dev(r, d->d_scal + 3, &al, &pending));
+    if (pending) hipLaunchKernelGGL(k_alive_bonus, dim3(1), dim3(1), 0, ctx->stream, al);
     return relabel_core(d, r, gamma, 0.f, d->d_scal + 4, nullptr);
 }
 
diff --git a/simgan_amd/csrc/sg_disc_kernels.hpp b/simgan_amd/csrc/sg_disc_kernels.hpp
--- a/simgan_amd/csrc/sg_disc_kernels.hpp
+++ b/simgan_amd/csrc/sg_disc_kernels.hpp
@@ -72,8 +72,10 @@
     int n_d, B_loc, batch_size, roff, F;
     int remap_N, remap_W;
     int64_t TN_loc;
+    double* zero_acc;
 };
 __global__ __launch_bounds__(256) void k_disc_epoch_rows(EpochRowsArgs a) {
+    if (a.zero_acc && blockIdx.x == 0 && threadIdx.x < 3) a.zero_acc[threadIdx.x] = 0.0;
     const int64_t total = (int64_t)a.n_d * a.B_loc * a.F;
     for (int64_t i = (int64_t)blockIdx.x * blockDim.x + threadIdx.x; i < total; i += (int64_t)gridDim.x * blockDim.x) {
         const int64_t row = i / a.F;
@@ -126,8 +128,9 @@
     }
 }
 
-__global__ __launch_bounds__(512) void k_disc_pregather(PregatherArgs p) {
+__global__ __launch_bounds__(512) void k_disc_pregather(PregatherArgs p, double* zero_acc) {
     if (blockIdx.x == 0 && threadIdx.x == 0) sg_opt_prepare(p.st, p.st->t0 + 1);
+    if (zero_acc && blockIdx.x == 0 && threadIdx.x >= 64 && threadIdx.x < 67) zero_acc[threadIdx.x - 64] = 0.0;
     sg_disc_pregather(p, blockIdx.x);
 }
 
diff --git a/simgan_amd/csrc/sg_ppo.hip b/simgan_amd/csrc/sg_ppo.hip
--- a/simgan_amd/csrc/sg_ppo.hip
+++ b/simgan_amd/csrc/sg_ppo.hip
@@ -11,15 +11,15 @@
 #include "sg_kfac.hpp"
 #include "sg_gru_kernels.hpp"
 
-__global__ void k_fill_perm(int64_t* perm, int64_t n, int half_bits, uint64_t key) {
+__global__ void k_fill_perms(int64_t* perms, int64_t n, int half_bits, uint64_t seed, uint64_t rank) {
     const int64_t i = (int64_t)blockIdx.x * blockDim.x + threadIdx.x;
-    if (i < n) perm[i] = sg_perm_at(i, n, half_bits, key);
-}
-
-int sg_fill_perm(sg_ctx* ctx, int64_t* d_perm, int64_t n, uint64_t seed, uint64_t stream_id) {
-    const uint64_t key = sg_key(seed, 0x5045524Dull, stream_id);
-    hipLaunchKernelGGL(k_fill_perm, dim3((unsigned)((n + 255) / 256)), dim3(256), 0, ctx->stream, d_perm, n,
-                       sg_perm_half_bits((uint64_t)n), key);
+    const uint64_t e = blockIdx.y;
+    if (i < n) perms[e * (uint64_t)n + i] = sg_perm_at(i, n, half_bits, sg_key(seed, 0x5045524Dull, e * 2654435761ull + rank));
+}
+
+static int sg_fill_perms(sg_ctx* ctx, int64_t* d_perms, int E, int64_t n, uint64_t seed, uint64_t rank) {
+    hipLaunchKernelGGL(k_fill_perms, dim3((unsigned)((n + 255) / 256), (unsigned)E), dim3(256), 0, ctx->stream, d_perms, n,
+                       sg_perm_half_bits((uint64_t)n), seed, rank);
     SG_CHECK(hipGetLastError());
     return 0;
 }
@@ -310,12 +310,12 @@
     SG_CHECK(sg_dev_malloc((void**)&a->d_v, sizeof(float) * tot));
     SG_CHECK(sg_dev_malloc((void**)&a->d_grad, sizeof(float) * tot));
     SG_CHECK(sg_dev_malloc((void**)&a->d_state, sizeof(SgOptState)));
-    SG_CHECK(sg_dev_malloc((void**)&a->d_loss_acc, sizeof(double) * 8));
+    SG_CHECK(sg_dev_malloc((void**)&a->d_loss_acc, sizeof(double) * (8 + SG_RED_DOUBLES)));
     SG_CHECK(sg_dev_malloc((void**)&a->d_part, sizeof(float) * ((tot + 8 + SG_PPO_REDUCE_PARAMS - 1) / SG_PPO_REDUCE_PARAMS + 8 +
                                                                  (p->recurrent ? (p->gru.total + 255) / 256 : 0))));
     SG_CHECK(hipMemsetAsync(a->d_m, 0, sizeof(float) * tot, ctx->stream));
     SG_CHECK(hipMemsetAsync(a->d_v, 0, sizeof(float) * tot, ctx->stream));
-    SG_CHECK(hipMemsetAsync(a->d_loss_acc, 0, sizeof(double) * 8, ctx->stream));
+    SG_CHECK(hipMemsetAsync(a->d_loss_acc, 0, sizeof(double) * (8 + SG_RED_DOUBLES), ctx->stream));
     SG_CHECK(sg_dev_malloc((void**)&a->d_pair, SG_PAIR_BYTES));
     SG_CHECK(hipMemsetAsync(a->d_pair, 0, SG_PAIR_BYTES, ctx->stream));
     SgOptState st;
@@ -899,9 +899,10 @@
 
     float* adv = r->d_field[SG_F_ADVANTAGES];
     double* stats = a->d_loss_acc + 4;
-    hipLaunchKernelGGL(k_adv_stats, dim3(1), dim3(1024), 0, ctx->stream, r->d_field[SG_F_RETURNS], r->d_field[SG_F_VALUE_PREDS], TN, adv, stats, 0);
-    hipLaunchKernelGGL(k_adv_stats, dim3(1), dim3(1024), 0, ctx->stream, r->d_field[SG_F_RETURNS], r->d_field[SG_F_VALUE_PREDS], TN, adv, stats, 1);
-    hipLaunchKernelGGL(k_adv_stats, dim3(64), dim3(1024), 0, ctx->stream, r->d_field[SG_F_RETURNS], r->d_field[SG_F_VALUE_PREDS], TN, adv, stats, 2);
+    double* red = a->d_loss_acc + 8;
+    hipLaunchKernelGGL(k_adv_stats, dim3(SG_RED_BLOCKS), dim3(1024), 0, ctx->stream, r->d_field[SG_F_RETURNS], r->d_field[SG_F_VALUE_PREDS], TN, adv, stats, red, 0);
+    hipLaunchKernelGGL(k_adv_stats, dim3(SG_RED_BLOCKS), dim3(1024), 0, ctx->stream, r->d_field[SG_F_RETURNS], r->d_field[SG_F_VALUE_PREDS], TN, adv, stats, red, 1);
+    hipLaunchKernelGGL(k_adv_stats, dim3(64), dim3(1024), 0, ctx->stream, r->d_field[SG_F_RETURNS], r->d_field[SG_F_VALUE_PREDS], TN, adv, stats, red, 2);
     SG_CHECK(hipGetLastError());
 
     if (a->perms_cap < (int64_t)E * N) {
@@ -916,7 +917,7 @@
         SG_CHECK(hipMemcpyAsync(a->d_perms, perms, sizeof(int64_t) * (size_t)E * N, hipMemcpyHostToDevice, ctx->stream));
         if (!out3) SG_CHECK(hipStreamSynchronize(ctx->stream));
     } else {
-        for (int e = 0; e < E; ++e) SG_TRY(sg_fill_perm(ctx, a->d_perms + (size_t)e * N, N, seed, (uint64_t)e * 2654435761ull));
+        SG_TRY(sg_fill_perms(ctx, a->d_perms, E, N, seed, 0));
     }
 
     const int mb = T * per;
@@ -1176,14 +1177,15 @@
 
     float* adv = r->d_field[SG_F_ADVANTAGES];
     double* stats = a->d_loss_acc + 4;
-    hipLaunchKernelGGL(k_adv_stats, dim3(1), dim3(1024), 0, ctx->stream, r->d_field[SG_F_RETURNS],
-                       r->d_field[SG_F_VALUE_PREDS], TN, adv, stats, 0);
+    double* red = a->d_loss_acc + 8;
+    hipLaunchKernelGGL(k_adv_stats, dim3(SG_RED_BLOCKS), dim3(1024), 0, ctx->stream, r->d_field[SG_F_RETURNS],
+                       r->d_field[SG_F_VALUE_PREDS], TN, adv, stats, red, 0);
     if (ctx->use_comm) SG_TRY(sg_comm_allreduce_f64(ctx, stats, 3));
-    hipLaunchKernelGGL(k_adv_stats, dim3(1), dim3(1024), 0, ctx->stream, r->d_field[SG_F_RETURNS],
-                       r->d_field[SG_F_VALUE_PREDS], TN, adv, stats, 1);
+    hipLaunchKernelGGL(k_adv_stats, dim3(SG_RED_BLOCKS), dim3(1024), 0, ctx->stream, r->d_field[SG_F_RETURNS],
+                       r->d_field[SG_F_VALUE_PREDS], TN, adv, stats, red, 1);
     if (ctx->use_comm) SG_TRY(sg_comm_allreduce_f64(ctx, stats + 1, 1));
     hipLaunchKernelGGL(k_adv_stats, dim3(64), dim3(1024), 0, ctx->stream, r->d_field[SG_F_RETURNS],
-                       r->d_field[SG_F_VALUE_PREDS], TN, adv, stats, 2);
+                       r->d_field[SG_F_VALUE_PREDS], TN, adv, stats, red, 2);
     SG_CHECK(hipGetLastError());
 
     if (a->perms_cap < (int64_t)E * TN) {
@@ -1200,8 +1202,7 @@
         SG_CHECK(hipMemcpyAsync(a->d_perms, perms, sizeof(int64_t) * (size_t)E * TN, hipMemcpyHostToDevice, ctx->stream));
         if (!out3) SG_CHECK(hipStreamSynchronize(ctx->stream));
     } else {
-        for (int e = 0; e < E; ++e)
-            SG_TRY(sg_fill_perm(ctx, a->d_perms + (size_t)e * TN, TN, seed, (uint64_t)e * 2654435761ull + (uint64_t)ctx->rank));
+        SG_TRY(sg_fill_perms(ctx, a->d_perms, E, TN, seed, (uint64_t)ctx->rank));
     }
 
     const int ncols = d.n_trunks + (sym ? 1 : 0);
@@ -1244,7 +1245,8 @@
         SG_CHECK(hipMemsetAsync(a->d_stacks, 0, sizeof(float) * (epoch_f + stack_f), ctx->stream));
         a->scratch_key = key;
     }
-    hipLaunchKernelGGL(k_zero_f64, dim3(1), dim3(64), 0, ctx->stream, a->d_loss_acc, 4);
+    const bool fold_first = epoch_rows[0] > 0;
+    if (!fold_first) hipLaunchKernelGGL(k_zero_f64, dim3(1), dim3(64), 0, ctx->stream, a->d_loss_acc, 4);
 
     float* epX = a->d_stacks;
     float* epACT = epX + (size_t)TNp * d.ldO;
@@ -1293,10 +1295,12 @@
     SgOptState* st = reinterpret_cast<SgOptState*>(a->d_state);
 
     auto enqueue_steps = [&]() -> int {
-        hipLaunchKernelGGL(k_opt_prepare_first, dim3(1), dim3(1), 0, ctx->stream, st);
+        if (!fold_first) hipLaunchKernelGGL(k_opt_prepare_first, dim3(1), dim3(1), 0, ctx->stream, st);
         for (int e = 0; e < E; ++e) {
             ga.perm = a->d_perms + (size_t)e * TN;
             ga.TN = epoch_rows[e];
+            ga.zero_acc = (fold_first && e == 0) ? a->d_loss_acc : nullptr;
+            ga.prep_st = (fold_first && e == 0) ? st : nullptr;
             if (ga.TN) hipLaunchKernelGGL(sym ? k_ppo_epoch_gather_sym : k_ppo_epoch_gather, dim3((unsigned)((ga.TN + 63) / 64)), dim3(256), 0,
                                           ctx->stream, ga);
             for (int k = 0; k < M; ++k) {
@@ -1358,7 +1362,7 @@
                                   (uint64_t)TN, ((uint64_t)E << 32) | (uint64_t)M, ((uint64_t)MT << 32) | (uint64_t)G,
                                   ((uint64_t)fbits[0] << 32) | fbits[1], ((uint64_t)fbits[2] << 32) | fbits[3],
                                   ((uint64_t)fbits[4] << 32) | fbits[5], (uint64_t)a->cfg.use_clipped_value_loss,
-                                  (uint64_t)(uintptr_t)r->d_field[SG_F_LOGP], 0x50504full + (fused ? 1 : 0) + (ctx->use_comm ? 2 : 0) + (crit_first ? 4 : 0) + (gw ? 8 : 0) + (pair ? 16 : 0) + (sg_comm_peer_on(ctx) ? 32 : 0) + (sym ? 64 : 0) + ((uint64_t)sg_comm_peer_generation(ctx) << 32),
+                                  (uint64_t)(uintptr_t)r->d_field[SG_F_LOGP], 0x50504Full + (fold_first ? 0x1000000ull : 0) + (fused ? 1 : 0) + (ctx->use_comm ? 2 : 0) + (crit_first ? 4 : 0) + (gw ? 8 : 0) + (pair ? 16 : 0) + (sg_comm_peer_on(ctx) ? 32 : 0) + (sym ? 64 : 0) + ((uint64_t)sg_comm_peer_generation(ctx) << 32),
                                   sym ? (uint64_t)(uintptr_t)a->d_mrows : 0, sym ? (uint64_t)cbits : 0};
         if (!a->steps_graph || memcmp(key, a->steps_graph_key, sizeof key) != 0) {
             if (a->steps_graph) { SG_CHECK(hipGraphExecDestroy(a->steps_graph)); a->steps_graph = nullptr; }
diff --git a/simgan_amd/csrc/sg_ppo_kernels.hpp b/simgan_amd/csrc/sg_ppo_kernels.hpp
--- a/simgan_amd/csrc/sg_ppo_kernels.hpp
+++ b/simgan_amd/csrc/sg_ppo_kernels.hpp
@@ -50,6 +50,8 @@
     float *X, *ACT, *SC;
     const float* mobs;
     float* Xm;
+    double* zero_acc;
+    SgOptState* prep_st;
 };
 
 template <bool SYM = false, bool ROLLOUT_ORDER = false>
@@ -57,6 +59,10 @@
     __shared__ int IDX[64];
     const int tid = threadIdx.x;
     const int64_t row0 = (int64_t)blockIdx.x * 64;
+    if (blockIdx.x == 0) {
+        if (a.zero_acc && tid >= 64 && tid < 68) a.zero_acc[tid - 64] = 0.0;
+        if (a.prep_st && tid == 128) sg_opt_prepare(a.prep_st, a.prep_st->t0 + 1);
+    }
     if (tid < 64) {
         const int64_t rr = row0 + tid;
         const int idx = rr < a.TN ? (ROLLOUT_ORDER ? (int)rr : (int)a.perm[rr]) : -1;
@@ -711,43 +717,31 @@
 
 __global__ __launch_bounds__(1024) void k_adv_stats(const float* ret, const float* vpred, int64_t n, float* adv,
                                                     double* stats ,
-                                                    int pass) {
-    __shared__ double ws[16];
-    __shared__ double s_mean;
+                                                    double* red, int pass) {
     const int tid = threadIdx.x;
     if (pass == 0) {
-        double s = 0.0;
-        for (int64_t i = tid; i < n; i += blockDim.x) {
+        int64_t lo, hi;
+        sg_red_slice(n, &lo, &hi);
+        double s = 0.0, t;
+        for (int64_t i = lo + tid; i < hi; i += blockDim.x) {
             const float a = ret[i] - vpred[i];
             adv[i] = a;
             s += (double)a;
         }
-        s = sg_wave_sum(s);
-        if ((tid & 63) == 0) ws[tid >> 6] = s;
-        __syncthreads();
-        if (tid == 0) {
-            double t = 0.0;
-            for (int w = 0; w < (int)(blockDim.x >> 6); ++w) t += ws[w];
+        if (sg_red_finish(s, red, &t) && tid == 0) {
             stats[0] = t;
             stats[2] = (double)n;
         }
     } else if (pass == 1) {
-        if (tid == 0) s_mean = (double)(float)(stats[0] / stats[2]);
-        __syncthreads();
-        const double mean = s_mean;
-        double s = 0.0;
-        for (int64_t i = tid; i < n; i += blockDim.x) {
+        int64_t lo, hi;
+        sg_red_slice(n, &lo, &hi);
+        const double mean = (double)(float)(stats[0] / stats[2]);
+        double s = 0.0, t;
+        for (int64_t i = lo + tid; i < hi; i += blockDim.x) {
             const double dd = (double)adv[i] - mean;
             s += dd * dd;
         }
-        s = sg_wave_sum(s);
-        if ((tid & 63) == 0) ws[tid >> 6] = s;
-        __syncthreads();
-        if (tid == 0) {
-            double t = 0.0;
-            for (int w = 0; w < (int)(blockDim.x >> 6); ++w) t += ws[w];
-            stats[1] = t;
-        }
+        if (sg_red_finish(s, red, &t) && tid == 0) stats[1] = t;
     } else {
         const float mean = (float)(stats[0] / stats[2]);
         const float sd = (float)sqrt(stats[1] / (stats[2] - 1.0));
diff --git a/simgan_amd/csrc/sg_rollout.hip b/simgan_amd/csrc/sg_rollout.hip
--- a/simgan_amd/csrc/sg_rollout.hip
+++ b/simgan_amd/csrc/sg_rollout.hip
@@ -30,6 +30,8 @@
     std::vector<float> ones((size_t)(T + 1) * N, 1.0f);
     SG_CHECK(hipMemcpyAsync(r->d_field[SG_F_MASKS], ones.data(), sizeof(float) * ones.size(), hipMemcpyHostToDevice, ctx->stream));
     SG_CHECK(hipMemcpyAsync(r->d_field[SG_F_BAD_MASKS], ones.data(), sizeof(float) * ones.size(), hipMemcpyHostToDevice, ctx->stream));
+    SG_CHECK(sg_dev_malloc((void**)&r->d_red, sizeof(double) * SG_RED_DOUBLES));
+    SG_CHECK(hipMemsetAsync(r->d_red, 0, sizeof(double) * SG_RED_DOUBLES, ctx->stream));
     SG_CHECK(hipStreamSynchronize(ctx->stream));
     *out = r;
     return 0;
@@ -42,6 +44,7 @@
     for (int f = 0; f < SG_F_COUNT; ++f)
         if (r->d_field[f]) (void)sg_dev_free(r->d_field[f]);
     if (r->d_perm) (void)sg_dev_free(r->d_perm);
+    if (r->d_red) (void)sg_dev_free(r->d_red);
     delete r;
     return 0;
 }
@@ -200,23 +203,24 @@
     return 0;
 }
 
-__global__ void k_count_dones(const float* masks, int64_t n, double* out) {
-    __shared__ double ws[16];
-    double s = 0.0;
-    for (int64_t i = threadIdx.x; i < n; i += blockDim.x) s += 1.0 - (double)masks[i];
-    s = sg_wave_sum(s);
-    if ((threadIdx.x & 63) == 0) ws[threadIdx.x >> 6] = s;
-    __syncthreads();
-    if (threadIdx.x == 0) {
-        double t = 0.0;
-        for (int w = 0; w < (int)(blockDim.x >> 6); ++w) t += ws[w];
+__global__ __launch_bounds__(1024) void k_count_dones(const float* masks, int64_t n, double* out, double* red, SgAliveArgs alive) {
+    int64_t lo, hi;
+    sg_red_slice(n, &lo, &hi);
+    double s = 0.0, t;
+    for (int64_t i = lo + threadIdx.x; i < hi; i += blockDim.x) s += 1.0 - (double)masks[i];
+    if (sg_red_finish(s, red, &t) && threadIdx.x == 0) {
         *out = t;
-    }
-}
-
-int sg_rollout_count_dones_dev(sg_rollout* r, double* d_out) {
-    hipLaunchKernelGGL(k_count_dones, dim3(1), dim3(1024), 0, r->ctx->stream, r->d_field[SG_F_MASKS],
-                       (int64_t)(r->T + 1) * r->N, d_out);
+        if (alive.scal) sg_alive_bonus(alive, t);
+    }
+}
+
+int sg_rollout_count_dones_dev(sg_rollout* r, double* d_out, const SgAliveArgs* alive, int* alive_pending) {
+    SgAliveArgs none;
+    memset(&none, 0, sizeof none);
+    const bool fold = alive && !r->ctx->use_comm;
+    if (alive_pending) *alive_pending = (alive && !fold) ? 1 : 0;
+    hipLaunchKernelGGL(k_count_dones, dim3(SG_RED_BLOCKS), dim3(1024), 0, r->ctx->stream, r->d_field[SG_F_MASKS],
+                       (int64_t)(r->T + 1) * r->N, d_out, r->d_red, fold ? *alive : none);
     SG_CHECK(hipGetLastError());
     if (r->ctx->use_comm) SG_TRY(sg_comm_allreduce_f64(r->ctx, d_out, 1));
     return 0;
@@ -227,10 +231,7 @@
     float* scratch = nullptr;
     SG_TRY(sg_ctx_scratch(r->ctx, 64, &scratch));
     double* d_out = reinterpret_cast<double*>(scratch);
-    hipLaunchKernelGGL(k_count_dones, dim3(1), dim3(1024), 0, r->ctx->stream, r->d_field[SG_F_MASKS],
-                       (int64_t)(r->T + 1) * r->N, d_out);
-    SG_CHECK(hipGetLastError());
-    if (r->ctx->use_comm) SG_TRY(sg_comm_allreduce_f64(r->ctx, d_out, 1));
+    SG_TRY(sg_rollout_count_dones_dev(r, d_out, nullptr, nullptr));
     SG_TRY(sg_ctx_fetch_f64(r->ctx, d_out, dones, 1));
     return 0;
 }
diff --git a/simgan_amd/csrc/sg_test_api.h b/simgan_amd/csrc/sg_test_api.h
--- a/simgan_amd/csrc/sg_test_api.h
+++ b/simgan_amd/csrc/sg_test_api.h
@@ -21,6 +21,8 @@
 SG_API int sg_test_disc_gathers(sg_disc *d, long long *out);
 SG_API int sg_test_tear_probe(sg_ctx *ctx, int mode, int pairs4, int iters, long long *out4);
 SG_API int sg_test_rng(sg_ctx *ctx, int kind, int64_t n, uint64_t seed, void *out);
+SG_API int sg_test_draw(sg_ctx *ctx, int kind, int64_t n, uint64_t seed, uint64_t stream, void *out);
+SG_API int sg_test_adv_stats(sg_ppo *a, double out3[3]);
 SG_API int sg_test_raise_handoff_error(sg_disc *d, sg_ppo *a);
 SG_API int sg_test_kfac_eig(sg_ctx *ctx, int n, const float *A, float *Q, float *d, int *sweeps);
 SG_API int sg_test_acktr_noise(sg_ctx *ctx, int64_t n, uint64_t seed, int64_t update, float *out);
```
